# blefaudeux/rusty-marcher

Measured on AMD Instinct MI355X. Metric: Mpixels/sec at 1920x1080, max-bounce=5, higher is better.
Workload: dtype f64

## Files before the change

### rusty-marcher_amd/csrc/rm_classify.inc

```
namespace RM_FLAVOR_NS {
using namespace rmdev;

__device__ __forceinline__ V3 unit(V3 a) {
    const double x = dot(a, a);
    double y = __builtin_amdgcn_rsq(x);
    const double h = 0.5 * x;
    y = y * (1.5 - h * y * y);
    y = y * (1.5 - h * y * y);
    return scaled(a, y);
}

#if RM_KERNEL_ORIENTED
__device__ __forceinline__ V3 cls_dir(const KernelArgs &a, double bx, double by) {
    return mk((bx * a.cam_rx + by * a.cam_ux) + a.cam_fx, (bx * a.cam_ry + by * a.cam_uy) + a.cam_fy, (bx * a.cam_rz + by * a.cam_uz) + a.cam_fz);
}
#else
__device__ __forceinline__ V3 cls_dir(const KernelArgs &, double bx, double by) { return mk(bx, by, -1.); }
#endif
template <bool SHARED>
__device__ __forceinline__ bool cone_of(Bundle &b, const KernelArgs &a, double bx0, double bx1, double by0, double by1, uint32_t sub) {
    const V3 u = unit(cls_dir(a, 0.5 * (bx0 + bx1), 0.5 * (by0 + by1)));
    double cm;
    if (SHARED) {
        cm = dot(unit(cls_dir(a, (sub & 1u) ? bx1 : bx0, (sub & 2u) ? by1 : by0)), u);
// ... 93 lines not shown
struct ClsAsked { double px0, px1, py0, py1, tx0, tx1, ty0, ty1; };
__device__ __forceinline__ ClsAsked classify_ask(const KernelArgs &a, uint32_t patch, bool valid) {
    const uint32_t tile = (valid ? patch : 0u) * 16u + (threadIdx.x & 15u);
    uint32_t tx0, ty0, tyf, ty8;
    tile_origin(a, tile, tx0, ty0, tyf, ty8);
    const uint32_t px0 = tx0 & ~31u, py0 = ty0 & ~31u;
    return ClsAsked{a.bp_x[px0], a.bp_x[px0 + 31u], a.bp_y[py0], a.bp_y[py0 + 31u],
                    a.bp_x[tx0], a.bp_x[tx0 + TILE_W - 1u], a.bp_y[ty0], a.bp_y[ty0 + TILE_H - 1u]};
}
template <bool EDGES>
__device__ __forceinline__ bool classify_patches(const ClsView &scene_blob, const KernelArgs &a, uint32_t patch, bool valid, const ClsAsked &asked,
                                                 unsigned long long *__restrict__ tile_mask, uint32_t n, uint32_t tag, unsigned long long &sig, unsigned long long &own) {
    const uint32_t lane = threadIdx.x & 63u, sub = lane & 15u;
    const uint32_t tile = (valid ? patch : 0u) * 16u + sub;

    Bundle b;
    const bool patch_usable = cone_of<true>(b, a, asked.px0, asked.px1, asked.py0, asked.py1, sub);
    unsigned long long pm = 0ull;
#ifdef RM_CLASSIFY_TWO_CHAINS
    for (uint32_t base = 0; base < n; base += 32u) {
        const uint32_t pid_a = base + sub, pid_b = base + 16u + sub;
        const bool in_a = pid_a < n, in_b = pid_b < n;
        bool keep_a, keep_b;
        keeps2<EDGES>(scene_blob, a, b, pid_a, in_a, pid_b, in_b, keep_a, keep_b);
        pm |= (in_a & (keep_a | !patch_usable)) ? (1ull << (pid_a & 63u)) : 0ull;
        pm |= (in_b & (keep_b | !patch_usable)) ? (1ull << (pid_b & 63u)) : 0ull;
    }
#else
    for (uint32_t base = 0; base < n; base += 16u) {
        const uint32_t pid = base + sub;
        const bool in = pid < n;
        const bool keep = in & (keeps<EDGES>(scene_blob, a, b, pid, in) | !patch_usable);
        pm |= keep ? (1ull << (pid & 63u)) : 0ull;
    }
#endif
    auto group_or = [](unsigned long long v) {
        for (uint32_t off = 1u; off < 16u; off <<= 1) {
            const uint32_t lo = (uint32_t)v | (uint32_t)__shfl_xor((int)(uint32_t)v, (int)off, 64);
            const uint32_t hi = (uint32_t)(v >> 32) | (uint32_t)__shfl_xor((int)(uint32_t)(v >> 32), (int)off, 64);
            v = ((unsigned long long)hi << 32) | lo;
        }
        return v;
    };
    pm = group_or(pm);

    unsigned long long mask = 0ull;
    if (n > (tag ? 56u : 64u)) {
        mask = pm != 0ull ? ~0ull : 0ull;
    } else if (__any(pm != 0ull)) {
        const bool tile_usable = cone_of<false>(b, a, asked.tx0, asked.tx1, asked.ty0, asked.ty1, sub);
        unsigned long long m = pm;
#ifdef RM_CLASSIFY_TWO_CHAINS
        while (__any(m != 0ull)) {
            const bool in_a = m != 0ull;
            const uint32_t pid_a = in_a ? (uint32_t)__builtin_ctzll(m) : 0u;
            m &= m - 1ull;
            const bool in_b = m != 0ull;
            const uint32_t pid_b = in_b ? (uint32_t)__builtin_ctzll(m) : 0u;
            m &= m - 1ull;
            bool keep_a, keep_b;
            keeps2<EDGES>(scene_blob, a, b, pid_a, in_a, pid_b, in_b, keep_a, keep_b);
            mask |= (in_a & (keep_a | !tile_usable)) ? (1ull << pid_a) : 0ull;
            mask |= (in_b & (keep_b | !tile_usable)) ? (1ull << pid_b) : 0ull;
        }
#else
        while (__any(m != 0ull)) {
            const bool in = m != 0ull;
            const uint32_t pid = in ? (uint32_t)__builtin_ctzll(m) : 0u;
            m &= m - 1ull;
            const bool keep = in & (keeps<EDGES>(scene_blob, a, b, pid, in) | !tile_usable);
            mask |= keep ? (1ull << pid) : 0ull;
        }
#endif
    }
    if (valid) {
        if (tag) __hip_atomic_store(tile_mask + tile, ((unsigned long long)tag << 56) | (mask & 0x00FFFFFFFFFFFFFFull), __ATOMIC_RELAXED, __HIP_MEMORY_SCOPE_AGENT);
        else tile_mask[tile] = mask;
    }
    own = valid ? mask : 0ull;
    sig = group_or(own);
    return sig != 0ull;
}

__device__ __forceinline__ uint32_t cost_bucket(uint32_t ticks) {
    if (ticks < 512u) return RM_ORD_SKY - 1u;
    const uint32_t e = 31u - (uint32_t)__builtin_clz(ticks);
    const uint32_t b = 2u * (e - 9u) + ((ticks >> (e - 1u)) & 1u);
    return RM_ORD_SKY - 1u - min(b, RM_ORD_SKY - 1u);
}

struct OrdRec { uint32_t patch, bucket_slot, index; };

struct OrdAsked { uint32_t done, index, cost; };
__device__ __forceinline__ OrdAsked order_ask(const KernelArgs &a, uint32_t patch, bool valid) {
    OrdAsked q;
    q.done = (a.static_list && a.lists_done) ? *a.lists_done : 0u;
    q.index = a.dyn_index ? a.dyn_index[valid ? patch : 0u] : 0u;
    q.cost = (a.key_mode == RM_KEY_COST && a.cost_prev) ? a.cost_prev[valid ? patch : 0u] : 0u;
    return q;
}
__device__ __forceinline__ void order_slot(const KernelArgs &a, uint32_t id, uint32_t patch, bool valid, unsigned long long sig, unsigned long long own, uint32_t prim_cost, const OrdAsked &asked, OrdRec *rec, uint32_t *grec) {
    const uint32_t lane = threadIdx.x & 63u, n_patches = a.n_tiles >> 4, n_dyn = n_patches - (a.n_static >> 4);
    uint32_t c = 0u;
    if (a.key_mode == RM_KEY_CONTENT) {
        unsigned long long m = (valid && own != ~0ull) ? own : 0ull;
        bool unseen = false;
        while (__any(m != 0ull)) {
            const bool in = m != 0ull;
            const uint32_t pid = in ? (uint32_t)__builtin_ctzll(m) : 0u;
            const uint32_t v = (uint32_t)__shfl((int)prim_cost, (int)pid, 64);
            m &= m - 1ull;
            unseen = unseen | (in & (v == ~0u));
            c = max(c, (in && v != ~0u) ? v : 0u);
        }
        c = unseen ? 0x00FFFFFFu : c;
        for (uint32_t off = 1u; off < 16u; off <<= 1) c = max(c, (uint32_t)__shfl_xor((int)c, (int)off, 64));
    } else if (a.key_mode == RM_KEY_COST) {
        c = asked.cost;
    }
    const bool leader = (lane & 15u) == 0u;
    const bool have_lists = a.static_list && a.lists_done && uniform_u32(asked.done) == a.lists_tag;
    const uint32_t index = !valid ? RM_ORD_STATIC_BIT : have_lists ? asked.index : patch < n_dyn ? 0u : RM_ORD_STATIC_BIT | (n_patches - 1u - patch);
    const bool placed = valid & leader & !(index & RM_ORD_STATIC_BIT), first_round = valid & leader & ((index & RM_ORD_STATIC_BIT) != 0u);
    const uint32_t bucket = sig == 0ull ? RM_ORD_SKY
                          : a.key_mode == RM_KEY_PLACE ? (uint32_t)(((unsigned long long)(n_patches - 1u - patch) * (RM_ORD_SKY)) / n_patches)
                                                       : cost_bucket(c);
    const uint32_t counter = bucket * RM_ORD_SUBS + (id & (RM_ORD_SUBS - 1u));
    const uint32_t key = (placed | first_round) ? ((first_round ? RM_ORD_COUNTERS : 0u) | counter) : 0xFFFFu;
    uint32_t before = 0u, total = 0u, first_of = lane >> 4;
#pragma unroll
    for (uint32_t i = 0; i < 4u; i++) {
        const bool same = (uint32_t)__builtin_amdgcn_readlane((int)key, (int)(16u * i)) == key;
        total += same ? 1u : 0u;
        before += (same & (i < (lane >> 4))) ? 1u : 0u;
        first_of = (same & (i < first_of)) ? i : first_of;
    }
    uint32_t base = 0u;
    if (key != 0xFFFFu && before == 0u)
        base = __hip_atomic_fetch_add(a.ord_cnt + ((key & RM_ORD_COUNTERS) ? RM_ORD_FIRST : 0u) + (key & (RM_ORD_COUNTERS - 1u)) * RM_ORD_LINE, total, __ATOMIC_RELAXED, __HIP_MEMORY_SCOPE_AGENT);
    const uint32_t slot = (uint32_t)__shfl((int)base, (int)(16u * first_of), 64) + before;
    if (leader) {
        rec[lane >> 4].patch = valid ? patch : ~0u;
        rec[lane >> 4].bucket_slot = (counter << 24) | slot;
        rec[lane >> 4].index = index;
        if (grec) {
            __hip_atomic_store(grec + (lane >> 4) * 3u + 0u, valid ? patch : ~0u, __ATOMIC_RELAXED, __HIP_MEMORY_SCOPE_AGENT);
            __hip_atomic_store(grec + (lane >> 4) * 3u + 1u, (counter << 24) | slot, __ATOMIC_RELAXED, __HIP_MEMORY_SCOPE_AGENT);
            __hip_atomic_store(grec + (lane >> 4) * 3u + 2u, index, __ATOMIC_RELAXED, __HIP_MEMORY_SCOPE_AGENT);
        }
        if (valid && a.cost_zero) a.cost_zero[patch] = 0u;
    }
}

__device__ __forceinline__ void order_places(const KernelArgs &a, uint32_t id, const OrdRec *rec, bool arrive, bool wait) {
    const uint32_t lane = threadIdx.x & 63u, n_patches = a.n_tiles >> 4, ns16 = a.n_static >> 4, n_dyn = n_patches - ns16;
    const uint32_t n_groups = (a.cls_blocks + 31u) >> 5;
    uint32_t go = 0u;
    if (arrive && lane == 0u && !(a.test_stall == 2u && a.ord_read == a.ord_flat)) {
        const uint32_t g = id >> 5, of = min(32u, a.cls_blocks - 32u * g);
        if (__hip_atomic_fetch_add(a.ord_cnt + RM_ORD_ARRIVE + g * RM_ORD_LINE, 1u, __ATOMIC_RELAXED, __HIP_MEMORY_SCOPE_AGENT) + 1u == of)
            if (__hip_atomic_fetch_add(a.ord_cnt + RM_ORD_GROUPS, 1u, __ATOMIC_RELAXED, __HIP_MEMORY_SCOPE_AGENT) + 1u == n_groups) {
                uint32_t expected = 0u;
                go = __hip_atomic_compare_exchange_strong(a.ord_cnt + RM_ORD_GO, &expected, a.ord_tag, __ATOMIC_RELAXED, __ATOMIC_RELAXED, __HIP_MEMORY_SCOPE_AGENT) ? a.ord_tag : expected;
                if (go == a.ord_tag && a.lists_done_next && a.static_next) *a.lists_done_next = a.ord_tag;
            }
    }
// ... 57 lines not shown
```

### rusty-marcher_amd/csrc/rm_device.hip

```cpp
#include <hip/hip_runtime.h>

#include <chrono>
#include <cmath>
#include <cstdio>
#include <cstdlib>
#include <cstring>
#include <initializer_list>
#include <limits>
#include <new>
#include <string>
#include <utility>
#include <vector>

#include "rm_image.hpp"
#include "rm_internal.h"
#include "rm_kernel_args.hpp"
#include "rm_plan.hpp"
#include "rm_sampling.hpp"
#include "rm_query.hpp"
#include "rm_radiance.hpp"
#include "rm_refine.hpp"
#include "rm_lens.hpp"
#include "rm_accum.hpp"
#include "rm_soft.hpp"
// ... 40 lines not shown
        m = __builtin_fmax(__builtin_fmax(part[0], part[1]), __builtin_fmax(part[2], part[3]));
        atomicMax(out_bits, (unsigned long long)__double_as_longlong(m));
    }
}

__global__ __launch_bounds__(256) void rm_scale_quantize_kernel(double *__restrict__ v, size_t n, const unsigned long long *max_bits,
                                                               int do_scale, uint8_t *__restrict__ out8) {
    double s = 1.;
    bool scale = false;
    if (do_scale) {
        const double max_val = __longlong_as_double((long long)*max_bits);
        if (max_val > 0.) { s = 1. / max_val; scale = true; }
    }
    for (size_t i = (size_t)blockIdx.x * blockDim.x + threadIdx.x; i < n; i += (size_t)gridDim.x * blockDim.x) {
        double f = v[i];
        if (scale) { f = f * s; v[i] = f; }
        if (out8) {
            const double c = 255. * __builtin_fmin(__builtin_fmax(f, 0.), 1.);
            out8[i] = (uint8_t)c;
        }
    }
}


struct rm_frame_slot {
    hipStream_t render = nullptr;
    hipEvent_t begun = nullptr, rendered = nullptr, gathered = nullptr;
    hipEvent_t exchanged = nullptr;
    bool used = false;
    bool stamped = false;
};

struct rm_feedback {
    hipStream_t stream = nullptr;
    void *block = nullptr;
    size_t set_bytes = 0;
    uint64_t used = 0;
    rm_feedback_state s;
};

struct rm_hostio;
struct rm_progressive;
struct rm_tick_swept;
struct rm_converging;
struct rm_denoising;

struct rm_tile_lists {
    hipStream_t stream = nullptr;
    uint32_t cap = 0;
    void *block = nullptr;
    uint64_t used = 0;
    void *order_block = nullptr;
    uint32_t order_cap = 0;
    unsigned long long *hint = nullptr;
    rm_stream_state s;
    unsigned long long *mask() const { return static_cast<unsigned long long *>(block); }
};

struct rm_ctx {
    int device = -1;
    hipStream_t stream = nullptr;
    hipEvent_t ev0 = nullptr, ev1 = nullptr;
    std::string error;
    hipDeviceProp_t prop{};

    bool have_scene = false;
    rm_image image;
    double *d_scene = nullptr;
    size_t d_scene_words = 0;
    rm_vec3 camera{0., 0., 0.};
    bool oriented = false;
    rm_camera_basis basis{{1., 0., 0.}, {0., 1., 0.}, {0., 0., -1.}};
    uint64_t upload_calls = 0, upload_copies = 0;
    std::vector<unsigned char> desc_bytes;
    size_t desc_sizes[6] = {0, 0, 0, 0, 0, 0};
    const rm_knobs knobs = rm_knobs_from_env();
    bool last_launch_exact_only = false;
    uint32_t *d_redo = nullptr;
    std::vector<rm_feedback> feedback;
    uint64_t feedback_clock = 0, scene_epoch = 0;
    uint64_t image_epoch = 0;
    std::vector<rm_tile_lists> tile_lists;
    uint32_t last_launch_grid = 0, last_launch_tail = 0;
    uint32_t last_launch_tiles = 0;
    bool last_launch_classified = false;
    hipStream_t last_launch_stream = nullptr;

    double *d_frame = nullptr;
    size_t frame_bytes = 0;
    uint32_t frame_w = 0, frame_h = 0;

    void *comm = nullptr;
    void *slot_comm[RM_MAX_FRAME_SLOTS] = {};
    int n_comms = 0;
    bool frame_stamps = false;
    bool exchange_all_ranks = false;
    bool comm_failed = false;
    bool comm_local = false;
    int rank = 0, world = 1;
    rm_frame_slot slots[RM_MAX_FRAME_SLOTS];

    double *d_backproject = nullptr;
    size_t backproject_words = 0;
    double backproject_key[6] = {};

    rm_hostio *hostio = nullptr;
    bool comm_stuck = false;

    uint32_t *d_pid_map = nullptr;
    size_t pid_map_words = 0;
    void *d_query = nullptr;
    size_t query_bytes = 0;

    std::vector<std::pair<const void *, int>> shade_occupancy;

    void *d_refine_ws = nullptr;
    size_t refine_ws_bytes = 0;

    void *d_lens_table = nullptr;
    void *d_lens_frame = nullptr;
    size_t lens_frame_bytes = 0;

    rm_progressive *progressive = nullptr;

    rm_converging *converging = nullptr;

    rm_denoising *denoising = nullptr;

    rm_tick_swept *tick_swept = nullptr;
    uint32_t swept_walked = 0;
    uint32_t swept_builds = 0;
    std::vector<rm_swept *> swept_handles;

    unsigned long long *d_max = nullptr;
    uint8_t *d_rgb8 = nullptr;
    size_t rgb8_bytes = 0;
};

static void hostio_destroy(rm_ctx *ctx, bool device_ok);
static bool hostio_packs(rm_ctx *ctx, size_t band_bytes);
static void progressive_destroy(rm_ctx *ctx, bool device_ok);
static void converging_destroy(rm_ctx *ctx, bool device_ok);
static void denoising_destroy(rm_ctx *ctx, bool device_ok);
static void tick_swept_destroy(rm_ctx *ctx, bool device_ok);

static rm_status ctx_fail(rm_ctx *ctx, rm_status st, const std::string &msg) {
    if (ctx) ctx->error = msg;
    else rm_set_host_error(msg);
    return st;
}

template <class F>
static rm_status guarded(rm_ctx *ctx, const char *who, F &&body) {
    try {
        return body();
    } catch (const std::bad_alloc &) {
        return ctx_fail(ctx, RM_ERR_INVALID_ARG, std::string(who) + ": out of host memory");
    } catch (const std::exception &e) {
        return ctx_fail(ctx, RM_ERR_INVALID_ARG, std::string(who) + ": " + e.what());
    } catch (...) {
        return ctx_fail(ctx, RM_ERR_INVALID_ARG, std::string(who) + ": unexpected exception");
    }
}

template <class T>
static T *entry_of(std::vector<T> &v, hipStream_t stream) {
// ... 308 lines not shown
    if (!p) return ctx_fail(ctx, RM_ERR_INVALID_ARG, "render: NULL params");
    if (!ctx->have_scene) return ctx_fail(ctx, RM_ERR_NO_SCENE, "render: no scene uploaded (rm_scene_upload)");
    if (p->patch_size != RM_PATCH_SIZE) return ctx_fail(ctx, RM_ERR_INVALID_ARG, "render: patch_size must be 32 (renderer.rs:47)");
    if (p->max_depth > RM_MAX_DEPTH) return ctx_fail(ctx, RM_ERR_DEPTH, "render: max_depth above RM_MAX_DEPTH");
    if (p->frame_width == 0 || p->frame_height == 0) return ctx_fail(ctx, RM_ERR_INVALID_ARG, "render: empty frame");
    if (p->frame_width % RM_PATCH_SIZE != 0)
        return ctx_fail(ctx, RM_ERR_DIMENSIONS,
                        "render: frame width is not a multiple of 32; the reference's scatter "
                        "(renderer.rs:92-108) indexes out of bounds and panics");
    if (!rm_band_of(*p, band)) return ctx_fail(ctx, RM_ERR_INVALID_ARG, "render: patch_row_begin > patch_row_end");
    return RM_OK;
}

static rm_status backproject_tables(rm_ctx *ctx, const rm_params *p) {
    const double key[6] = {p->width, p->height, p->half_fov, p->ratio, (double)p->frame_width, (double)p->frame_height};
    if (ctx->d_backproject && std::memcmp(key, ctx->backproject_key, sizeof key) == 0) return RM_OK;
    std::vector<double> t((size_t)p->frame_width + p->frame_height);
    for (uint32_t x = 0; x < p->frame_width; x++) t[x] = 2. * ((double)x / p->width - 0.5) * p->half_fov * p->ratio;
    for (uint32_t y = 0; y < p->frame_height; y++) t[p->frame_width + y] = -2. * ((double)y / p->height - 0.5) * p->half_fov;
    RM_HIP(ctx, hipDeviceSynchronize());
    if (ctx->backproject_words < t.size()) {
        if (ctx->d_backproject) RM_HIP(ctx, hipFree(ctx->d_backproject));
        ctx->d_backproject = nullptr;
        RM_HIP(ctx, hipMalloc(&ctx->d_backproject, t.size() * sizeof(double)));
        ctx->backproject_words = t.size();
    }
    RM_HIP(ctx, hipMemcpy(ctx->d_backproject, t.data(), t.size() * sizeof(double), hipMemcpyHostToDevice));
    std::memcpy(ctx->backproject_key, key, sizeof key);
    return RM_OK;
}

static constexpr uint32_t RM_FEEDBACK_STREAMS = 8, RM_CLASSIFY_STREAMS = 8;

static rm_status feedback_for(rm_ctx *ctx, hipStream_t stream, const rm_launch_plan &P, rm_feedback **out) {
    rm_feedback *f = entry_of(ctx->feedback, stream);
    if (!f) {
        if (ctx->feedback.size() >= RM_FEEDBACK_STREAMS) {
            size_t old = 0;
            for (size_t i = 1; i < ctx->feedback.size(); i++)
                if (ctx->feedback[i].used < ctx->feedback[old].used) old = i;
            if (ctx->feedback[old].block) RM_HIP(ctx, hipFree(ctx->feedback[old].block));
            ctx->feedback.erase(ctx->feedback.begin() + (long)old);
        }
        ctx->feedback.emplace_back();
        f = &ctx->feedback.back();
        f->stream = stream;
    }
    f->used = ++ctx->feedback_clock;
    if (P.feedback_reset) {
        f->s.valid = false;
        if (!f->block || f->set_bytes != P.feedback_set_bytes) {
            if (f->block) RM_HIP(ctx, hipFree(f->block));
            f->block = nullptr;
            RM_HIP(ctx, hipMalloc(&f->block, P.feedback_bytes));
        }
        f->set_bytes = P.feedback_set_bytes;
        RM_HIP(ctx, hipMemsetAsync(f->block, 0, P.feedback_bytes, stream));
    }
    *out = f;
    return RM_OK;
}

static rm_status tile_lists_for(rm_ctx *ctx, hipStream_t stream, uint32_t n_tiles, rm_tile_lists **out) {
    rm_tile_lists *t = entry_of(ctx->tile_lists, stream);
    if (!t) {
        if (ctx->tile_lists.size() >= RM_CLASSIFY_STREAMS) {
            size_t old = 0;
            for (size_t i = 1; i < ctx->tile_lists.size(); i++)
                if (ctx->tile_lists[i].used < ctx->tile_lists[old].used) old = i;
            if (ctx->tile_lists[old].block) RM_HIP(ctx, hipFree(ctx->tile_lists[old].block));
            if (ctx->tile_lists[old].order_block) RM_HIP(ctx, hipFree(ctx->tile_lists[old].order_block));
            if (ctx->tile_lists[old].hint) RM_HIP(ctx, hipHostFree(ctx->tile_lists[old].hint));
            ctx->tile_lists.erase(ctx->tile_lists.begin() + (long)old);
        }
        ctx->tile_lists.emplace_back();
        t = &ctx->tile_lists.back();
        t->stream = stream;
    }
    t->used = ++ctx->feedback_clock;
    if (!t->block || t->cap < n_tiles) {
        if (t->block) RM_HIP(ctx, hipFree(t->block));
        t->block = nullptr;
        t->cap = n_tiles;
        RM_HIP(ctx, hipMalloc(&t->block, (size_t)n_tiles * sizeof(unsigned long long)));
    }
    *out = t;
    return RM_OK;
}

static rm_status void_frame_check(rm_ctx *ctx, const char *who) {
    for (rm_tile_lists &t : ctx->tile_lists)
        if (t.hint) {
            const unsigned long long e = *(volatile unsigned long long *)(t.hint + 1);
            if (e) {
                *(volatile unsigned long long *)(t.hint + 1) = 0ull;
                return ctx_fail(ctx, RM_ERR_HIP, std::string(who) + ": launch " + std::to_string((uint32_t)(e >> 32)) +
                                                     " of its stream gave up waiting for its own classification (that frame is void)");
            }
        }
    return RM_OK;
}

static rm_plan_scene plan_scene_of(const rm_ctx *ctx) {
    const rm_image &img = ctx->image;
    return rm_plan_scene{&img.H, ctx->scene_epoch, img.occ_camera_limit, img.integer_exponents, ctx->oriented,
                         ctx->camera, &ctx->basis, (uint32_t)ctx->prop.multiProcessorCount, img.exact_only, img.dead_camera_limit};
}

static rm_status no_kernel(rm_ctx *ctx) { return ctx_fail(ctx, RM_ERR_INVALID_ARG, "render: no kernel for this scene / depth combination"); }

static rm_status choose_kernel(rm_ctx *ctx, const rm_params *p, uint32_t tiles, rm_kernel_choice *k) {
    return choose_kernel(ctx->knobs, plan_scene_of(ctx), *p, tiles, k) ? RM_OK : no_kernel(ctx);
}

static rm_status dump_order(rm_ctx *ctx, const rm_launch_plan &P, hipStream_t stream) {
    const KernelArgs &a = P.args;
    uint32_t c[RM_ORD_BUCKETS] = {}, c1[RM_ORD_BUCKETS] = {}, raw[RM_ORD_ARRIVE] = {};
    RM_HIP(ctx, hipStreamSynchronize(stream));
    RM_HIP(ctx, hipMemcpy(raw, a.ord_cnt, sizeof raw, hipMemcpyDeviceToHost));
    for (uint32_t b = 0; b < RM_ORD_BUCKETS; b++)
        for (uint32_t u = 0; u < RM_ORD_SUBS; u++) { c[b] += raw[(b * RM_ORD_SUBS + u) * RM_ORD_LINE]; c1[b] += raw[RM_ORD_FIRST + (b * RM_ORD_SUBS + u) * RM_ORD_LINE]; }
    uint32_t lit = 0;
    for (uint32_t b = 0; b < RM_ORD_SKY; b++) lit += c[b];
    std::fprintf(stderr, "[rm_order] launch %u keys %u: %u classifying workgroups x %u, first round %u waves, %u + %u sky places; tail %u, room to hand on %u, handed on %u; buckets", a.launch_seq, a.key_mode,
                 a.cls_blocks, a.cls_iters, a.n_static, lit, c[RM_ORD_SKY], a.tail_patches, a.ov_cap, a.tail_patches > c[RM_ORD_SKY] ? std::min(a.ov_cap, a.tail_patches - c[RM_ORD_SKY]) : 0u);
    for (uint32_t b = 0; b < RM_ORD_BUCKETS; b++) std::fprintf(stderr, " %u", c[b]);
    std::fprintf(stderr, " | first round's");
    for (uint32_t b = 0; b < RM_ORD_BUCKETS; b++) std::fprintf(stderr, " %u", c1[b]);
    const uint32_t n_pat = a.n_tiles / 16u, n_dyn_ = n_pat - a.n_static / 16u;
    std::vector<uint32_t> fl(n_dyn_);
    RM_HIP(ctx, hipMemcpy(fl.data(), a.ord_flat, n_dyn_ * sizeof(uint32_t), hipMemcpyDeviceToHost));
    std::vector<uint8_t> seen(n_pat, 0);
    uint32_t untagged = 0, twice = 0, bad = 0;
    for (uint32_t v : fl) {
        if ((v >> RM_ORD_TAG_SHIFT) != a.ord_tag) { untagged++; continue; }
        const uint32_t pch = v & (RM_ORD_SKY_BIT - 1u);
        if (pch >= n_pat) { bad++; continue; }
        twice += seen[pch]; seen[pch] = 1;
    }
    std::fprintf(stderr, " | order laid out: %u places, %u without the tag, %u patches twice, %u out of range; dispatched by %s order; places written %s\n", n_dyn_, untagged, twice, bad,
                 a.ord_read == a.ord_flat ? "its own" : "its predecessor's", a.ord_rec ? "at the grid's end" : "by the classifying workgroups");
    return RM_OK;
}

#if defined(RM_EXP_STAMPS) || defined(RM_EXP_PHASES)
static rm_status stamps_begin(rm_ctx *ctx, rm_launch_plan &P, hipStream_t stream) {
    const size_t n_waves = (size_t)P.grid * P.k.mode.waves;
    RM_HIP(ctx, hipMalloc(&P.args.debug_stamps, n_waves * 48));
    RM_HIP(ctx, hipMemsetAsync(P.args.debug_stamps, 0, n_waves * 48, stream));
    return RM_OK;
}
static rm_status stamps_end(rm_ctx *ctx, const rm_launch_plan &P, hipStream_t stream) {
    const KernelArgs &a = P.args;
    const size_t n_waves = (size_t)P.grid * P.k.mode.waves;
    RM_HIP(ctx, hipStreamSynchronize(stream));
    if (const char *path = std::getenv("RM_DEBUG_STAMPS")) {
        std::fprintf(stderr, "stamps: grid %u cls_blocks %u n_static %u n_tiles %u tail_patches %u tail_q %u ov_cap %u key_mode %u\n", P.grid, a.cls_blocks, a.ord_cnt ? a.n_static : 0u, a.n_tiles, a.tail_patches, a.tail_q, a.ov_cap, a.key_mode);
        std::vector<unsigned long long> h(n_waves * 4);
        RM_HIP(ctx, hipMemcpy(h.data(), a.debug_stamps, n_waves * 32, hipMemcpyDeviceToHost));
        if (FILE *f = std::fopen(path, "wb")) { std::fwrite(h.data(), 8, h.size(), f); std::fclose(f); }
        std::vector<unsigned long long> x(n_waves * 2);
        RM_HIP(ctx, hipMemcpy(x.data(), a.debug_stamps + n_waves * 4, n_waves * 16, hipMemcpyDeviceToHost));
        if (FILE *f = std::fopen((std::string(path) + ".ext").c_str(), "wb")) { std::fwrite(x.data(), 8, x.size(), f); std::fclose(f); }
    }
    RM_HIP(ctx, hipFree(a.debug_stamps));
    return RM_OK;
}
#endif

static rm_status launch_render(rm_ctx *ctx, const rm_params *p, const rm_band &band, double *d_frame,
                               uint8_t *d_frame8, hipStream_t stream) {
    const uint32_t n_rows = band.count();
    if (n_rows == 0) return RM_OK;
    if (p->max_depth == 0) {
        const uint32_t run = band.stride == 1 ? n_rows : 1u;
        for (uint32_t k = 0; k < n_rows; k += run) {
            const size_t first_px = (size_t)((p->flags & RM_FLAG_F64_COMPACT) ? k : band.begin + k * band.stride) * 32u * p->frame_width;
            const size_t n_px = (size_t)run * 32u * p->frame_width;
            hipLaunchKernelGGL(rm_fill_band_kernel, dim3((unsigned)((n_px + 255) / 256)), dim3(256), 0, stream, d_frame,
                               first_px, n_px, p->background.x, p->background.y, p->background.z);
            RM_HIP(ctx, hipGetLastError());
        }
        return RM_OK;
    }
    rm_status bst = backproject_tables(ctx, p);
    if (bst != RM_OK) return bst;
    static const rm_stream_state no_launches;
    static const rm_feedback_state no_feedback;
    rm_tile_lists *tl = entry_of(ctx->tile_lists, stream);
    rm_feedback *fb = entry_of(ctx->feedback, stream);
    const unsigned long long hint = tl && tl->hint ? *(volatile unsigned long long *)tl->hint : 0ull;
    rm_launch_plan P;
    if (!plan_launch(ctx->knobs, plan_scene_of(ctx), *p, band, tl ? tl->s : no_launches, tl ? tl->order_cap : 0u, fb ? fb->s : no_feedback, hint, &P))
        return no_kernel(ctx);
    if (P.ordered)
        if (rm_status vst = void_frame_check(ctx, "render")) return vst;

    if (P.feedback)
        if (rm_status fst = feedback_for(ctx, stream, P, &fb)) return fst;
    if (P.classify) {
        if (rm_status cst = tile_lists_for(ctx, stream, P.args.n_tiles, &tl)) return cst;
        if (P.clear_masks) RM_HIP(ctx, hipMemsetAsync(tl->block, 0, (size_t)tl->cap * sizeof(unsigned long long), stream));
    }
    if (P.ordered) {
        if (tl->order_cap < P.order_patches) {
            if (tl->order_block) RM_HIP(ctx, hipFree(tl->order_block));
            tl->order_block = nullptr;
            tl->order_cap = 0;
            RM_HIP(ctx, hipMalloc(&tl->order_block, rm_order_layout{P.order_cap}.bytes()));
            tl->order_cap = P.order_cap;
        }
        const rm_order_layout L{tl->order_cap};
        if (P.order_clear == rm_launch_plan::ORDER_CLEAR_ALL)
            RM_HIP(ctx, hipMemsetAsync(tl->order_block, 0, L.bytes(), stream));
        else if (P.order_clear == rm_launch_plan::ORDER_CLEAR_FLAT)
            RM_HIP(ctx, hipMemsetAsync(static_cast<uint32_t *>(tl->order_block) + L.flat(0), 0, 2u * L.cap * sizeof(uint32_t), stream));
        if (!tl->hint) {
            RM_HIP(ctx, hipHostMalloc((void **)&tl->hint, 2u * sizeof(unsigned long long), hipHostMallocDefault));
            tl->hint[0] = tl->hint[1] = 0ull;
        }
    }

    KernelArgs &a = P.args;
    char *base[RM_BUF_COUNT] = {};
    if (P.classify) { base[RM_BUF_MASKS] = static_cast<char *>(tl->block); base[RM_BUF_ORDER] = static_cast<char *>(tl->order_block); base[RM_BUF_HINT] = reinterpret_cast<char *>(tl->hint); }
    if (P.feedback) base[RM_BUF_FEEDBACK] = static_cast<char *>(fb->block);
    for (uint32_t i = 0; i < P.n_refs; i++) {
        char *at = base[P.refs[i].buf] + P.refs[i].offset;
        std::memcpy(reinterpret_cast<char *>(&a) + P.refs[i].field, &at, sizeof at);
    }
    a.bp_x = ctx->d_backproject;
    a.bp_y = ctx->d_backproject + p->frame_width;
    a.frame8 = d_frame8;
    a.redo_count = ctx->d_redo;

    if (P.cls_fn) {
        P.cls_args.tile_mask = tl->mask();
        void *cargs[] = {(void *)&ctx->d_scene, (void *)&a, (void *)&P.cls_args};
        RM_HIP(ctx, hipLaunchKernel(P.cls_fn, dim3(P.cls_grid), dim3(64), cargs, 0, stream));
    }
#if defined(RM_EXP_STAMPS) || defined(RM_EXP_PHASES)
    if (rm_status sst = stamps_begin(ctx, P, stream)) return sst;
#endif
    void *args[] = {(void *)&ctx->d_scene, (void *)&a, (void *)&d_frame};
    RM_HIP(ctx, hipLaunchKernel(P.k.fn, dim3(P.grid), dim3(P.block), args, P.lds_bytes, stream));

    if (P.classify) tl->s = P.after;
    if (P.feedback) fb->s = P.feedback_after;
    ctx->last_launch_tiles = a.n_tiles;
    ctx->last_launch_classified = P.classify;
    ctx->last_launch_stream = stream;
    ctx->last_launch_grid = P.grid;
    ctx->last_launch_tail = a.tail_patches;
    ctx->last_launch_exact_only = P.exact_only;
    if (ctx->knobs.debug_tail && P.ordered)
        if (rm_status dst = dump_order(ctx, P, stream)) return dst;
#if defined(RM_EXP_STAMPS) || defined(RM_EXP_PHASES)
    if (rm_status sst = stamps_end(ctx, P, stream)) return sst;
#endif
    return RM_OK;
}

static rm_status rm_render_device_impl(rm_ctx *ctx, const rm_params *params, void *device_rgb, void *hip_stream) {
    if (!ctx) return ctx_fail(nullptr, RM_ERR_INVALID_ARG, "rm_render_device: NULL ctx");
    if (!device_rgb) return ctx_fail(ctx, RM_ERR_INVALID_ARG, "rm_render_device: NULL device buffer");
    rm_band band;
    rm_status st = check_params(ctx, params, &band);
    if (st != RM_OK) return st;
    RM_HIP(ctx, hipSetDevice(ctx->device));
    hipStream_t s = (hipStream_t)hip_stream;
    return launch_render(ctx, params, band, (double *)device_rgb, nullptr, s);
}

rm_status rm_render_device(rm_ctx *ctx, const rm_params *params, void *device_rgb, void *hip_stream) {
    return guarded(ctx, "rm_render_device", [&]() { return rm_render_device_impl(ctx, params, device_rgb, hip_stream); });
}

static rm_status rm_render_device_u8_impl(rm_ctx *ctx, const rm_params *params, void *device_rgb, void *device_rgb8,
                              void *hip_stream) {
    if (!ctx) return ctx_fail(nullptr, RM_ERR_INVALID_ARG, "rm_render_device_u8: NULL ctx");
    if (!device_rgb || !device_rgb8) return ctx_fail(ctx, RM_ERR_INVALID_ARG, "rm_render_device_u8: NULL device buffer");
    rm_band band;
    rm_status st = check_params(ctx, params, &band);
    if (st != RM_OK) return st;
    if (params->max_depth == 0)
        return ctx_fail(ctx, RM_ERR_DEPTH, "rm_render_device_u8: max_depth 0 renders no ray; use rm_render_device + rm_postprocess");
    RM_HIP(ctx, hipSetDevice(ctx->device));
    return launch_render(ctx, params, band, (double *)device_rgb, (uint8_t *)device_rgb8, (hipStream_t)hip_stream);
}

rm_status rm_render_device_u8(rm_ctx *ctx, const rm_params *params, void *device_rgb, void *device_rgb8,
                              void *hip_stream) {
    return guarded(ctx, "rm_render_device_u8", [&]() { return rm_render_device_u8_impl(ctx, params, device_rgb, device_rgb8, hip_stream); });
}

static rm_status rm_render_impl(rm_ctx *ctx, const rm_params *params, double *host_rgb, rm_timing *timing) {
    if (!ctx) return ctx_fail(nullptr, RM_ERR_INVALID_ARG, "rm_render: NULL ctx");
    const auto t_begin = std::chrono::steady_clock::now();
    rm_band band;
    rm_status st = check_params(ctx, params, &band);
    if (st != RM_OK) return st;
    if (params->flags & (RM_FLAG_F64_COMPACT | RM_FLAG_U8_COMPACT))
        return ctx_fail(ctx, RM_ERR_INVALID_ARG, "rm_render: the packed layouts are for rm_render_device* (caller-owned device buffers)");
    RM_HIP(ctx, hipSetDevice(ctx->device));

    const size_t need = (size_t)params->frame_width * params->frame_height * 3u * sizeof(double);
    if (ctx->frame_bytes != need || ctx->frame_w != params->frame_width || ctx->frame_h != params->frame_height) {
        RM_HIP(ctx, hipStreamSynchronize(ctx->stream));
        if (ctx->d_frame) RM_HIP(ctx, hipFree(ctx->d_frame));
        ctx->d_frame = nullptr;
        ctx->frame_bytes = 0;
        RM_HIP(ctx, hipMalloc(&ctx->d_frame, need));
        RM_HIP(ctx, hipMemsetAsync(ctx->d_frame, 0, need, ctx->stream));
        ctx->frame_bytes = need;
        ctx->frame_w = params->frame_width;
        ctx->frame_h = params->frame_height;
    }

    const size_t row_bytes = (size_t)params->frame_width * 3u * sizeof(double);
    const uint32_t n_rows = band.count();
    if (host_rgb && n_rows > 0 && hostio_packs(ctx, (size_t)n_rows * 32u * row_bytes)) {
        std::vector<double *> rows(params->frame_height);
        for (uint32_t y = 0; y < params->frame_height; y++) rows[y] = host_rgb + (size_t)y * params->frame_width * 3u;
        return rm_render_rows(ctx, params, rows.data(), timing);
    }
    RM_HIP(ctx, hipEventRecord(ctx->ev0, ctx->stream));
    st = launch_render(ctx, params, band, ctx->d_frame, nullptr, ctx->stream);
    if (st != RM_OK) return st;
    RM_HIP(ctx, hipEventRecord(ctx->ev1, ctx->stream));

    double d2h_ms = 0.;
    if (host_rgb && n_rows > 0) {
        RM_HIP(ctx, hipStreamSynchronize(ctx->stream));
        const auto t0 = std::chrono::steady_clock::now();
        const uint32_t run = band.stride == 1 ? n_rows : 1u;
        for (uint32_t k = 0; k < n_rows; k += run) {
            const size_t off = (size_t)(band.begin + k * band.stride) * 32u * row_bytes;
            RM_HIP(ctx, hipMemcpy((char *)host_rgb + off, (const char *)ctx->d_frame + off, (size_t)run * 32u * row_bytes,
                                  hipMemcpyDeviceToHost));
        }
        d2h_ms = std::chrono::duration<double, std::milli>(std::chrono::steady_clock::now() - t0).count();
    } else {
        RM_HIP(ctx, hipStreamSynchronize(ctx->stream));
    }
    if (rm_status vst = void_frame_check(ctx, "rm_render")) return vst;
    if (timing) {
        float ms = 0.f;
        RM_HIP(ctx, hipEventElapsedTime(&ms, ctx->ev0, ctx->ev1));
        timing->kernel_ms = ms;
        timing->d2h_ms = d2h_ms;
        timing->total_ms = std::chrono::duration<double, std::milli>(std::chrono::steady_clock::now() - t_begin).count();
    }
    return RM_OK;
}

rm_status rm_render(rm_ctx *ctx, const rm_params *params, double *host_rgb, rm_timing *timing) {
    return guarded(ctx, "rm_render", [&]() { return rm_render_impl(ctx, params, host_rgb, timing); });
}

rm_status rm_kernel_name(rm_ctx *ctx, const rm_params *params, char *buf, size_t buflen) {
    if (!ctx) return ctx_fail(nullptr, RM_ERR_INVALID_ARG, "rm_kernel_name: NULL ctx");
    if (!buf || buflen == 0) return ctx_fail(ctx, RM_ERR_INVALID_ARG, "rm_kernel_name: NULL buffer");
    rm_band band;
    rm_status st = check_params(ctx, params, &band);
    if (st != RM_OK) return st;
    if (params->max_depth == 0) { std::snprintf(buf, buflen, "rm_fill_band_kernel"); return RM_OK; }
    rm_kernel_choice k;
    st = choose_kernel(ctx, params, band.count() * (params->frame_width / RM_PATCH_SIZE) * 16u, &k);
    if (st != RM_OK) return st;
    std::snprintf(buf, buflen, "%s%s::rm_render_static<%d, %d, %d, %d, %s, %s, %s, %s, %s, %s>", k.fast ? "rmdev_fast" : "rmdev_strict", ctx->oriented ? "_o" : "", k.stack,
                  k.pow_mode, k.mode.waves, k.mode.per_wave, k.staged ? "true" : "false", k.bvh ? "true" : "false",
                  k.cull ? "true" : "false", k.edges ? "true" : "false", (k.order || ctx->oriented) ? "true" : "false", k.feedback ? "true" : "false");
    return RM_OK;
}

rm_status rm_launch_stats(rm_ctx *ctx, uint32_t *workgroups, uint32_t *tail_patches) {
    if (!ctx) return ctx_fail(nullptr, RM_ERR_INVALID_ARG, "rm_launch_stats: NULL ctx");
    if (workgroups) *workgroups = ctx->last_launch_grid;
    if (tail_patches) *tail_patches = ctx->last_launch_tail;
    return RM_OK;
}

static rm_status rm_tile_stats_impl(rm_ctx *ctx, void *hip_stream, uint32_t *tiles, uint32_t *tiles_listed) {
    if (!ctx) return ctx_fail(nullptr, RM_ERR_INVALID_ARG, "rm_tile_stats: NULL ctx");
    RM_HIP(ctx, hipSetDevice(ctx->device));
    RM_HIP(ctx, hipDeviceSynchronize());
    const uint32_t n = ctx->last_launch_tiles;
    uint32_t listed = n;
    for (const rm_tile_lists &t : ctx->tile_lists)
        if (t.stream == (hip_stream ? (hipStream_t)hip_stream : ctx->last_launch_stream) && t.block && ctx->last_launch_classified && n <= t.cap) {
            std::vector<unsigned long long> m(n);
            RM_HIP(ctx, hipMemcpy(m.data(), t.mask(), (size_t)n * 8u, hipMemcpyDeviceToHost));
            listed = 0;
            uint32_t hist[64] = {};
            uint64_t bits = 0;
            for (unsigned long long v : m) {
                if (t.s.tagged) v &= 0x00FFFFFFFFFFFFFFull;
                listed += v != 0ull;
                for (int b = 0; b < 64 && v != ~0ull; b++)
                    if (v >> b & 1ull) { hist[b]++; bits++; }
            }
            if (std::getenv("RM_DEBUG_CLASSIFY")) {
                std::fprintf(stderr, "[rm_classify] %u of %u tiles have something to hit, %.2f primitives each; tiles per pid:", listed, n,
                             listed ? (double)bits / listed : 0.);
                for (int b = 0; b < 64; b++)
                    if (hist[b]) std::fprintf(stderr, " %d:%u", b, hist[b]);
                std::fprintf(stderr, "\n");
            }
        }
    if (tiles) *tiles = n;
    if (tiles_listed) *tiles_listed = listed;
    return RM_OK;
}

rm_status rm_tile_stats(rm_ctx *ctx, void *hip_stream, uint32_t *tiles, uint32_t *tiles_listed) {
    return guarded(ctx, "rm_tile_stats", [&]() { return rm_tile_stats_impl(ctx, hip_stream, tiles, tiles_listed); });
}

rm_status rm_device_framebuffer(rm_ctx *ctx, void **device_rgb, size_t *bytes) {
    if (!ctx) return ctx_fail(nullptr, RM_ERR_INVALID_ARG, "rm_device_framebuffer: NULL ctx");
    if (!ctx->d_frame) return ctx_fail(ctx, RM_ERR_INVALID_ARG, "rm_device_framebuffer: nothing rendered yet");
    if (device_rgb) *device_rgb = ctx->d_frame;
    if (bytes) *bytes = ctx->frame_bytes;
    return RM_OK;
}

static rm_status rm_postprocess_impl(rm_ctx *ctx, void *device_rgb, uint32_t w, uint32_t h, int normalize, uint8_t *host_rgb8,
                         double *max_out) {
    if (!ctx) return ctx_fail(nullptr, RM_ERR_INVALID_ARG, "rm_postprocess: NULL ctx");
    RM_HIP(ctx, hipSetDevice(ctx->device));
    double *v = (double *)device_rgb;
    if (!v) {
        if (!ctx->d_frame) return ctx_fail(ctx, RM_ERR_INVALID_ARG, "rm_postprocess: nothing rendered yet");
        if (w != ctx->frame_w || h != ctx->frame_h)
            return ctx_fail(ctx, RM_ERR_INVALID_ARG, "rm_postprocess: size differs from the rendered frame");
        v = ctx->d_frame;
    }
    const size_t n = (size_t)w * h * 3u;
    if (n == 0) return ctx_fail(ctx, RM_ERR_INVALID_ARG, "rm_postprocess: empty frame");
    const unsigned blocks = (unsigned)std::min<size_t>((n + 255) / 256, 2048);
    RM_HIP(ctx, hipMemsetAsync(ctx->d_max, 0, sizeof(unsigned long long), ctx->stream));
    if (normalize) {
        hipLaunchKernelGGL(rm_max_kernel, dim3(blocks), dim3(256), 0, ctx->stream, v, n, ctx->d_max);
        RM_HIP(ctx, hipGetLastError());
    }
    uint8_t *d8 = nullptr;
    if (host_rgb8) {
        if (ctx->rgb8_bytes < n) {
            RM_HIP(ctx, hipStreamSynchronize(ctx->stream));
            if (ctx->d_rgb8) RM_HIP(ctx, hipFree(ctx->d_rgb8));
            ctx->d_rgb8 = nullptr;
            ctx->rgb8_bytes = 0;
            RM_HIP(ctx, hipMalloc(&ctx->d_rgb8, n));
            ctx->rgb8_bytes = n;
        }
        d8 = ctx->d_rgb8;
    }
    if (normalize || d8) {
        hipLaunchKernelGGL(rm_scale_quantize_kernel, dim3(blocks), dim3(256), 0, ctx->stream, v, n, ctx->d_max,
                           normalize ? 1 : 0, d8);
        RM_HIP(ctx, hipGetLastError());
    }
    RM_HIP(ctx, hipStreamSynchronize(ctx->stream));
// ... 37 lines not shown
```

### rusty-marcher_amd/csrc/rm_image.cpp

```cpp
#include "rm_image.hpp"

#include <algorithm>
#include <cmath>
#include <cstring>
#include <limits>

#include "rm_bvh.hpp"
#include "rm_plan.hpp"

namespace {

constexpr uint64_t RM_SCENE_MAX_WORDS = 0xFFFFFFF0ull;
constexpr size_t RM_BVH_MIN_SPHERES = 16, RM_BVH_MIN_TRIANGLES = 12;
constexpr uint32_t RM_SHADOW_MASK_MAX_PRIMS = 64u;
constexpr unsigned RM_EMPTY_SIDE_POS = 1u, RM_EMPTY_SIDE_NEG = 2u;
constexpr double RM_EMPTY_SIDES_CAMERA_MAX = 1e9;

inline uint64_t pack_u32x2(uint32_t lo, uint32_t hi) { return (uint64_t)lo | ((uint64_t)hi << 32); }

inline rm_vec3 v3(double x, double y, double z) { return rm_vec3{x, y, z}; }
inline rm_vec3 operator-(rm_vec3 a, rm_vec3 b) { return v3(a.x - b.x, a.y - b.y, a.z - b.z); }
inline rm_vec3 scaled(rm_vec3 a, double s) { return v3(a.x * s, a.y * s, a.z * s); }
inline double dot(rm_vec3 a, rm_vec3 b) { return a.x * b.x + a.y * b.y + a.z * b.z; }
inline rm_vec3 cross(rm_vec3 a, rm_vec3 b) { return v3(a.y * b.z - a.z * b.y, a.z * b.x - a.x * b.z, a.x * b.y - a.y * b.x); }


struct PlaneSep { bool h = false, n = false; };
inline void try_plane(PlaneSep &sep, rm_vec3 n, const rm_vec3 *w, uint32_t nv, rm_vec3 cl, double r, rm_vec3 a, double sin_t,
                      double marg) {
    const double len = std::sqrt(dot(n, n));
    if (!(len > 1e-150) || !std::isfinite(len)) return;
    n = scaled(n, 1. / len);
    for (int sign = 0; sign < 2; sign++, n = scaled(n, -1.)) {
        double lo = HUGE_VAL;
        for (uint32_t i = 0; i < nv; i++) lo = std::fmin(lo, dot(w[i], n));
        if (!std::isfinite(lo)) continue;
        sep.h = sep.h || lo > std::fmax(0., dot(cl, n) + r) + marg;
        sep.n = sep.n || (dot(a, n) >= sin_t + 1e-9 && lo > marg);
    }
}

void rm_build_shadow_masks(const double *blob, const rm_dev_header &H, unsigned long long *occ) {
    const uint32_t n = H.n_spheres + H.n_polygons + H.n_triangles, nl = H.n_lights;
    const unsigned long long all = n >= 64u ? ~0ull : ((1ull << n) - 1ull);
    const double rho = H.shadow_rho;
    auto finite3 = [](rm_vec3 v) { return std::isfinite(v.x) && std::isfinite(v.y) && std::isfinite(v.z); };
    auto mag = [](rm_vec3 v) { return std::fabs(v.x) + std::fabs(v.y) + std::fabs(v.z); };
    for (uint32_t l = 0; l < nl; l++) {
        const double *lw = blob + H.off_lights + RM_LIGHT_WORDS * l;
        const rm_vec3 L = v3(lw[0], lw[1], lw[2]);
        for (uint32_t P = 0; P < n; P++) {
            unsigned long long &m = occ[(size_t)P * nl + l];
            m = all;
            const double *bp = blob + H.off_bounds + 4u * P;
            const rm_vec3 c = v3(bp[0], bp[1], bp[2]);
            if (!(bp[3] >= 0.) || !std::isfinite(bp[3]) || !finite3(c) || !finite3(L) || !(rho >= 0.) || !std::isfinite(rho)) continue;
            const double tol = 1e-7 * (1. + mag(L) + mag(c) + bp[3]);
            const double r = bp[3] + tol;
            const rm_vec3 cl = c - L;
            const double D = std::sqrt(dot(cl, cl));
            if (!(D > r * (1. + 1e-6) + rho + tol)) continue;
            const rm_vec3 a = scaled(cl, 1. / D);
            const double sin_t = std::fmin(1., r / D * (1. + 1e-9) + 1e-9);
            const double cos_t = std::sqrt(std::fmax(0., 1. - sin_t * sin_t)) * (1. - 1e-9);
            const double cap = D + r;
            unsigned long long keep = 1ull << P;
            for (uint32_t Q = 0; Q < n; Q++) {
                if (Q == P) continue;
                const double *bq = blob + H.off_bounds + 4u * Q;
                if (bq[3] < 0.) continue;
                const rm_vec3 cq = v3(bq[0], bq[1], bq[2]);
                if (!std::isfinite(bq[3]) || !finite3(cq)) { keep |= 1ull << Q; continue; }
                const double marg = rho + tol + 1e-7 * (mag(cq) + bq[3]);
                const double R = bq[3] + marg;
                const rm_vec3 v = cq - L, x = cross(v, a);
                const double h = dot(v, a), q = std::sqrt(dot(x, x));
                bool out = (q * cos_t - std::fabs(h) * sin_t > R) || (h - R > cap);
                if (!out && Q >= H.n_spheres) {
                    const double *pl = blob + H.off_planar + 16u * (Q - H.n_spheres);
                    const uint32_t nv = pl[12] == 3. ? 3u : pl[12] == 4. ? 4u : 0u;
                    rm_vec3 w[4];
                    bool fin = nv != 0u;
                    for (uint32_t i = 0; i < nv; i++) { w[i] = v3(pl[3 * i], pl[3 * i + 1], pl[3 * i + 2]) - L; fin = fin && finite3(w[i]); }
                    if (fin) {
                        PlaneSep sep;
                        try_plane(sep, a, w, nv, cl, r, a, sin_t, marg);
                        try_plane(sep, v3(1., 0., 0.), w, nv, cl, r, a, sin_t, marg);
                        try_plane(sep, v3(0., 1., 0.), w, nv, cl, r, a, sin_t, marg);
                        try_plane(sep, v3(0., 0., 1.), w, nv, cl, r, a, sin_t, marg);
                        try_plane(sep, cross(w[1] - w[0], w[2] - w[0]), w, nv, cl, r, a, sin_t, marg);
                        for (uint32_t i = 0; i < nv; i++) try_plane(sep, cross(w[i], w[(i + 1u) % nv]), w, nv, cl, r, a, sin_t, marg);
                        out = sep.h && sep.n;
                    }
                }
                if (!out) keep |= 1ull << Q;
            }
            m = keep;
        }
    }
}

void rm_build_empty_sides(const double *blob, const rm_dev_header &H, unsigned char *sides) {
    const uint32_t n = H.n_spheres + H.n_polygons + H.n_triangles;
    const double rho = H.shadow_rho, big = 1e6;
    auto finite3 = [](rm_vec3 v) { return std::isfinite(v.x) && std::isfinite(v.y) && std::isfinite(v.z); };
    auto mag = [](rm_vec3 v) { return std::fabs(v.x) + std::fabs(v.y) + std::fabs(v.z); };
    for (uint32_t P = 0; P < n; P++) sides[P] = 0;
    if (!(rho >= 0.) || !std::isfinite(rho)) return;
    for (uint32_t P = H.n_spheres; P < n; P++) {
        const double *rec = P < H.n_spheres + H.n_polygons ? blob + H.off_polygons + RM_POLYGON_WORDS * (P - H.n_spheres)
                                                           : blob + H.off_triangles + RM_TRIANGLE_WORDS * (P - H.n_spheres - H.n_polygons);
        const rm_vec3 nrm = v3(rec[0], rec[1], rec[2]), pp = v3(rec[3], rec[4], rec[5]);
        const double *bp = blob + H.off_bounds + 4u * P;
        const rm_vec3 c = v3(bp[0], bp[1], bp[2]);
        if (!(bp[3] >= 0.) || !std::isfinite(bp[3]) || !finite3(c) || !finite3(nrm) || !finite3(pp)) continue;
        if (!(std::fabs(std::sqrt(dot(nrm, nrm)) - 1.) <= 1e-6)) continue;
        if (!(mag(c) + bp[3] < big) || !(mag(pp) < big)) continue;
        bool pos = true, neg = true;
        for (uint32_t Q = 0; Q < n && (pos || neg); Q++) {
            if (Q == P) continue;
            const double *bq = blob + H.off_bounds + 4u * Q;
            if (bq[3] < 0.) continue;
            const rm_vec3 cq = v3(bq[0], bq[1], bq[2]);
            if (!std::isfinite(bq[3]) || !finite3(cq) || !(mag(cq) + bq[3] < big)) { pos = neg = false; break; }
            const double marg = 1e-4 + rho + 1e-7 * (1. + mag(pp) + mag(cq) + bq[3]);
            const double h = dot(cq - pp, nrm);
            bool below = h + bq[3] < -marg, above = h - bq[3] > marg;
            if (!below && !above && Q >= H.n_spheres) {
                const double *pl = blob + H.off_planar + 16u * (Q - H.n_spheres);
                const uint32_t nv = pl[12] == 3. ? 3u : pl[12] == 4. ? 4u : 0u;
                bool lo = nv != 0u, hi = nv != 0u;
                for (uint32_t i = 0; i < nv; i++) {
                    const rm_vec3 w = v3(pl[3 * i], pl[3 * i + 1], pl[3 * i + 2]);
                    if (!finite3(w) || !(mag(w) < big)) { lo = hi = false; break; }
                    const double mw = 1e-4 + rho + 1e-7 * (1. + mag(pp) + mag(w));
                    const double hw = dot(w - pp, nrm);
                    lo = lo && hw < -mw;
                    hi = hi && hw > mw;
                }
                below = lo; above = hi;
            }
            pos = pos && below;
            neg = neg && above;
        }
        sides[P] = (unsigned char)((pos ? RM_EMPTY_SIDE_POS : 0u) | (neg ? RM_EMPTY_SIDE_NEG : 0u));
    }
}
bool scene_exact_only(const rm_scene_desc *d) {
    bool ok = true;
    auto v3 = [&](const rm_vec3 &v) { ok = ok && rm_checked_coord_ok(v.x) && rm_checked_coord_ok(v.y) && rm_checked_coord_ok(v.z); };
    for (uint32_t i = 0; i < d->n_spheres; i++) {
        v3(d->spheres[i].center);
        const double r2 = d->spheres[i].radius_square;
        ok = ok && r2 >= RM_CHECKED_R2_MIN && r2 <= RM_CHECKED_R2_MAX && rm_checked_coord_ok(r2);
    }
    for (uint32_t i = 0; i < d->n_polygons; i++) { v3(d->polygons[i].plane_normal); v3(d->polygons[i].plane_point); }
    for (uint32_t i = 0; i < d->n_polygon_vertices; i++) v3(d->polygon_vertices[i]);
    for (uint32_t i = 0; i < d->n_triangles; i++) {
        const rm_triangle &t = d->triangles[i];
        v3(t.normal); v3(t.center);
        for (const rm_vec3 &v : t.vertices) v3(v);
    }
    for (uint32_t i = 0; i < d->n_lights; i++) {
        v3(d->lights[i].position); v3(d->lights[i].color);
        ok = ok && rm_checked_coord_ok(d->lights[i].intensity);
    }
    return !ok;
}

struct kind_list {
    std::vector<uint32_t> src;
    std::vector<uint32_t> key;
};

// ... 283 lines not shown
    double camera_limit() const {
        double size = 0.;
        for (uint32_t q = 0; q < n_prims; q++) {
            const double *w = &blob[H.off_bounds + 4u * q];
            if (w[3] >= 0.) size = std::fmax(size, std::fabs(w[0]) + std::fabs(w[1]) + std::fabs(w[2]) + w[3]);
        }
        for (uint32_t l = 0; l < H.n_lights; l++) {
            const double *w = &blob[H.off_lights + RM_LIGHT_WORDS * l];
            size = std::fmax(size, std::fabs(w[0]) + std::fabs(w[1]) + std::fabs(w[2]));
        }
        return std::isfinite(size) ? 1e6 * (1. + size) : 0.;
    }

    void mark_empty_sides() {
        if (n_prims == 0u || n_prims > RM_SHADOW_MASK_MAX_PRIMS) return;
        img.empty_sides.assign(n_prims, 0);
        rm_build_empty_sides(blob.data(), H, img.empty_sides.data());
        bool any = false;
        for (uint32_t q = 0; q < n_prims; q++) {
            double &glass = blob[H.off_materials + RM_MATERIAL_WORDS * q + 8];
            if (glass != 0. && img.empty_sides[q]) {
                glass = 1. + ((img.empty_sides[q] & RM_EMPTY_SIDE_POS) ? 2. : 0.) + ((img.empty_sides[q] & RM_EMPTY_SIDE_NEG) ? 4. : 0.);
                any = true;
            }
        }
        if (any) img.dead_camera_limit = std::fmin(camera_limit(), RM_EMPTY_SIDES_CAMERA_MAX);
    }

    void append_occluder_masks() {
        if (n_prims == 0u || n_prims > RM_SHADOW_MASK_MAX_PRIMS || H.n_lights == 0u) return;
        const uint64_t words = (uint64_t)n_prims * H.n_lights;
        if ((uint64_t)H.total_words + words + 2u > RM_SCENE_MAX_WORDS) return;
        H.off_occ = H.total_words;
        blob.resize((size_t)H.total_words + ((words + 1u) & ~1ull), 0.);
        rm_build_shadow_masks(blob.data(), H, reinterpret_cast<unsigned long long *>(&blob[H.off_occ]));
        img.occ_camera_limit = camera_limit();
    }
};

}

bool rm_desc_arrays_present(const rm_scene_desc *d) {
    return !((d->n_shapes && !d->shapes) || (d->n_spheres && !d->spheres) || (d->n_polygons && !d->polygons) ||
             (d->n_polygon_vertices && !d->polygon_vertices) || (d->n_triangles && !d->triangles) || (d->n_lights && !d->lights));
}

rm_status rm_build_image(const rm_scene_desc *d, const rm_image_options &opt, rm_image &img, std::string &error) {
    img = rm_image{};
    image_builder b(d, img, error);
    if (!rm_desc_arrays_present(d)) return b.fail(RM_ERR_INVALID_ARG, "rm_scene_upload: NULL array with non-zero count");
    if (rm_status st = b.regroup()) return st;
    if (opt.use_bvh) b.build_hierarchies();
    b.number_pids();
    if (rm_status st = b.lay_out()) return st;
    b.write_records();
    b.write_groups();
    b.mark_empty_sides();
    if (opt.shadow_masks) b.append_occluder_masks();
    img.exact_only = scene_exact_only(d);
    return RM_OK;
}


static rm_status hook_image(const char *who, const rm_scene_desc *d, const void *out, const rm_image_options &opt, rm_image &img) {
    std::string error = std::string(who) + ": NULL argument";
    const rm_status st = (d && out) ? rm_build_image(d, opt, img, error) : RM_ERR_INVALID_ARG;
    if (st) rm_set_host_error(error);
    return st;
}

extern "C" rm_status rmi_shadow_masks(const rm_scene_desc *d, uint64_t *occ, uint32_t *shape_of, uint32_t cap, uint32_t *dims) {
    rm_image img;
    if (rm_status st = hook_image("rmi_shadow_masks", d, dims, rm_image_options{}, img)) return st;
    const rm_dev_header &H = img.H;
    const uint32_t n = H.n_spheres + H.n_polygons + H.n_triangles;
    dims[0] = n; dims[1] = H.n_lights; dims[2] = H.off_occ ? 1u : 0u;
    if (H.off_occ && occ && shape_of && (uint64_t)n * H.n_lights <= cap) {
        std::memcpy(occ, &img.blob[H.off_occ], (size_t)n * H.n_lights * sizeof(uint64_t));
        for (uint32_t q = 0; q < n; q++) shape_of[q] = img.pid_map[2u * q];
    }
    return RM_OK;
}

extern "C" rm_status rmi_empty_sides(const rm_scene_desc *d, uint8_t *sides, double *glass, uint32_t *shape_of, uint32_t cap, uint32_t *dims, double *camera_limit) {
    rm_image img;
    if (rm_status st = hook_image("rmi_empty_sides", d, dims, rm_image_options{}, img)) return st;
    const rm_dev_header &H = img.H;
    const uint32_t n = H.n_spheres + H.n_polygons + H.n_triangles;
    dims[0] = n; dims[1] = img.empty_sides.empty() ? 0u : 1u;
    if (camera_limit) *camera_limit = img.dead_camera_limit;
    if (dims[1] && sides && glass && shape_of && n <= cap) {
        for (uint32_t q = 0; q < n; q++) {
            sides[q] = img.empty_sides[q];
            glass[q] = img.blob[H.off_materials + RM_MATERIAL_WORDS * q + 8];
            shape_of[q] = img.pid_map[2u * q];
        }
    }
    return RM_OK;
}

extern "C" rm_status rmi_upload_numerics(const rm_scene_desc *d, double *materials, uint32_t cap, uint32_t *dims) {
    rm_image img;
    if (rm_status st = hook_image("rmi_upload_numerics", d, dims, rm_image_options{}, img)) return st;
    const uint32_t n = img.H.n_spheres + img.H.n_polygons + img.H.n_triangles;
    dims[0] = n; dims[1] = img.exact_only ? 1u : 0u;
    if (materials && (uint64_t)n * RM_MATERIAL_WORDS <= cap)
        std::memcpy(materials, &img.blob[img.H.off_materials], (size_t)n * RM_MATERIAL_WORDS * sizeof(double));
    return RM_OK;
}

extern "C" rm_status rmi_scene_image(const rm_scene_desc *d, uint32_t use_bvh, uint32_t shadow_masks, uint64_t *sizes, uint32_t *header,
                                     double *reals, uint32_t *verdicts, uint64_t *blob, uint64_t blob_cap, uint32_t *pid_map, uint64_t map_cap) {
    rm_image img;
    const bool outs = sizes && header && reals && verdicts;
    if (rm_status st = hook_image("rmi_scene_image", d, outs ? sizes : nullptr, rm_image_options{use_bvh != 0, shadow_masks != 0}, img)) return st;
    const rm_dev_header &H = img.H;
    const uint32_t fields[19] = {H.n_spheres, H.n_polygons, H.n_triangles, H.n_lights, H.off_spheres, H.off_polygons, H.off_pverts,
                                 H.off_triangles, H.off_materials, H.off_lights, H.off_keys, H.total_words, H.list_ordered,
                                 H.off_bvh_spheres, H.off_bvh_triangles, H.off_bounds, H.off_planar, H.off_groups, H.off_occ};
    std::memcpy(header, fields, sizeof fields);
    reals[0] = H.shadow_rho; reals[1] = img.occ_camera_limit; reals[2] = img.dead_camera_limit;
    verdicts[0] = img.exact_only ? 1u : 0u; verdicts[1] = img.integer_exponents ? 1u : 0u;
    sizes[0] = img.blob.size(); sizes[1] = img.pid_map.size();
    if (blob && pid_map && img.blob.size() <= blob_cap && img.pid_map.size() <= map_cap) {
        std::memcpy(blob, img.blob.data(), img.blob.size() * sizeof(double));
        if (!img.pid_map.empty()) std::memcpy(pid_map, img.pid_map.data(), img.pid_map.size() * sizeof(uint32_t));
    }
    return RM_OK;
}
```

### rusty-marcher_amd/csrc/rm_kernel_args.hpp

```cpp
#ifndef RM_KERNEL_ARGS_HPP
#define RM_KERNEL_ARGS_HPP

#include <stdint.h>

#include "rm_internal.h"

#define RM_ORD_BUCKETS 16u
#define RM_ORD_SKY 15u
#define RM_ORD_MAX_CLS 1024u
#define RM_ORD_LINE 32u
#define RM_ORD_SUBS 4u
#define RM_ORD_COUNTERS (RM_ORD_BUCKETS * RM_ORD_SUBS)
#define RM_ORD_FIRST (RM_ORD_COUNTERS * RM_ORD_LINE)
#define RM_ORD_ARRIVE (2u * RM_ORD_COUNTERS * RM_ORD_LINE)
#define RM_ORD_GROUPS (RM_ORD_ARRIVE + (RM_ORD_MAX_CLS / 32u) * RM_ORD_LINE)
#define RM_ORD_GO (RM_ORD_GROUPS + RM_ORD_LINE)
#define RM_ORD_CNT_WORDS (RM_ORD_GO + RM_ORD_LINE)
#define RM_ORD_STATIC_BIT 0x80000000u
#define RM_ORD_FALLBACK_BIT 0x80000000u
#define RM_ORD_PATIENCE 4096u
#define RM_ORD_PATCH_BITS 20u
#define RM_ORD_SKY_BIT (1u << RM_ORD_PATCH_BITS)
#define RM_ORD_TAG_SHIFT (RM_ORD_PATCH_BITS + 1u)
#define RM_ORD_TAG_BITS 11u
#define RM_CTAB_WORDS 128u
enum { RM_KEY_PLACE = 0, RM_KEY_COST = 1, RM_KEY_CONTENT = 2 };

#ifndef RM_MIN_WAVES
#define RM_MIN_WAVES 4
#endif
#ifndef RM_EDGES_WAVES
#define RM_EDGES_WAVES 3
#endif

namespace rmdev {

enum { POW_GENERIC = 0, POW_INTEGER = 1 };


#ifndef RM_TILE_W
#define RM_TILE_W 16
#endif
constexpr uint32_t TILE_W = RM_TILE_W, TILE_H = 64u / RM_TILE_W;
static_assert(TILE_W == 8 || TILE_W == 16 || TILE_W == 32, "tile width");

struct KernelArgs {
    rm_dev_header H;
    double half_fov, height, width, ratio;
    double cam_x, cam_y, cam_z;
    double bg_x, bg_y, bg_z;
    uint32_t frame_width;
    uint32_t patch_row_begin;
    uint32_t patch_row_stride;
    uint32_t u8_compact;
    uint32_t max_depth;
    uint32_t n_width;
    uint32_t n_tiles;
    uint32_t order_mul;
    uint32_t order_add;
    uint32_t f64_compact;
    double cull_cos;
    uint8_t *frame8;
    const double *bp_x, *bp_y;
    unsigned long long *debug_stamps;
    const uint32_t *fb_list;
    const uint32_t *fb_count;
    const uint8_t *fb_flag;
    const uint32_t *fb_hist;
    uint32_t *fb_next_list, *fb_next_count, *fb_next_hist;
    uint8_t *fb_next_flag;
    uint32_t *fb_zero;
    uint32_t *fb_threshold;
    uint32_t fb_cap;
    uint32_t fb_long_ticks;
    uint32_t fb_target;
    const unsigned long long *tile_mask;
    uint32_t mask_exact;
    uint32_t mask_tag;
    uint32_t mask_tag_prev;
    uint32_t cls_blocks;
    uint32_t cls_prims;
    uint32_t cls_lds_words;
    uint32_t cull_lds_words;
    uint32_t *ord_cnt;
    uint32_t *ord_cnt_next;
    uint32_t *ord_flat;
    const uint32_t *ord_read;
    uint32_t ord_read_tag;
    uint32_t *ord_rec;
    uint32_t ord_cap;
    uint32_t ord_tag;
    uint32_t cls_iters;
    const uint32_t *static_list;
    const uint32_t *dyn_index;
    const uint32_t *dyn_inv;
    uint32_t *static_next, *dyn_index_next, *dyn_inv_next;
    const uint32_t *lists_done;
    uint32_t lists_tag;
    uint32_t *lists_done_next;
    uint32_t n_static;
    uint32_t key_mode;
    uint32_t *patch_cost;
    const uint32_t *cost_prev;
    uint32_t *cost_zero;
    const uint32_t *ctab;
    uint32_t *ctab_cur;
    uint32_t *ctab_zero;
    uint32_t tail_patches;
    uint32_t ov_cap;
    uint32_t first_round;
    uint32_t tail_q;
    unsigned long long *ord_hint;
    unsigned long long *err_word;
    uint32_t launch_seq;
    uint32_t test_stall;
    double cam_rx, cam_ry, cam_rz, cam_ux, cam_uy, cam_uz, cam_fx, cam_fy, cam_fz;
    uint32_t exact_only;
    uint32_t dead_children;
    uint32_t *redo_count;
};

static constexpr uint32_t RM_DEAD_DROP = 1u, RM_DEAD_EARLY_FATES = 2u;

struct ClassifyArgs {
    unsigned long long *tile_mask;
    uint32_t n_prims;
    uint32_t _pad;
};

const void *rm_classify_kernel(bool edges);
const void *rm_classify_kernel_oriented(bool edges);

#define RM_FB_BUCKETS 64u
#define RM_FB_SAMPLE 8u
struct StackEntry {
    double ox, oy, oz, dx, dy, dz, w;
    uint32_t depth, _pad;
};

#define RM_WAVE_L0_DEPTH_WORDS 448u
#define RM_WAVE_BVH_STACK_WORDS 480u
#define RM_WAVE_SUM_WORDS 512u
#define RM_WAVE_PAIR_WORDS 704u
#define RM_WAVE_T0_WORDS 736u
#define RM_WAVE_LDS_WORDS 738u
#define RM_LDS_SCENE_LIMIT_WORDS 512u

}

const void *rm_pick_kernel(bool fast, bool staged, bool bvh, bool cull, bool edges, int order, bool feedback, int stack, int pow_mode);
const void *rm_pick_kernel_oriented(bool fast, bool staged, bool bvh, bool cull, bool edges, int stack, int pow_mode);

#endif
```

### rusty-marcher_amd/csrc/rm_plan.cpp

```cpp
#include "rm_plan.hpp"

#include <algorithm>
#include <cmath>
#include <cstdlib>
#include <cstring>
#include <string>

using namespace rmdev;

namespace {

enum knob_rule {
    IS_1,
    NOT_0,
    IS_SET,
    ONE_OR_ZERO,
    ATOI,
    ATOI_MIN_0,
    ATOI_MIN_1,
    STRTOUL,
    TILE_ORDER,
    TAIL_PLACE,
    CULL_OFF,
    CULL_COS,
    DEAD_CHILDREN,
};

struct knob {
    const char *name;
    knob_rule rule;
    bool rm_knobs::*b = nullptr;
    int rm_knobs::*i = nullptr;
    uint32_t rm_knobs::*u = nullptr;
    double rm_knobs::*d = nullptr;
    constexpr knob(const char *n, bool rm_knobs::*f, knob_rule r) : name(n), rule(r), b(f) {}
    constexpr knob(const char *n, int rm_knobs::*f, knob_rule r) : name(n), rule(r), i(f) {}
    constexpr knob(const char *n, uint32_t rm_knobs::*f, knob_rule r) : name(n), rule(r), u(f) {}
    constexpr knob(const char *n, double rm_knobs::*f, knob_rule r) : name(n), rule(r), d(f) {}
};

const knob k_knobs[] = {
    {"RM_FORCE_GENERIC_POW", &rm_knobs::force_generic_pow, IS_1},
    {"RM_FORCE_FAST_FP", &rm_knobs::force_fast_fp, IS_1},
    {"RM_FORCE_UNSTAGED", &rm_knobs::force_unstaged, IS_1},
    {"RM_SHADOW_MASKS", &rm_knobs::shadow_masks, NOT_0},
    {"RM_DEAD_CHILDREN", &rm_knobs::dead_children, DEAD_CHILDREN},
    {"RM_DISABLE_BVH", &rm_knobs::disable_bvh, IS_1},
    {"RM_SWEPT_BVH", &rm_knobs::swept_bvh, NOT_0},
    {"RM_FORCE_STACK", &rm_knobs::force_stack, ATOI},
    {"RM_FEEDBACK", &rm_knobs::feedback_mode, ONE_OR_ZERO},
    {"RM_FEEDBACK_US", &rm_knobs::feedback_us, ATOI_MIN_1},
    {"RM_FEEDBACK_TARGET", &rm_knobs::feedback_target, ATOI_MIN_0},
    {"RM_DEBUG_EMPTY", &rm_knobs::debug_empty, IS_1},
    {"RM_TILE_CLASSIFY", &rm_knobs::classify_mode, ONE_OR_ZERO},
    {"RM_CLASSIFY_IN_LAUNCH", &rm_knobs::classify_in_launch, IS_1},
    {"RM_PATCH_ORDER", &rm_knobs::patch_order_mode, ONE_OR_ZERO},
    {"RM_SKY_TAIL", &rm_knobs::sky_tail, NOT_0},
    {"RM_SKY_TAIL_FORCE", &rm_knobs::sky_tail_force, ATOI},
    {"RM_PATCH_ORDER_MAX", &rm_knobs::patch_order_max, ATOI_MIN_0},
    {"RM_SKY_TAIL_BIG", &rm_knobs::sky_tail_big, NOT_0},
    {"RM_PATCH_ORDER_MAX_DEEP", &rm_knobs::patch_order_max_deep, ATOI_MIN_0},
    {"RM_SKY_TAIL_ROOM_DIV", &rm_knobs::sky_tail_room_div, ATOI_MIN_1},
    {"RM_SKY_TAIL_BIG_MIN", &rm_knobs::sky_tail_big_min, ATOI_MIN_0},
    {"RM_SKY_TAIL_PLACE", &rm_knobs::sky_tail_place, TAIL_PLACE},
    {"RM_SKY_TAIL_MOTION", &rm_knobs::sky_tail_motion, NOT_0},
    {"RM_SKY_TAIL_CAP", &rm_knobs::sky_tail_cap, ATOI_MIN_0},
    {"RM_ORDER_KEYS", &rm_knobs::order_keys, ATOI},
    {"RM_FIRST_ROUND", &rm_knobs::first_round, ATOI_MIN_0},
    {"RM_FIRST_ROUND_FROM_ORDER", &rm_knobs::first_round_from_order, NOT_0},
    {"RM_ORDER_REUSE", &rm_knobs::order_reuse, NOT_0},
    {"RM_STATIC_ROUNDS", &rm_knobs::static_rounds, ATOI_MIN_1},
    {"RM_CLS_MAX_BLOCKS", &rm_knobs::cls_max_blocks, ATOI_MIN_1},
    {"RM_ORDER_FREEZE", &rm_knobs::order_freeze, ATOI_MIN_0},
    {"RM_ORDER_LATE_PLACES", &rm_knobs::order_late_places, NOT_0},
    {"RM_MASK_REUSE", &rm_knobs::mask_reuse, NOT_0},
    {"RM_CLASSIFY_LDS", &rm_knobs::classify_lds, NOT_0},
    {"RM_CLASSIFY_IN_LAUNCH_PRIMS", &rm_knobs::classify_in_launch_prims, ATOI_MIN_0},
    {"RM_CLASSIFY_MIN_TILES", &rm_knobs::classify_min_tiles, ATOI_MIN_0},
    {"RM_ORD_TAG_WRAP", &rm_knobs::ord_tag_wrap, ATOI_MIN_1},
    {"RM_TEST_STALL_ORDER", &rm_knobs::test_stall_order, ATOI},
    {"RM_TILE_ORDER", &rm_knobs::tile_order, TILE_ORDER},
    {"RM_DISABLE_CULL", &rm_knobs::cull_cos, CULL_OFF},
    {"RM_CULL_COS", &rm_knobs::cull_cos, CULL_COS},
    {"RM_CULL_MIN", &rm_knobs::cull_min_prims, STRTOUL},
    {"RM_CULL_EDGES", &rm_knobs::cull_edges, NOT_0},
    {"RM_CHECKED_NUMERICS", &rm_knobs::checked_numerics, NOT_0},
    {"RM_REFINE_MAX_BLOCKS", &rm_knobs::refine_max_blocks, ATOI_MIN_0},
    {"RM_LENS_MAX_BLOCKS", &rm_knobs::lens_max_blocks, ATOI_MIN_0},
    {"RM_DEBUG_TAIL", &rm_knobs::debug_tail, IS_SET},
};

}

rm_knobs rm_knobs_from_env() {
    rm_knobs kn;
    for (const knob &k : k_knobs) {
        const char *env = std::getenv(k.name);
        if (!env) continue;
        switch (k.rule) {
        case IS_1: kn.*k.b = env[0] == '1'; break;
        case NOT_0: kn.*k.b = env[0] != '0'; break;
        case IS_SET: kn.*k.b = true; break;
        case ONE_OR_ZERO: kn.*k.i = env[0] == '1' ? 1 : 0; break;
        case ATOI: kn.*k.i = std::atoi(env); break;
        case ATOI_MIN_0:
            if (k.i) kn.*k.i = std::max(0, std::atoi(env));
            else kn.*k.u = (uint32_t)std::max(0, std::atoi(env));
            break;
        case ATOI_MIN_1: kn.*k.u = (uint32_t)std::max(1, std::atoi(env)); break;
        case STRTOUL: kn.*k.u = (uint32_t)std::strtoul(env, nullptr, 10); break;
        case TILE_ORDER:
            kn.*k.i = !std::strcmp(env, "reverse") ? TILE_ORDER_REVERSE : !std::strcmp(env, "hash") ? TILE_ORDER_HASH : TILE_ORDER_NATURAL;
            break;
        case TAIL_PLACE: kn.*k.i = env[0] == 'e' && env[1] == 'v' ? 1 : env[0] == 'e' ? 2 : 0; break;
        case CULL_OFF: kn.*k.d = env[0] == '1' ? 2. : kn.*k.d; break;
        case CULL_COS: kn.*k.d = std::max(0.05, std::atof(env)); break;
        case DEAD_CHILDREN: kn.*k.b = env[0] != '0'; kn.early_fates = env[0] != '0' && env[0] != '1'; break;
        }
    }
    if (kn.classify_min_tiles == 0u) kn.classify_min_tiles = RM_CLASSIFY_MIN_TILES_DEFAULT;
    return kn;
}


static constexpr size_t RM_LDS_SCENE_LIMIT_BYTES = RM_LDS_SCENE_LIMIT_WORDS * sizeof(double);
static constexpr uint32_t RM_FEEDBACK_MIN_TILES = 32768;
static constexpr uint32_t RM_CLASSIFY_MAX_COST = 4000;
static constexpr uint32_t RM_CLASSIFY_IN_LAUNCH_MAX_COST = 1000;
// ... 84 lines not shown
    a.frame_width = p.frame_width;
    a.patch_row_begin = band.begin;
    a.patch_row_stride = band.stride;
    a.u8_compact = (p.flags & RM_FLAG_U8_COMPACT) ? 1u : 0u;
    a.f64_compact = (p.flags & RM_FLAG_F64_COMPACT) ? 1u : 0u;
    a.max_depth = p.max_depth;
    a.n_width = p.frame_width / RM_PATCH_SIZE;
    a.n_tiles = band.count() * a.n_width * 16u;
    a.order_mul = 1; a.order_add = 0;
    if (kn.tile_order == TILE_ORDER_REVERSE && a.n_tiles > 1) {
        a.order_mul = a.n_tiles - 1; a.order_add = a.n_tiles - 1;
    } else if (kn.tile_order == TILE_ORDER_HASH && a.n_tiles > 2) {
        uint32_t mul = (uint32_t)(a.n_tiles * 0.6180339887) | 1u;
        auto gcd = [](uint32_t x, uint32_t y) { while (y) { uint32_t t = x % y; x = y; y = t; } return x; };
        while (gcd(mul, a.n_tiles) != 1) mul += 2;
        a.order_mul = mul % a.n_tiles;
    }

    if (!choose_kernel(kn, sc, p, a.n_tiles, &P.k)) return false;
    const rm_kernel_choice &k = P.k;
    const uint32_t n_prims = k.n_prims, n_planar = k.n_planar;
    a.dead_children = ((kn.dead_children && !k.bvh && !k.cull && sc.dead_camera_limit > 0. &&
                        std::fabs(sc.camera.x) + std::fabs(sc.camera.y) + std::fabs(sc.camera.z) <= sc.dead_camera_limit) ? RM_DEAD_DROP : 0u) |
                      ((kn.early_fates && !k.bvh && !k.cull) ? RM_DEAD_EARLY_FATES : 0u);
    const uint32_t cull_steps = (n_prims + 63u) / 64u;
    const uint32_t planar_steps = n_planar ? cull_steps - H.n_spheres / 64u : 0u;
    const uint32_t cull_cost = 25u * cull_steps + (k.planar_edges ? 85u * planar_steps : 0u);
    a.cull_cos = cull_cost > RM_CULL_MAX_COST ? 2. : kn.cull_cos;
    a.first_round = sc.n_cus * 4u * (k.edges ? RM_EDGES_WAVES : RM_MIN_WAVES);
    if (kn.first_round >= 0) a.first_round = (uint32_t)kn.first_round;
    P.block = (uint32_t)k.mode.waves * 64u;
    P.lds_bytes = k.lds_bytes;
    const uint32_t per_wg = (uint32_t)(k.mode.waves * k.mode.per_wave);
    P.grid = (a.n_tiles + per_wg - 1) / per_wg;
    P.feedback = k.feedback && per_wg == 1u && !kn.debug_empty;
    if (P.feedback) {
        const rm_feedback_layout L(a.n_tiles);
        rm_feedback_state &next = P.feedback_after;
        next.valid = true;
        next.key[0] = (uint64_t)a.n_tiles | ((uint64_t)p.frame_width << 32);
        next.key[1] = (uint64_t)band.begin | ((uint64_t)band.stride << 32);
        next.key[2] = sc.scene_epoch;
        next.n_tiles = a.n_tiles;
        const bool same = fb.valid && fb.n_tiles == a.n_tiles && std::memcmp(fb.key, next.key, sizeof fb.key) == 0;
        P.feedback_reset = !same;
        P.feedback_bytes = L.bytes();
        P.feedback_set_bytes = L.set_bytes;
        const int r = same ? fb.cur : 0, w = (r + 1) % 3, z = (r + 2) % 3;
        next.cur = w;
        point(P, &KernelArgs::fb_list, RM_BUF_FEEDBACK, L.list(r)); point(P, &KernelArgs::fb_count, RM_BUF_FEEDBACK, L.count(r));
        point(P, &KernelArgs::fb_flag, RM_BUF_FEEDBACK, L.flag(r)); point(P, &KernelArgs::fb_hist, RM_BUF_FEEDBACK, L.hist(r));
        point(P, &KernelArgs::fb_next_list, RM_BUF_FEEDBACK, L.list(w)); point(P, &KernelArgs::fb_next_count, RM_BUF_FEEDBACK, L.count(w));
        point(P, &KernelArgs::fb_next_flag, RM_BUF_FEEDBACK, L.flag(w)); point(P, &KernelArgs::fb_next_hist, RM_BUF_FEEDBACK, L.hist(w));
        point(P, &KernelArgs::fb_zero, RM_BUF_FEEDBACK, L.hist(z));
        point(P, &KernelArgs::fb_threshold, RM_BUF_FEEDBACK, L.threshold());
        a.fb_cap = L.cap;
        a.fb_long_ticks = kn.feedback_us * 100u;
        const uint32_t slots = sc.n_cus * 16u;
        a.fb_target = kn.feedback_target >= 0 ? (uint32_t)kn.feedback_target : 4u * slots;
        a.fb_target = std::min(a.fb_target, L.cap / 2u);
        P.grid = a.n_tiles + L.cap;
    }
    if (kn.debug_empty) a.n_tiles = 0;

    rm_stream_state s = before;
    uint32_t mask_tag_before = 0u;
    uint32_t cls_words_wanted = 0u;
    P.classify = kn.classify_mode != 0 && !kn.debug_empty && per_wg == 1u && n_prims > 0u &&
                 k.classify_cost <= RM_CLASSIFY_MAX_COST && (kn.classify_mode == 1 || a.n_tiles >= kn.classify_min_tiles);
    if (P.classify) {
        const bool in_launch = kn.classify_in_launch && (n_prims <= kn.classify_in_launch_prims || k.order_in_big_scene) && !k.feedback;
        if (in_launch) {
            if (!s.tagged || s.tagged_tiles != a.n_tiles || s.tagged_scene != sc.scene_epoch || s.tag >= 255u) {
                P.clear_masks = true;
                s.tag = 0;
                s.tagged = true; s.tagged_tiles = a.n_tiles; s.tagged_scene = sc.scene_epoch;
            }
            a.mask_tag = ++s.tag;
            mask_tag_before = a.mask_tag > 1u ? a.mask_tag - 1u : 0u;
            a.cls_blocks = (a.n_tiles / 16u + 3u) / 4u;
            a.cls_prims = n_prims;
            P.grid += a.cls_blocks;
            cls_words_wanted = (!k.staged && kn.classify_lds) ? 4u * n_prims + 22u * n_planar : 0u;
        } else {
            s.tagged = false;
            P.cls_fn = sc.oriented ? rm_classify_kernel_oriented(n_planar > 0u) : rm_classify_kernel(n_planar > 0u);
            P.cls_grid = (a.n_tiles / 16u + 3u) / 4u;
            P.cls_args.n_prims = n_prims;
        }
        point(P, &KernelArgs::tile_mask, RM_BUF_MASKS, 0);
        a.mask_exact = n_prims <= (in_launch ? 56u : 64u) ? 1u : 0u;
    }
    const uint32_t n_patches = a.n_tiles / 16u;
    const uint64_t rounds = (uint64_t)a.first_round * kn.static_rounds * 2u <= a.n_tiles ? kn.static_rounds : 1u;
    a.n_static = (uint32_t)std::min<uint64_t>(((uint64_t)a.first_round * rounds) & ~15ull, a.n_tiles);
    const uint32_t n_dyn = n_patches - a.n_static / 16u;
    const uint32_t cls_max = std::min<uint32_t>(RM_ORD_MAX_CLS, std::max(1u, kn.cls_max_blocks));
    P.ordered = k.order && per_wg == 1u && a.cls_blocks != 0u && n_dyn > 0u && n_patches < (1u << RM_ORD_PATCH_BITS) &&
                n_patches <= 16u * 4u * cls_max;
    if (P.ordered) {
        const uint64_t key[3] = {(uint64_t)a.n_tiles | ((uint64_t)p.frame_width << 32), (uint64_t)band.begin | ((uint64_t)band.stride << 32),
                                 sc.scene_epoch ^ ((uint64_t)a.n_static << 40)};
        P.order_patches = n_patches;
        const bool grown = order_cap < n_patches;
        const rm_order_layout L{grown ? n_patches : order_cap};
        P.order_cap = (uint32_t)L.cap;
        const uint32_t tag_wrap = kn.ord_tag_wrap ? kn.ord_tag_wrap : (1u << RM_ORD_TAG_BITS) - 1u;
        const bool fresh = grown || std::memcmp(s.order_key, key, sizeof key) != 0;
        if (fresh || s.ord_tag >= tag_wrap) {
            P.order_clear = fresh ? rm_launch_plan::ORDER_CLEAR_ALL : rm_launch_plan::ORDER_CLEAR_FLAT;
            if (fresh) {
                std::memcpy(s.order_key, key, sizeof key);
                s.order_frames = 0;
                s.static_read = s.static_written = -1;
                s.list_tag[0] = s.list_tag[1] = 0u;
            }
            s.ord_tag = 0;
            s.last_tag = 0;
        }
        const uint32_t f = s.order_frames++;
        const uint32_t seq = ++s.seq;
        if (f == 0u) s.key_seq0 = seq;
        const double view[16] = {sc.camera.x, sc.camera.y, sc.camera.z, p.half_fov, p.height, p.width, p.ratio,
                                 cb.right.x, cb.right.y, cb.right.z, cb.up.x, cb.up.y, cb.up.z, cb.forward.x, cb.forward.y, cb.forward.z};
        if (f == 0u || std::memcmp(s.view, view, sizeof view) != 0) {
            std::memcpy(s.view, view, sizeof view);
            s.view_seq0 = seq;
        }
        const bool timed = n_patches <= (k.order_in_big_scene ? kn.patch_order_max_deep : kn.patch_order_max);
        const uint32_t groups4 = (n_patches + 3u) / 4u;
        a.cls_iters = (groups4 + cls_max - 1u) / cls_max;
        a.cls_blocks = (groups4 + a.cls_iters - 1u) / a.cls_iters;
        const bool reuse = kn.order_reuse && f >= 3u && seq >= s.view_seq0 + 3u && s.last_tag != 0u;
        a.ord_cap = P.order_cap;
        a.ord_tag = ++s.ord_tag;
        a.ord_read_tag = reuse ? s.last_tag : a.ord_tag;
        s.last_tag = a.ord_tag;
        const bool late_places = reuse && kn.order_late_places;
        a.mask_tag_prev = reuse && kn.mask_reuse ? mask_tag_before : 0u;
        P.frozen = kn.order_freeze > 0 && reuse && f >= 4u && before.frozen_run < (uint32_t)kn.order_freeze && a.mask_tag > 1u &&
                   a.mask_tag_prev != 0u && late_places && kn.test_stall_order == 0 && kn.sky_tail_force < 0 && !kn.debug_tail;
        const bool lays_out = !P.frozen;
        point(P, &KernelArgs::ord_cnt, RM_BUF_ORDER, 4u * L.cnt(f & 1u));
        point(P, &KernelArgs::ord_flat, RM_BUF_ORDER, 4u * L.flat(f & 1u));
        point(P, &KernelArgs::ord_read, RM_BUF_ORDER, 4u * L.flat(reuse ? (f + 1u) & 1u : f & 1u));
        if (lays_out) point(P, &KernelArgs::ord_cnt_next, RM_BUF_ORDER, 4u * L.cnt((f + 1u) & 1u));
        if (lays_out && late_places) point(P, &KernelArgs::ord_rec, RM_BUF_ORDER, 4u * L.rec());
        if (timed) point(P, &KernelArgs::patch_cost, RM_BUF_ORDER, 4u * L.cost(f % 3u));
        if (timed) point(P, &KernelArgs::cost_prev, RM_BUF_ORDER, 4u * L.cost((f + 2u) % 3u));
        if (timed && lays_out) point(P, &KernelArgs::cost_zero, RM_BUF_ORDER, 4u * L.cost((f + 1u) % 3u));
        point(P, &KernelArgs::ctab, RM_BUF_ORDER, 4u * L.ctab((f + 2u) % 3u));
        if (timed && kn.order_keys != 1) point(P, &KernelArgs::ctab_cur, RM_BUF_ORDER, 4u * L.ctab(f % 3u));
        if (lays_out) point(P, &KernelArgs::ctab_zero, RM_BUF_ORDER, 4u * L.ctab((f + 1u) % 3u));
        if (kn.first_round_from_order) {
            const int read = reuse ? s.static_read : s.static_written;
            const uint32_t write = read == 0 ? 1u : 0u;
            if (read >= 0) {
                point(P, &KernelArgs::static_list, RM_BUF_ORDER, 4u * L.first((uint32_t)read));
                point(P, &KernelArgs::dyn_index, RM_BUF_ORDER, 4u * L.index((uint32_t)read));
                point(P, &KernelArgs::dyn_inv, RM_BUF_ORDER, 4u * L.inv((uint32_t)read));
                point(P, &KernelArgs::lists_done, RM_BUF_ORDER, 4u * (L.done() + (uint32_t)read));
                a.lists_tag = s.list_tag[read];
            }
            if (lays_out) {
                point(P, &KernelArgs::static_next, RM_BUF_ORDER, 4u * L.first(write));
                point(P, &KernelArgs::dyn_index_next, RM_BUF_ORDER, 4u * L.index(write));
// ... 183 lines not shown
```

### rusty-marcher_amd/csrc/rm_plan.hpp

```cpp
#ifndef RM_PLAN_HPP
#define RM_PLAN_HPP

#include <stddef.h>
#include <stdint.h>

#include "rm_internal.h"
#include "rm_kernel_args.hpp"

enum { TILE_ORDER_NATURAL = 0, TILE_ORDER_REVERSE = 1, TILE_ORDER_HASH = 2 };

static constexpr uint32_t RM_CLASSIFY_MIN_TILES_DEFAULT = 3584;
static constexpr uint32_t RM_CULL_MIN_PRIMS = 12, RM_CULL_EDGES_MIN_PLANAR = 4, RM_CULL_MAX_COST = 250;

struct rm_knobs {
    bool force_generic_pow = false;
    bool force_fast_fp = false;
    int tile_order = TILE_ORDER_REVERSE;
    bool disable_bvh = false;
    bool swept_bvh = true;
    double cull_cos = 0.975;
    uint32_t cull_min_prims = RM_CULL_MIN_PRIMS;
    bool cull_edges = true;
    bool force_unstaged = false;
    bool shadow_masks = true;
    bool dead_children = true;
    bool early_fates = true;
    int force_stack = 0;
    bool debug_empty = false;
    int feedback_mode = -1;
    uint32_t feedback_us = 50;
    int feedback_target = -1;
    int classify_mode = -1;
    bool classify_in_launch = true;
    bool sky_tail = true;
    uint32_t patch_order_max = 4096;
    uint32_t patch_order_max_deep = 65536;
    uint32_t sky_tail_big_min = 16384;
    uint32_t sky_tail_room_div = 16;
    bool sky_tail_big = true;
    bool sky_tail_motion = true;
    int sky_tail_place = 0;
    int sky_tail_cap = -1;
    bool classify_lds = true;
    uint32_t classify_in_launch_prims = 56;
    uint32_t classify_min_tiles = RM_CLASSIFY_MIN_TILES_DEFAULT;
    bool mask_reuse = true;
    uint32_t static_rounds = 2;
    uint32_t cls_max_blocks = RM_ORD_MAX_CLS;
    int order_freeze = 7;
    bool order_late_places = true;
    bool order_reuse = true;
    bool first_round_from_order = true;
    int first_round = -1;
    int order_keys = -1;
    uint32_t ord_tag_wrap = 0;
    int test_stall_order = 0;
    int sky_tail_force = -1;
    int patch_order_mode = -1;
    bool checked_numerics = true;
    uint32_t refine_max_blocks = 0;
    uint32_t lens_max_blocks = 0;
    bool debug_tail = false;
};
rm_knobs rm_knobs_from_env();

struct rm_band {
    uint32_t begin = 0, end = 0, stride = 1;
    uint32_t count() const { return end > begin ? (end - begin + stride - 1) / stride : 0; }
};

bool rm_band_of(const rm_params &p, rm_band *band);

struct rm_plan_scene {
    const rm_dev_header *H;
    uint64_t scene_epoch;
    double occ_camera_limit;
    bool integer_exponents;
    bool oriented;
    rm_vec3 camera;
    const rm_camera_basis *basis;
    uint32_t n_cus;
    bool exact_only = false;
    double dead_camera_limit = 0.;
};

static constexpr double RM_CHECKED_COORD_MAX = 0x1p+200;
static constexpr double RM_CHECKED_R2_MIN = 0x1p-600, RM_CHECKED_R2_MAX = 0x1p+600;
inline bool rm_checked_coord_ok(double v) { return v >= -RM_CHECKED_COORD_MAX && v <= RM_CHECKED_COORD_MAX; }
bool rm_camera_exact_only(const rm_plan_scene &sc);

struct rm_launch_mode {
    int waves = 0;
    int per_wave = 1;
};

struct rm_kernel_choice {
    const void *fn = nullptr;
    rm_launch_mode mode;
    size_t lds_bytes = 0;
    int stack = 0, pow_mode = 0;
    bool fast = false, staged = false, bvh = false, cull = false, edges = false, order = false, feedback = false;
    bool order_in_big_scene = false;
    uint32_t n_prims = 0, n_planar = 0, classify_cost = 0;
    bool planar_edges = false;
};
bool choose_kernel(const rm_knobs &kn, const rm_plan_scene &sc, const rm_params &p, uint32_t tiles, rm_kernel_choice *k);

struct rm_shading_variant {
    bool bvh;
    int pow_mode;
    int stack;
};
rm_shading_variant rm_shading_variant_of(const rm_knobs &kn, const rm_dev_header &H, bool integer_exponents, uint32_t max_depth);

uint32_t rm_shading_grid(uint32_t total, uint32_t rays_per_pixel, int n_cus, int per_cu, uint32_t max_blocks);

struct rm_stream_state {
    uint32_t order_frames = 0;
    uint64_t order_key[3] = {0, 0, 0};
    uint32_t list_tag[2] = {0, 0};
    int static_read = -1, static_written = -1;
    uint32_t last_tag = 0;
    uint32_t seq = 0, view_seq0 = 0, key_seq0 = 0, ord_tag = 0;
    double view[16] = {0., 0., 0., 0., 0., 0., 0., 0., 0., 0., 0., 0., 0., 0., 0., 0.};
    uint32_t tag = 0, tagged_tiles = 0;
    uint64_t tagged_scene = 0;
    bool tagged = false;
    uint32_t frozen_run = 0;
};

struct rm_feedback_state {
    bool valid = false;
    uint64_t key[3] = {0, 0, 0};
    uint32_t n_tiles = 0;
    int cur = 0;
};

struct rm_order_layout {
    size_t cap;
    size_t cost(uint32_t j) const { return (size_t)j * cap; }
    size_t ctab(uint32_t j) const { return 3u * cap + j * RM_CTAB_WORDS; }
    size_t cnt(uint32_t j) const { return 3u * cap + 3u * RM_CTAB_WORDS + j * RM_ORD_CNT_WORDS; }
    size_t flat(uint32_t j) const { return cnt(2) + (size_t)j * cap; }
    size_t first(uint32_t j) const { return flat(2u + j); }
    size_t index(uint32_t j) const { return flat(4u + j); }
    size_t inv(uint32_t j) const { return flat(6u + j); }
    size_t rec() const { return flat(8u); }
    size_t done() const { return rec() + 3u * (cap + 4096u); }
    size_t bytes() const { return (cap * 11u + 64u + 3u * (cap + 4096u) + 3u * RM_CTAB_WORDS + 2u * RM_ORD_CNT_WORDS) * 4u; }
};

struct rm_feedback_layout {
    uint32_t n_tiles, cap;
    size_t set_bytes;
    explicit rm_feedback_layout(uint32_t tiles)
        : n_tiles(tiles), cap((tiles + 7u) / 8u > 64u ? (tiles + 7u) / 8u : 64u),
          set_bytes((((size_t)cap + RM_FB_BUCKETS + 4u) * sizeof(uint32_t) + tiles + 255u) & ~(size_t)255u) {}
    size_t hist(int j) const { return (size_t)j * set_bytes; }
    size_t count(int j) const { return hist(j) + RM_FB_BUCKETS * 4u; }
    size_t list(int j) const { return hist(j) + (RM_FB_BUCKETS + 4u) * 4u; }
    size_t flag(int j) const { return list(j) + (size_t)cap * 4u; }
    size_t threshold() const { return hist(3); }
    size_t bytes() const { return 3u * set_bytes + 256u; }
};

enum rm_buf : uint8_t { RM_BUF_MASKS, RM_BUF_ORDER, RM_BUF_HINT, RM_BUF_FEEDBACK, RM_BUF_COUNT };
struct rm_arg_ref {
    uint16_t field;
    rm_buf buf;
    uint32_t offset;
};

struct rm_launch_plan {
    rm_kernel_choice k;
    uint32_t grid = 0, block = 0;
    size_t lds_bytes = 0;
    rmdev::KernelArgs args{};
    rm_arg_ref refs[40];
    uint32_t n_refs = 0;
    bool feedback = false;
    bool classify = false;
    const void *cls_fn = nullptr;
    uint32_t cls_grid = 0;
    rmdev::ClassifyArgs cls_args{};
    bool exact_only = false;
    bool ordered = false;
    bool frozen = false;
    bool feedback_reset = false;
    size_t feedback_bytes = 0, feedback_set_bytes = 0;
    bool clear_masks = false;
    uint32_t order_patches = 0;
    enum { ORDER_CLEAR_NONE, ORDER_CLEAR_FLAT, ORDER_CLEAR_ALL } order_clear = ORDER_CLEAR_NONE;
    uint32_t order_cap = 0;
    rm_stream_state after;
    rm_feedback_state feedback_after;
};

bool plan_launch(const rm_knobs &kn, const rm_plan_scene &sc, const rm_params &p, const rm_band &band, const rm_stream_state &s,
                 uint32_t order_cap, const rm_feedback_state &fb, unsigned long long hint, rm_launch_plan *out);

#endif
```

### rusty-marcher_amd/csrc/rm_render_kernel.hpp

```cpp
#ifndef RM_RENDER_KERNEL_HPP
#define RM_RENDER_KERNEL_HPP

#include <hip/hip_runtime.h>

#include "rm_kernel_args.hpp"

namespace rmdev {

__device__ __forceinline__ uint32_t fb_bucket(uint32_t ticks) {
    const uint32_t t = ticks < 4u ? 4u : ticks;
    const uint32_t e = 31u - (uint32_t)__builtin_clz(t);
    const uint32_t b = 4u * (e - 2u) + ((t >> (e - 2u)) & 3u);
    return b < RM_FB_BUCKETS ? b : RM_FB_BUCKETS - 1u;
}
__device__ __forceinline__ uint32_t fb_edge(uint32_t b) { return (4u + (b & 3u)) << (b >> 2); }

__device__ __forceinline__ double own_sgpr(double v) { double r; asm("s_mov_b64 %0, %1" : "=s"(r) : "s"(v)); return r; }
__device__ __forceinline__ uint32_t own_sgpr(uint32_t v) { uint32_t r; asm("s_mov_b32 %0, %1" : "=s"(r) : "s"(v)); return r; }

__device__ __forceinline__ uint32_t uniform_u32(uint32_t v) { return (uint32_t)__builtin_amdgcn_readfirstlane((int)v); }
__device__ __forceinline__ unsigned long long uniform_u64(unsigned long long v) {
    return ((unsigned long long)uniform_u32((uint32_t)(v >> 32)) << 32) | uniform_u32((uint32_t)v);
}

__device__ __forceinline__ bool lists_ok(const KernelArgs &a) {
    return a.static_list && a.lists_done && uniform_u32(*a.lists_done) == a.lists_tag;
}

__device__ __forceinline__ const char *reread_kernargs(const char *kargs) {
    unsigned long long p = uniform_u64((unsigned long long)kargs);
    asm volatile("s_mov_b64 %0, %1" : "=s"(p) : "s"(p));
    return (const char *)reinterpret_cast<const __attribute__((address_space(4))) char *>(p);
}

extern __shared__ double rm_lds[];

__device__ __forceinline__ void stage_scene(const double *__restrict__ scene_blob, const rm_dev_header &H) {
    const double2 *src = reinterpret_cast<const double2 *>(scene_blob);
    double2 *dst = reinterpret_cast<double2 *>(rm_lds);
    const uint32_t n2 = H.total_words / 2;
    for (uint32_t i = threadIdx.x; i < n2; i += blockDim.x) dst[i] = src[i];
    __syncthreads();
}

struct SceneAsked { double2 v[RM_LDS_SCENE_LIMIT_WORDS / 128u]; };
__device__ __forceinline__ SceneAsked stage_scene_ask(const double *__restrict__ scene_blob, const rm_dev_header &H) {
    const double2 *src = reinterpret_cast<const double2 *>(scene_blob);
    const uint32_t n2 = H.total_words / 2, lane = threadIdx.x & 63u;
    SceneAsked p;
#pragma unroll
    for (uint32_t k = 0; k < RM_LDS_SCENE_LIMIT_WORDS / 128u; k++) {
        p.v[k] = double2{0., 0.};
        if (lane + 64u * k < n2) p.v[k] = src[lane + 64u * k];
    }
    return p;
}
__device__ __forceinline__ void stage_scene_put(const SceneAsked &p, const rm_dev_header &H) {
    double2 *dst = reinterpret_cast<double2 *>(rm_lds);
    const uint32_t n2 = H.total_words / 2, lane = threadIdx.x & 63u;
#pragma unroll
    for (uint32_t k = 0; k < RM_LDS_SCENE_LIMIT_WORDS / 128u; k++)
        if (lane + 64u * k < n2) dst[lane + 64u * k] = p.v[k];
    __syncthreads();
}

__device__ __forceinline__ uint32_t tile_of_id(const KernelArgs &a, uint32_t id) {
    const uint32_t last = a.n_tiles - 1u;
    return (a.order_mul == 1u && a.order_add == 0u) ? id
         : (a.order_mul == last && a.order_add == last) ? last - id
         : (uint32_t)(((unsigned long long)id * a.order_mul + a.order_add) % a.n_tiles);
}

__device__ __forceinline__ void tile_origin(const KernelArgs &a, uint32_t tile, uint32_t &tx0, uint32_t &ty0, uint32_t &tyf,
                                            uint32_t &ty8) {
    const uint32_t patch = tile >> 4, sub = tile & 15u;
    const uint32_t pcol = patch % a.n_width, prow = patch / a.n_width;
    tx0 = pcol * 32u + (sub & (32u / TILE_W - 1u)) * TILE_W;
    const uint32_t in_patch = (sub / (32u / TILE_W)) * TILE_H;
    ty0 = (a.patch_row_begin + prow * a.patch_row_stride) * 32u + in_patch;
    const uint32_t packed = prow * 32u + in_patch;
    tyf = a.f64_compact ? packed : ty0;
    ty8 = a.u8_compact ? packed : ty0;
}

}

#ifndef RM_KERNEL_ORIENTED
#define RM_KERNEL_ORIENTED 0
// ... 53 lines not shown
```

### rusty-marcher_amd/csrc/rm_render_kernel.inc

```
namespace RM_FLAVOR_NS {
using namespace rmdev;

template <int STACK, int POW, bool BVH, bool CULL, bool EDGES, bool PREFETCHED>
__device__ __forceinline__ bool render_tile(const SceneView &sc, const KernelArgs &a, uint32_t tx0, uint32_t ty0,
                                            uint32_t tyf, uint32_t ty8, double bp_x, double bp_y, double *wl,
                                            double *__restrict__ frame_in, unsigned long long *stats, bool have_mask,
                                            unsigned long long first_mask, const char *kargs_of_kernel) {
    const uint32_t lane = threadIdx.x & 63u;
    const V3 bg = mk(own_sgpr(a.bg_x), own_sgpr(a.bg_y), own_sgpr(a.bg_z));
    const uint32_t max_depth = own_sgpr(a.max_depth);
#if RM_CHECKED
    bool sus = false;
#endif

    double *const lds0 = wl + lane;
    uint32_t *const l0_depth = reinterpret_cast<uint32_t *>(wl + RM_WAVE_L0_DEPTH_WORDS);
    double *const sum = wl + RM_WAVE_SUM_WORDS;
    uint32_t *const pair = reinterpret_cast<uint32_t *>(wl + RM_WAVE_PAIR_WORDS);

#if RM_KERNEL_ORIENTED
    const double bx = PREFETCHED ? bp_x : a.bp_x[tx0 + (lane % TILE_W)], by = PREFETCHED ? bp_y : a.bp_y[ty0 + (lane / TILE_W)];
    V3 dir = RM_NORMALIZED(mk((bx * a.cam_rx + by * a.cam_ux) + a.cam_fx, (bx * a.cam_ry + by * a.cam_uy) + a.cam_fy, (bx * a.cam_rz + by * a.cam_uz) + a.cam_fz), true);
#else
    V3 dir = RM_NORMALIZED(PREFETCHED ? mk(bp_x, bp_y, -1.) : mk(a.bp_x[tx0 + (lane % TILE_W)], a.bp_y[ty0 + (lane / TILE_W)], -1.), true);
#endif
    V3 orig = mk(a.cam_x, a.cam_y, a.cam_z);
    double weight = 1.;
    uint32_t depth = 1;
    uint32_t pix = lane;
    bool on = true;
    V3 acc = mk(0., 0., 0.);
    bool handed = false;

    StackEntry deep[STACK > 1 ? STACK - 1 : 1];
    uint32_t n_deep = 0;
    bool l0_full = false;
#ifdef RM_EXP_STAMPS
    uint32_t st_steps = 0, st_rays = 0, st_taken = 0;
#endif
    __builtin_amdgcn_wave_barrier();
#if defined(RM_EXP_STAMPS) && defined(RM_EXP_STARTUP)
    if (dir.x == 12345.678) sc.cnt[2] = 1u;
    sc.cnt[1] |= (((uint32_t)__builtin_amdgcn_s_memrealtime() - sc.cnt[3]) & 0xFFFFu) << 16;
#endif

    constexpr bool DIV = !CULL;
    constexpr bool HANDOVER = CULL;
    const uint32_t dead_word = DIV ? own_sgpr(a.dead_children) : 0u;
    const bool dead_children = (dead_word & RM_DEAD_DROP) != 0u, early_fates = (dead_word & RM_DEAD_EARLY_FATES) != 0u;
    uint32_t step = 0;
    for (;; step++) {
        if (step == 1u) __builtin_amdgcn_s_setprio(1);
        else if (step == 2u) __builtin_amdgcn_s_setprio(2);
        else if (step == 3u) __builtin_amdgcn_s_setprio(3);
#ifdef RM_EXP_STAMPS
        st_steps++; st_rays += (uint32_t)__popcll(__ballot(on));
#endif
        bool next = false;
        if (where<DIV>(on)) {
            Hit h;
            const unsigned long long t_ch = RM_PHASE_T();
            const bool got = closest_hit<BVH, CULL, EDGES>(sc, orig, dir, on, h, have_mask & (step == 0u), first_mask) & on;
            RM_PHASE_ADD(sc, 0, t_ch);
            V3 L = bg;
            const double w_add = (on & (got | (depth > 1u))) ? weight : 0.;
            double w_cap = 0.;
            if (DIV && !got && depth > 1u) acc = acc + scaled(bg, weight);
            if (where<DIV>(got)) {
                const Surface s = surface_at<DIV>(sc, orig, dir, h, got RM_SUS_ARG);
                const unsigned long long t_sd = RM_PHASE_T();
                L = pick(got, bg + shade_direct<POW, BVH, CULL, EDGES>(sc, neg(dir), s, got, h.pid RM_SUS_ARG), bg);
                RM_PHASE_ADD(sc, 3, t_sd);
                if (DIV) acc = acc + scaled(L, weight);
                const bool glass = got & (s.mat[8] != 0.);
                if (where<DIV>(glass)) {
                    const double reflection = s.mat[6], ri = s.mat[7], inv_ri = s.mat[9];
                    V3 ro, rd, to, td;
                    double dn_r, dn_t;
                    const bool has_r = glass & reflect_child<DIV>(dir, s, ri, inv_ri, ro, rd, dn_r);
                    bool has_t = false, fated_dead = false;
                    if (!DIV) has_t = glass & refract_child(dir, s, ri, inv_ri, glass, to, td, dn_t RM_SUS_ARG);
                    const double wr = weight * reflection, wt = weight * (1. - reflection);
                    const bool capped = depth + 1u > max_depth;
                    if (DIV) {
                        const RefractFate f = refract_fate(dir, s, ri, inv_ri);
                        has_t = glass & f.has;
                        bool ray = glass;
                        if (early_fates) {
                            const uint32_t sides = (uint32_t)s.mat[8];
                            fated_dead = dead_children & has_t & !capped & (f.cos_theta_2 >= RM_FATE_COS2_MIN) & (f.r <= RM_FATE_R_MAX) &
                                         ((sides & (f.flip ? 2u : 4u)) != 0u);
                            ray = has_t & !capped & !fated_dead;
                        }
                        dn_t = 0.;
                        if (ray) {
                            refract_ray(dir, s, f, glass, to, td, dn_t RM_SUS_ARG);
                            orig = to;
                            dir = td;
                        }
                    }
                    w_cap = ((capped & has_r) ? wr : 0.) + ((capped & has_t) ? wt : 0.);
                    if (DIV && capped) acc = acc + scaled(bg, w_cap);
                    bool live_r = has_r & !capped, live_t = has_t & !capped;
                    if (DIV && dead_children) {
                        const uint32_t sides = (uint32_t)s.mat[8];
                        const bool dead_t = fated_dead | (live_t & (((dn_t > 0.) & ((sides & 2u) != 0u)) | ((dn_t < 0.) & ((sides & 4u) != 0u))));
                        if (dead_t) acc = acc + scaled(bg, wt);
                        live_t = live_t & !dead_t;
                        if (live_r & !live_t) {
                            const bool dead_r = ((dn_r > 0.) & ((sides & 2u) != 0u)) | ((dn_r < 0.) & ((sides & 4u) != 0u));
                            if (dead_r) acc = acc + scaled(bg, wr);
                            live_r = live_r & !dead_r;
                        }
                    }
                    const bool park = live_r & live_t, park_l0 = park & (n_deep == 0u) & !l0_full;
                    if (park_l0) {
                        lds0[0] = ro.x; lds0[64] = ro.y; lds0[128] = ro.z;
                        lds0[192] = rd.x; lds0[256] = rd.y; lds0[320] = rd.z;
                        lds0[384] = wr;
                        l0_depth[lane] = depth + 1u;
                    }
                    if (park & !park_l0) {
                        StackEntry &e = deep[n_deep];
                        e.ox = ro.x; e.oy = ro.y; e.oz = ro.z;
                        e.dx = rd.x; e.dy = rd.y; e.dz = rd.z;
                        e.w = wr; e.depth = depth + 1u;
                    }
                    n_deep += (park & !park_l0) ? 1u : 0u;
                    l0_full = l0_full | park_l0;
                    next = live_r | live_t;
                    orig = pick(live_t, DIV ? orig : to, ro);
                    dir = pick(live_t, DIV ? dir : td, rd);
                    weight = live_t ? wt : wr;
                    depth += 1u;
                }
            }
            const V3 term = mk(__builtin_fma(bg.x, w_cap, L.x * w_add), __builtin_fma(bg.y, w_cap, L.y * w_add),
                               __builtin_fma(bg.z, w_cap, L.z * w_add));
            if (DIV) {
            } else if (!HANDOVER || pix == lane) {
                acc = acc + term;
            } else {
                __hip_atomic_fetch_add(&sum[pix * 3 + 0], term.x, __ATOMIC_RELAXED, __HIP_MEMORY_SCOPE_WAVEFRONT);
                __hip_atomic_fetch_add(&sum[pix * 3 + 1], term.y, __ATOMIC_RELAXED, __HIP_MEMORY_SCOPE_WAVEFRONT);
                __hip_atomic_fetch_add(&sum[pix * 3 + 2], term.z, __ATOMIC_RELAXED, __HIP_MEMORY_SCOPE_WAVEFRONT);
            }
            const bool pop_deep = on & !next & (n_deep > 0u);
            if (where<DIV>(pop_deep)) {
                n_deep -= pop_deep ? 1u : 0u;
                const StackEntry &e = deep[pop_deep ? n_deep : 0u];
                orig = pick(pop_deep, mk(e.ox, e.oy, e.oz), orig);
                dir = pick(pop_deep, mk(e.dx, e.dy, e.dz), dir);
                weight = pop_deep ? e.w : weight;
                depth = pop_deep ? e.depth : depth;
// ... 98 lines not shown
#else
    (void)stats;
#endif
    return false;
}
#undef RM_SUS_PARAM
#undef RM_SUS_ARG
#undef RM_NORMALIZED
#undef RM_SQRT_DISCRIMINANT
#if RM_CHECKED
#undef RM_CHECKED_X_MIN
#undef RM_CHECKED_X_MAX
#endif

#if !RM_CHECKED

#ifndef RM_PATCH_COST_OP
#define RM_PATCH_COST_OP atomicMax
#endif

#ifndef RM_ORD_POLLS
#define RM_ORD_POLLS 65536u
#endif
__device__ __forceinline__ uint32_t order_entry(const KernelArgs &a, uint32_t k, bool &sky, bool &last_resort) {
    const uint32_t n_dyn = (a.n_tiles >> 4) - (a.n_static >> 4);
    uint32_t entry = 0u;
    bool gave_up = k >= a.ord_cap || k >= n_dyn;
    last_resort = false;
    if (a.ord_read != a.ord_flat) {
        if (!gave_up) entry = a.ord_read[k];
        last_resort = (entry >> RM_ORD_TAG_SHIFT) != a.ord_read_tag;
    } else {
        for (uint32_t polls = 0u; !gave_up; polls++) {
            entry = uniform_u32(__hip_atomic_load(a.ord_flat + k, __ATOMIC_RELAXED, __HIP_MEMORY_SCOPE_AGENT));
            if ((entry >> RM_ORD_TAG_SHIFT) == a.ord_tag) break;
            if ((polls & 63u) == 63u) {
                uint32_t go = uniform_u32(__hip_atomic_load(a.ord_cnt + RM_ORD_GO, __ATOMIC_RELAXED, __HIP_MEMORY_SCOPE_AGENT));
                if (go == 0u && polls >= RM_ORD_PATIENCE) {
                    uint32_t expected = 0u;
                    if ((threadIdx.x & 63u) == 0u)
                        (void)__hip_atomic_compare_exchange_strong(a.ord_cnt + RM_ORD_GO, &expected, a.ord_tag | RM_ORD_FALLBACK_BIT, __ATOMIC_RELAXED, __ATOMIC_RELAXED, __HIP_MEMORY_SCOPE_AGENT);
                    go = uniform_u32(__hip_atomic_load(a.ord_cnt + RM_ORD_GO, __ATOMIC_RELAXED, __HIP_MEMORY_SCOPE_AGENT));
                }
                if (go == (a.ord_tag | RM_ORD_FALLBACK_BIT)) { last_resort = true; break; }
                if (polls >= RM_ORD_POLLS) { gave_up = true; break; }
            }
            __builtin_amdgcn_s_sleep(8);
        }
    }
    uint32_t patch = entry & (RM_ORD_SKY_BIT - 1u);
    sky = (entry & RM_ORD_SKY_BIT) != 0u;
    if (last_resort && !gave_up) {
        patch = lists_ok(a) ? a.dyn_inv[k] : n_dyn - 1u - k;
        sky = false;
    }
    if (gave_up || patch >= (a.n_tiles >> 4)) {
        if ((threadIdx.x & 63u) == 0u && a.err_word) __hip_atomic_store(a.err_word, ((unsigned long long)a.launch_seq << 32) | 1ull, __ATOMIC_RELAXED, __HIP_MEMORY_SCOPE_SYSTEM);
        return ~0u;
    }
    return patch;
}

template <int STACK, int POW, bool STAGED, bool BVH, bool CULL, bool EDGES>
__device__ __attribute__((noinline)) void render_patch_alone(const char *kargs_of_kernel, uint32_t tile0, uint32_t n = 16u, bool staged = false) {
    const unsigned long long kv = (unsigned long long)kargs_of_kernel;
    const unsigned long long ku = ((unsigned long long)(uint32_t)__builtin_amdgcn_readfirstlane((int)(uint32_t)(kv >> 32)) << 32) |
                                  (uint32_t)__builtin_amdgcn_readfirstlane((int)(uint32_t)kv);
    const char *kargs = (const char *)reinterpret_cast<const __attribute__((address_space(4))) char *>(ku);
    const double *__restrict__ scene_blob = *reinterpret_cast<const double *const *>(kargs);
    const KernelArgs &a = *reinterpret_cast<const KernelArgs *>(kargs + sizeof(const double *));
    double *__restrict__ frame = *reinterpret_cast<double *const *>(kargs + sizeof(const double *) + sizeof(KernelArgs));
    for (uint32_t t = 0; t < n; t++) {
        const uint32_t tile = tile0 + t;
        uint32_t tx0, ty0, tyf, ty8;
        tile_origin(a, tile, tx0, ty0, tyf, ty8);
        unsigned long long first_mask = ~0ull;
        bool have_mask = false;
        if (a.tile_mask && a.mask_tag) {
            const unsigned long long w = uniform_u64(__hip_atomic_load(const_cast<unsigned long long *>(a.tile_mask) + tile, __ATOMIC_RELAXED, __HIP_MEMORY_SCOPE_AGENT));
            if ((uint32_t)(w >> 56) == a.mask_tag) { first_mask = w & 0x00FFFFFFFFFFFFFFull; have_mask = true; }
        }
        if (STAGED && !staged) stage_scene(scene_blob, a.H);
        double *wl = rm_lds + (STAGED ? a.H.total_words : 0u);
        const unsigned long long t0 = __builtin_amdgcn_s_memrealtime();
        SceneView sc;
        if (STAGED) sc.S = rm_lds; else sc.S = scene_blob;
        sc.G = scene_blob;
        sc.cull_bounds = scene_blob + a.H.off_bounds;
        sc.cull_planar = scene_blob + a.H.off_planar;
        sc.bstack = reinterpret_cast<uint32_t *>(wl + RM_WAVE_BVH_STACK_WORDS);
        sc.cull_cos = a.cull_cos;
        sc.H = a.H;
#ifdef RM_EXP_STAMPS
        uint32_t cull_counts[4] = {0u, 0u, 0u, 0u};
        sc.cnt = cull_counts;
#endif
        (void)render_tile<STACK, POW, BVH, CULL, EDGES, false>(sc, a, tx0, ty0, tyf, ty8, 0., 0., wl, frame, nullptr, have_mask & (a.mask_exact != 0u), first_mask, kargs_of_kernel);
        if (a.patch_cost && (threadIdx.x & 63u) == 0u) {
            const unsigned long long dt = __builtin_amdgcn_s_memrealtime() - t0;
            RM_PATCH_COST_OP(a.patch_cost + (tile >> 4), dt < 0x00FFFFFFull ? (uint32_t)dt : 0x00FFFFFFu);
        }
        __builtin_amdgcn_wave_barrier();
    }
}

template <int STACK, int POW, bool STAGED, bool BVH, bool CULL, bool EDGES>
__device__ __attribute__((noinline)) void sky_tail_patch(const char *kargs_of_kernel, uint32_t t) {
    const unsigned long long kv = (unsigned long long)kargs_of_kernel;
    const unsigned long long ku = ((unsigned long long)(uint32_t)__builtin_amdgcn_readfirstlane((int)(uint32_t)(kv >> 32)) << 32) |
                                  (uint32_t)__builtin_amdgcn_readfirstlane((int)(uint32_t)kv);
    const char *kargs = (const char *)reinterpret_cast<const __attribute__((address_space(4))) char *>(ku);
    const KernelArgs &a = *reinterpret_cast<const KernelArgs *>(kargs + sizeof(const double *));
    double *__restrict__ frame = *reinterpret_cast<double *const *>(kargs + sizeof(const double *) + sizeof(KernelArgs));
    const uint32_t n_dyn = (a.n_tiles >> 4) - (a.n_static >> 4);
    bool sky, last_resort;
    const uint32_t patch = order_entry(a, n_dyn - a.tail_patches + t, sky, last_resort);
    if (patch == ~0u) return;
    const uint32_t tile0 = patch * 16u, lane = threadIdx.x & 63u;
    if (last_resort && a.tile_mask && a.mask_tag) {
        unsigned long long *word = const_cast<unsigned long long *>(a.tile_mask) + tile0 + (lane & 15u);
        for (uint32_t polls = 0u; polls < 64u; polls++) {
            const unsigned long long w = __hip_atomic_load(word, __ATOMIC_RELAXED, __HIP_MEMORY_SCOPE_AGENT);
            if (__all((uint32_t)(w >> 56) == a.mask_tag)) { sky = !__any((w & 0x00FFFFFFFFFFFFFFull) != 0ull); break; }
            __builtin_amdgcn_s_sleep(8);
        }
    }
    if (!sky) {
        if (t < a.ov_cap && !last_resort) return;
        render_patch_alone<STACK, POW, STAGED, BVH, CULL, EDGES>(kargs, tile0);
        return;
    }
    constexpr uint32_t PIECES = TILE_W * 3u / 2u, P8 = TILE_W * 3u / 8u;
    for (uint32_t i = 0; i < 16u; i++) {
        uint32_t tx0, ty0, tyf, ty8;
        tile_origin(a, tile0 + i, tx0, ty0, tyf, ty8);
        for (uint32_t q = lane; q < 96u; q += 64u) {
            double2 *dst = reinterpret_cast<double2 *>(frame + ((size_t)(tyf + q / PIECES) * a.frame_width + tx0) * 3u);
            dst[q % PIECES] = double2{0., 0.};
        }
        if (a.frame8 && lane < 24u) {
            unsigned long long *dst = reinterpret_cast<unsigned long long *>(a.frame8 + ((size_t)(ty8 + lane / P8) * a.frame_width + tx0) * 3u);
            dst[lane % P8] = 0ull;
        }
    }
}

#ifndef RM_ORDERED_TILE_INLINE
#define RM_ORDERED_TILE_INLINE __forceinline__
#endif
template <int STACK, int POW, bool STAGED, bool BVH, bool CULL, bool EDGES>
__device__ RM_ORDERED_TILE_INLINE uint32_t ordered_tile(const char *kargs_of_kernel, uint32_t id_v) {
    const unsigned long long kv = (unsigned long long)kargs_of_kernel;
    const unsigned long long ku = ((unsigned long long)(uint32_t)__builtin_amdgcn_readfirstlane((int)(uint32_t)(kv >> 32)) << 32) |
                                  (uint32_t)__builtin_amdgcn_readfirstlane((int)(uint32_t)kv);
    const char *kargs = (const char *)reinterpret_cast<const __attribute__((address_space(4))) char *>(ku);
    const KernelArgs &a = *reinterpret_cast<const KernelArgs *>(kargs + sizeof(const double *));
    const uint32_t id = (uint32_t)__builtin_amdgcn_readfirstlane((int)id_v);
    const uint32_t n_dyn = (a.n_tiles >> 4) - (a.n_static >> 4), behind = 16u * (n_dyn - a.tail_patches);
    uint32_t m = id - a.n_static, k, sub;
    bool handed = false;
    if (m >= behind + a.tail_patches) {
        m -= behind + a.tail_patches;
        if (m >= 16u * a.ov_cap) {
            order_places(a, m - 16u * a.ov_cap, nullptr, false, true);
            return ~0u;
        }
        k = n_dyn - a.tail_patches + (m >> 4);
        sub = m & 15u;
        handed = true;
    } else {
        if (a.tail_patches) {
            const uint32_t before = a.tail_q == 1u ? (m >= behind ? m - behind : 0u) : a.tail_q ? __umulhi(m, a.tail_q) : min(m, a.tail_patches);
            const bool mine = a.tail_q == 1u ? m >= behind : a.tail_q ? __umulhi(m + 1u, a.tail_q) > before : m < a.tail_patches;
            if (mine) {
                sky_tail_patch<STACK, POW, STAGED, BVH, CULL, EDGES>(kargs_of_kernel, before);
                return ~0u;
            }
            m -= before;
        }
        k = m >> 4;
        sub = 15u - (m & 15u);
    }
    bool sky, last_resort;
    const uint32_t patch = order_entry(a, k, sky, last_resort);
    if (patch == ~0u || (handed && (sky || last_resort))) return ~0u;
    return patch * 16u + sub;
}

#ifndef RM_CLASSIFY_WG_INLINE
#define RM_CLASSIFY_WG_INLINE __forceinline__
#endif
template <bool ORDER, bool STAGED>
__device__ RM_CLASSIFY_WG_INLINE unsigned long long classify_workgroup(const char *kargs_of_kernel, uint32_t id_v, unsigned long long t_start) {
    const unsigned long long kv = (unsigned long long)kargs_of_kernel;
    const unsigned long long ku = ((unsigned long long)(uint32_t)__builtin_amdgcn_readfirstlane((int)(uint32_t)(kv >> 32)) << 32) |
                                  (uint32_t)__builtin_amdgcn_readfirstlane((int)(uint32_t)kv);
    const char *kargs = (const char *)reinterpret_cast<const __attribute__((address_space(4))) char *>(ku);
    const double *__restrict__ scene_blob = *reinterpret_cast<const double *const *>(kargs);
    const KernelArgs &a = *reinterpret_cast<const KernelArgs *>(kargs + sizeof(const double *));
    const uint32_t id = (uint32_t)__builtin_amdgcn_readfirstlane((int)id_v);
    unsigned long long stats = 0ull;
    (void)t_start;
    const uint32_t n_patches = a.n_tiles >> 4;
    const bool bottom_up = a.order_mul == a.n_tiles - 1u && a.order_add == a.n_tiles - 1u && a.n_tiles > 1u;
    const bool ordering = ORDER && a.ord_cnt;
    if (ordering && a.ord_read == a.ord_flat) __builtin_amdgcn_s_setprio(3);
    const uint32_t iters = ordering ? a.cls_iters : 1u;
    auto patch_of = [&](uint32_t it, bool &valid) {
        const uint32_t q = (it * a.cls_blocks + id) * 4u + ((threadIdx.x & 63u) >> 4);
        valid = q < n_patches;
        return !valid ? 0u : bottom_up ? n_patches - 1u - q : q;
    };
    bool valid;
    uint32_t patch = patch_of(0u, valid);
    ClsAsked cls_asked = classify_ask(a, patch, valid);
    OrdAsked ord_asked{0u, 0u, 0u};
    if (ordering) ord_asked = order_ask(a, patch, valid);
    uint32_t ct_sum = 0u, ct_num = 0u;
    if (ordering && a.key_mode == RM_KEY_CONTENT) { ct_sum = a.ctab[threadIdx.x & 63u]; ct_num = a.ctab[64u + (threadIdx.x & 63u)]; }
#ifndef RM_CLASSIFY_FROM_MEMORY
    ClsView blob;
    OrdRec *rec;
    if (STAGED) {
        stage_scene(scene_blob, a.H);
        blob = cls_view_of_blob(rm_lds, a.H);
        rec = reinterpret_cast<OrdRec *>(rm_lds + a.H.total_words);
    } else if (a.cls_lds_words) {
        blob = cls_stage(scene_blob, a.H, rm_lds);
        rec = reinterpret_cast<OrdRec *>(rm_lds + a.cls_lds_words);
    } else {
        blob = cls_view_of_blob(scene_blob, a.H);
        rec = reinterpret_cast<OrdRec *>(rm_lds);
    }
#else
    const ClsView blob = cls_view_of_blob(scene_blob, a.H);
    OrdRec *rec = reinterpret_cast<OrdRec *>(rm_lds);
#endif
    const uint32_t prim_cost = !(ordering && a.key_mode == RM_KEY_CONTENT) ? 0u : ct_num ? (ct_sum / ct_num) << 6 : ~0u;
    if (ordering && id == 0u) {
        if (a.ord_cnt_next) for (uint32_t i = threadIdx.x & 63u; i < RM_ORD_CNT_WORDS; i += 64u) a.ord_cnt_next[i] = 0u;
        if (a.ctab_zero) for (uint32_t i = threadIdx.x & 63u; i < RM_CTAB_WORDS; i += 64u) a.ctab_zero[i] = 0u;
    }
    for (uint32_t it = 0; it < iters; it++) {
        bool valid_next = false;
        uint32_t patch_next = 0u;
        ClsAsked cls_next = cls_asked;
        OrdAsked ord_next = ord_asked;
        if (it + 1u < iters) {
            patch_next = patch_of(it + 1u, valid_next);
            cls_next = classify_ask(a, patch_next, valid_next);
            ord_next = order_ask(a, patch_next, valid_next);
        }
        unsigned long long sig, own;
        (void)classify_patches<true>(blob, a, patch, valid, cls_asked, const_cast<unsigned long long *>(a.tile_mask), a.cls_prims, a.mask_tag, sig, own);
#ifdef RM_EXP_STAMPS
        if (it + 1u == iters) stats = (__builtin_amdgcn_s_memrealtime() - t_start) & 0xFFFFFull;
#endif
        if (ordering) order_slot(a, id, patch, valid, sig, a.mask_exact ? own : ~0ull, prim_cost, ord_asked, rec + it * 4u, a.ord_rec ? a.ord_rec + (size_t)(it * a.cls_blocks + id) * 12u : nullptr);
        patch = patch_next; valid = valid_next; cls_asked = cls_next; ord_asked = ord_next;
    }
    if (ordering) {
        __builtin_amdgcn_wave_barrier();
#ifdef RM_EXP_STAMPS
        stats |= ((__builtin_amdgcn_s_memrealtime() - t_start) & 0xFFFFFull) << 20;
#endif
        order_places(a, id, rec, true, a.ord_rec == nullptr);
    }
    return stats;
}

template <int STACK, int POW, int WAVES, int TPW, bool STAGED = true, bool BVH = false, bool CULL = false, bool EDGES = false, bool ORDER = false, bool FEEDBACK = false>
__global__ __launch_bounds__(WAVES * 64) __attribute__((amdgpu_waves_per_eu(POW == POW_INTEGER ? (EDGES ? RM_EDGES_WAVES : RM_MIN_WAVES) : 1, 8))) void rm_render_static(const double *__restrict__ scene_blob, KernelArgs a,
                                                              double *__restrict__ frame) {
    static_assert(WAVES == 1 && TPW == 1, "one tile per wave, one wave per workgroup");
#ifdef RM_EXP_STAMPS
    const unsigned long long t_start = __builtin_amdgcn_s_memrealtime();
    unsigned long long tile_stats = 0;
    uint32_t cull_counts[4] = {0u, 0u, 0u, 0u};
    uint32_t st_tile = ~0u;
    unsigned long long st_mask = ~0ull;
    auto stamp = [&]() {
        if ((threadIdx.x & 63u) == 0 && a.debug_stamps) {
            unsigned long long *o = a.debug_stamps + 4ull * blockIdx.x;
            o[0] = t_start; o[1] = tile_stats; o[2] = __builtin_amdgcn_s_memrealtime();
            unsigned long long *x = a.debug_stamps + 4ull * gridDim.x + 2ull * blockIdx.x;
#if defined(RM_EXP_WALKSTATS) || defined(RM_EXP_PHASES) || defined(RM_EXP_STARTUP)
            o[3] = (unsigned long long)cull_counts[0] | ((unsigned long long)cull_counts[1] << 32);
            x[0] = st_tile; x[1] = (unsigned long long)cull_counts[2] | ((unsigned long long)cull_counts[3] << 32);
#else
            o[3] = (unsigned long long)cull_counts[0] | ((unsigned long long)cull_counts[1] << 16) |
                   ((unsigned long long)cull_counts[2] << 40) | ((unsigned long long)cull_counts[3] << 52);
            x[0] = st_tile; x[1] = st_mask;
#endif
        }
    };
#else
    auto stamp = []() {};
#endif
    const bool feedback = FEEDBACK && a.fb_flag != nullptr;
    if (feedback && blockIdx.x == 0u) {
        const uint32_t b = threadIdx.x;
        a.fb_zero[b] = 0u;
        if (b == 0u) a.fb_zero[RM_FB_BUCKETS] = 0u;
        if (a.fb_target != 0u) {
            uint32_t above = a.fb_hist[b] * RM_FB_SAMPLE;
            for (uint32_t off = 1u; off < 64u; off <<= 1) {
                const uint32_t o = (uint32_t)__shfl_down((int)above, off, 64);
                above += (b + off < 64u) ? o : 0u;
            }
            const unsigned long long fits = __ballot(above <= a.fb_target);
            const uint32_t first = (uint32_t)__builtin_ctzll(fits | (1ull << 63));
            const uint32_t total = (uint32_t)__shfl((int)above, 0, 64);
            if (b == 0u) *a.fb_threshold = total == 0u ? a.fb_long_ticks : max(fb_edge(first), 200u);
        }
    }

    uint32_t id = blockIdx.x;
    if (a.cls_blocks) {
        if (id < a.cls_blocks) {
#ifdef RM_EXP_STAMPS
            tile_stats = classify_workgroup<ORDER, STAGED>((const char *)__builtin_amdgcn_kernarg_segment_ptr(), id, t_start);
#else
            (void)classify_workgroup<ORDER, STAGED>((const char *)__builtin_amdgcn_kernarg_segment_ptr(), id, 0ull);
#endif
            stamp();
            return;
        }
        id -= a.cls_blocks;
    }
#ifdef RM_EARLY_LOADS
    constexpr bool EARLY = ORDER;
#else
    constexpr bool EARLY = false;
#endif
    SceneAsked scene_asked;
    if (STAGED && EARLY) scene_asked = stage_scene_ask(scene_blob, a.H);
    uint32_t tile = 0u;
    bool late = id >= a.first_round;
    bool listed_tile = false;
    if (ORDER && a.ord_cnt && id >= a.n_static) {
        tile = uniform_u32(ordered_tile<STACK, POW, STAGED, BVH, CULL, EDGES>((const char *)__builtin_amdgcn_kernarg_segment_ptr(), id));
        if (tile == ~0u) { stamp(); return; }
        late = true;
    } else if (feedback && id < a.fb_cap) {
        if (id >= min(a.fb_count[0], a.fb_cap)) { stamp(); return; }
        tile = a.fb_list[id];
        if (tile >= a.n_tiles) { stamp(); return; }
        listed_tile = true;
    } else {
        if (feedback) id -= a.fb_cap;
        if (id >= a.n_tiles) { stamp(); return; }
        if (ORDER && a.ord_cnt && a.static_list && a.lists_done) {
            const uint32_t done = *a.lists_done, cand = a.static_list[id >> 4];
            tile = done == a.lists_tag ? cand * 16u + (15u - (id & 15u)) : tile_of_id(a, id);
        } else {
            tile = tile_of_id(a, id);
        }
    }
#if defined(RM_EXP_STAMPS) && defined(RM_EXP_STARTUP)
    cull_counts[3] = (uint32_t)t_start;
    cull_counts[0] = ((uint32_t)__builtin_amdgcn_s_memrealtime() - cull_counts[3]) & 0xFFFFu;
#endif
    const uint32_t flagged = (feedback && !listed_tile) ? a.fb_flag[tile] : 0u;
    uint32_t tx0, ty0, tyf, ty8;
    tile_origin(a, tile, tx0, ty0, tyf, ty8);
    double bp_x = 0., bp_y = 0.;
    if (FEEDBACK || EARLY) { bp_x = a.bp_x[tx0 + ((threadIdx.x & 63u) % TILE_W)]; bp_y = a.bp_y[ty0 + ((threadIdx.x & 63u) / TILE_W)]; }
    uint32_t fb_thr = a.fb_long_ticks;
    if (feedback && a.fb_target != 0u) {
        fb_thr = __hip_atomic_load(a.fb_threshold, __ATOMIC_RELAXED, __HIP_MEMORY_SCOPE_AGENT);
        fb_thr = fb_thr ? fb_thr : a.fb_long_ticks;
    }
    if (flagged) { stamp(); return; }

    bool have_mask = a.tile_mask != nullptr && a.mask_exact != 0u;
    unsigned long long first_mask = ~0ull;
    if (a.tile_mask && a.mask_tag) {
        have_mask = false;
        if (late || a.mask_tag_prev) {
            unsigned long long *word = const_cast<unsigned long long *>(a.tile_mask) + tile;
            const unsigned long long t0 = __builtin_amdgcn_s_memrealtime();
            if (a.mask_tag_prev) {
                const unsigned long long w = a.tile_mask[tile];
                if ((uint32_t)(w >> 56) == a.mask_tag || (uint32_t)(w >> 56) == a.mask_tag_prev) { first_mask = w & 0x00FFFFFFFFFFFFFFull; have_mask = true; }
            }
            while (!have_mask) {
                const unsigned long long w = uniform_u64(__hip_atomic_load(word, __ATOMIC_RELAXED, __HIP_MEMORY_SCOPE_AGENT));
                if ((uint32_t)(w >> 56) == a.mask_tag || (a.mask_tag_prev && (uint32_t)(w >> 56) == a.mask_tag_prev)) { first_mask = w & 0x00FFFFFFFFFFFFFFull; have_mask = true; break; }
                if (__builtin_amdgcn_s_memrealtime() - t0 > 2000ull) break;
                __builtin_amdgcn_s_sleep(4);
            }
        }
    } else if (a.tile_mask) {
        first_mask = uniform_u64(a.tile_mask[tile]);
    }
    if (a.tile_mask) {
        if (first_mask == 0ull && !listed_tile) {
            const uint32_t lane = threadIdx.x & 63u;
            constexpr uint32_t PIECES = TILE_W * 3u / 2u, P8 = TILE_W * 3u / 8u;
            for (uint32_t q = lane; q < 96u; q += 64u) {
                double2 *dst = reinterpret_cast<double2 *>(frame + ((size_t)(tyf + q / PIECES) * a.frame_width + tx0) * 3u);
                dst[q % PIECES] = double2{0., 0.};
            }
            if (a.frame8 && lane < 24u) {
                unsigned long long *dst = reinterpret_cast<unsigned long long *>(a.frame8 + ((size_t)(ty8 + lane / P8) * a.frame_width + tx0) * 3u);
                dst[lane % P8] = 0ull;
            }
            if (feedback && (threadIdx.x & 63u) == 0u) a.fb_next_flag[tile] = 0;
            stamp();
            return;
        }
    }

#ifdef RM_EXP_STAMPS
    st_tile = tile; st_mask = have_mask ? first_mask : ~0ull;
#endif
    have_mask = have_mask & (a.mask_exact != 0u);
#if defined(RM_EXP_STAMPS) && defined(RM_EXP_STARTUP)
    cull_counts[0] |= (((uint32_t)__builtin_amdgcn_s_memrealtime() - cull_counts[3]) & 0xFFFFu) << 16;
#endif
    if (STAGED) { if (EARLY) stage_scene_put(scene_asked, a.H); else stage_scene(scene_blob, a.H); }
#if defined(RM_EXP_STAMPS) && defined(RM_EXP_STARTUP)
    cull_counts[1] = ((uint32_t)__builtin_amdgcn_s_memrealtime() - cull_counts[3]) & 0xFFFFu;
#endif
    const uint32_t cull_words = (!STAGED && CULL) ? a.cull_lds_words : 0u;
    if (!STAGED && CULL && cull_words) { cull_stage(scene_blob, a.H, rm_lds); __syncthreads(); }
    double *wl = rm_lds + (STAGED ? a.H.total_words : cull_words);
    if (ORDER && (threadIdx.x & 63u) == 0u) reinterpret_cast<uint32_t *>(wl + RM_WAVE_T0_WORDS)[0] = (uint32_t)__builtin_amdgcn_s_memrealtime();
#ifdef RM_CHECKED_NS
    constexpr bool CHECKED = STAGED && !BVH && !CULL;
    namespace tile_ns = RM_CHECKED_NS;
#else
    constexpr bool CHECKED = false;
    namespace tile_ns = RM_FLAVOR_NS;
#endif
    const unsigned long long fb_t0 = feedback ? __builtin_amdgcn_s_memrealtime() : 0ull;
    bool exact = CHECKED && a.exact_only != 0u;
    if (!exact) {
        tile_ns::SceneView sc;
        if (STAGED) sc.S = rm_lds; else sc.S = scene_blob;
        sc.G = scene_blob;
        sc.cull_bounds = cull_words ? rm_lds : scene_blob + a.H.off_bounds;
        sc.cull_planar = cull_words ? rm_lds + 4u * (a.H.n_spheres + a.H.n_polygons + a.H.n_triangles) : scene_blob + a.H.off_planar;
        sc.bstack = reinterpret_cast<uint32_t *>(wl + RM_WAVE_BVH_STACK_WORDS);
        sc.cull_cos = own_sgpr(a.cull_cos);
#ifdef RM_EXP_STAMPS
        sc.cnt = cull_counts;
#endif
        sc.H.n_spheres = own_sgpr(a.H.n_spheres);         sc.H.n_polygons = own_sgpr(a.H.n_polygons);
        sc.H.n_triangles = own_sgpr(a.H.n_triangles);     sc.H.n_lights = own_sgpr(a.H.n_lights);
        sc.H.off_spheres = own_sgpr(a.H.off_spheres);     sc.H.off_polygons = own_sgpr(a.H.off_polygons);
        sc.H.off_pverts = own_sgpr(a.H.off_pverts);       sc.H.off_triangles = own_sgpr(a.H.off_triangles);
        sc.H.off_materials = own_sgpr(a.H.off_materials); sc.H.off_lights = own_sgpr(a.H.off_lights);
        sc.H.off_keys = own_sgpr(a.H.off_keys);           sc.H.total_words = a.H.total_words;
        sc.H.list_ordered = own_sgpr(a.H.list_ordered);   sc.H.off_bvh_spheres = own_sgpr(a.H.off_bvh_spheres);
        sc.H.off_bvh_triangles = own_sgpr(a.H.off_bvh_triangles); sc.H.off_bounds = own_sgpr(a.H.off_bounds);
        sc.H.off_planar = own_sgpr(a.H.off_planar);       sc.H.off_groups = own_sgpr(a.H.off_groups);
        sc.H.off_occ = own_sgpr(a.H.off_occ);
        sc.H.shadow_rho = own_sgpr(a.H.shadow_rho);

#if defined(RM_EXP_STAMPS) && defined(RM_EXP_PHASES)
        cull_counts[2] = (uint32_t)(__builtin_amdgcn_s_memrealtime() - t_start);
#endif
#ifdef RM_EXP_STAMPS
        exact = tile_ns::render_tile<STACK, POW, BVH, CULL, EDGES, FEEDBACK || EARLY>(sc, a, tx0, ty0, tyf, ty8, bp_x, bp_y, wl, frame, &tile_stats, have_mask, first_mask, (const char *)__builtin_amdgcn_kernarg_segment_ptr());
#else
        exact = tile_ns::render_tile<STACK, POW, BVH, CULL, EDGES, FEEDBACK || EARLY>(sc, a, tx0, ty0, tyf, ty8, bp_x, bp_y, wl, frame, nullptr, have_mask, first_mask, (const char *)__builtin_amdgcn_kernarg_segment_ptr());
#endif
        if (CHECKED && exact) {
            const KernelArgs &b = *reinterpret_cast<const KernelArgs *>(reread_kernargs((const char *)__builtin_amdgcn_kernarg_segment_ptr()) + sizeof(const double *));
            if (b.redo_count && (threadIdx.x & 63u) == 0u) atomicAdd(b.redo_count, 1u);
        }
    }
    if constexpr (CHECKED) if (exact) render_patch_alone<STACK, POW, STAGED, BVH, CULL, EDGES>((const char *)__builtin_amdgcn_kernarg_segment_ptr(), tile, 1u, true);
    if (ORDER) {
#ifdef RM_NO_REREAD
        const KernelArgs &b = a;
#else
        const KernelArgs &b = *reinterpret_cast<const KernelArgs *>(reread_kernargs((const char *)__builtin_amdgcn_kernarg_segment_ptr()) + sizeof(const double *));
#endif
        if (b.patch_cost) {
            const uint32_t dt = min(uniform_u32((uint32_t)__builtin_amdgcn_s_memrealtime() - reinterpret_cast<const uint32_t *>(wl + RM_WAVE_T0_WORDS)[0]), 0x00FFFFFFu);
            if ((threadIdx.x & 63u) == 0u) RM_PATCH_COST_OP(b.patch_cost + (tile >> 4), dt);
            if ((tile & 15u) == 0u && b.ctab_cur && b.tile_mask && b.mask_tag && b.mask_exact) {
                const unsigned long long w = uniform_u64(__hip_atomic_load(const_cast<unsigned long long *>(b.tile_mask) + tile, __ATOMIC_RELAXED, __HIP_MEMORY_SCOPE_AGENT));
                if ((uint32_t)(w >> 56) == b.mask_tag && ((w >> (threadIdx.x & 63u)) & 1ull) && (threadIdx.x & 63u) < 56u) {
                    atomicAdd(b.ctab_cur + (threadIdx.x & 63u), dt >> 6);
                    atomicAdd(b.ctab_cur + 64u + (threadIdx.x & 63u), 1u);
                }
            }
        }
    }
#ifdef RM_EXP_STAMPS
    if (a.tile_mask) st_mask = __hip_atomic_load(const_cast<unsigned long long *>(a.tile_mask) + tile, __ATOMIC_RELAXED, __HIP_MEMORY_SCOPE_AGENT) & 0x00FFFFFFFFFFFFFFull;
#endif
    if (feedback) {
        const unsigned long long fb_dt = __builtin_amdgcn_s_memrealtime() - fb_t0;
        const uint32_t ticks = fb_dt < 0x7FFFFFFFull ? (uint32_t)fb_dt : 0x7FFFFFFFu;
        const bool is_long = ticks >= fb_thr;
        if ((threadIdx.x & 63u) == 0u) {
            if (a.fb_target != 0u && tile % RM_FB_SAMPLE == 0u) atomicAdd(a.fb_next_hist + fb_bucket(ticks), 1u);
            bool listed = false;
            if (is_long) {
                const uint32_t slot = atomicAdd(a.fb_next_count, 1u);
                if (slot < a.fb_cap) { a.fb_next_list[slot] = tile; listed = true; }
            }
            a.fb_next_flag[tile] = listed ? 1 : 0;
        }
    }
    stamp();
}
// ... 5 lines not shown
```

### rusty-marcher_amd/csrc/rm_trace.inc

```
namespace RM_FLAVOR_NS {
using namespace rmdev;


struct V3 { double x, y, z; };

__device__ __forceinline__ V3 mk(double x, double y, double z) { return V3{x, y, z}; }
__device__ __forceinline__ V3 operator+(V3 a, V3 b) { return mk(a.x + b.x, a.y + b.y, a.z + b.z); }
__device__ __forceinline__ V3 operator-(V3 a, V3 b) { return mk(a.x - b.x, a.y - b.y, a.z - b.z); }
__device__ __forceinline__ V3 operator*(V3 a, V3 b) { return mk(a.x * b.x, a.y * b.y, a.z * b.z); }
__device__ __forceinline__ V3 neg(V3 a) { return mk(-a.x, -a.y, -a.z); }
__device__ __forceinline__ V3 scaled(V3 a, double s) { return mk(a.x * s, a.y * s, a.z * s); }
__device__ __forceinline__ V3 pick(bool c, V3 a, V3 b) { return mk(c ? a.x : b.x, c ? a.y : b.y, c ? a.z : b.z); }
__device__ __forceinline__ double dot(V3 a, V3 b) { return a.x * b.x + a.y * b.y + a.z * b.z; }
#ifndef RM_CHECKED
#define RM_CHECKED 0
#endif
#if RM_CHECKED
#define RM_SUS_PARAM , bool &sus
#define RM_SUS_ARG , sus
#else
#define RM_SUS_PARAM
#define RM_SUS_ARG
#endif
#if RM_CHECKED
// ... 896 lines not shown
    const uint32_t ns = sc.H.n_spheres, np = sc.H.n_polygons;
    const uint32_t pid = got ? h.pid : 0u;
    const bool is_s = got & (pid < ns);
    const bool is_p = got & !is_s & (pid < ns + np);
    const bool is_t = got & !is_s & !is_p;
    s.normal = mk(0., 0., 0.);
    if (where<DIV>(is_s)) {
        const double *sp = sc.S + sc.H.off_spheres + RM_SPHERE_WORDS * (is_s ? pid : 0u);
        const V3 centre = spheres.centre(sp, is_s ? pid : 0u);
        s.normal = RM_NORMALIZED(mk(s.point.x - centre.x, s.point.y - centre.y, s.point.z - centre.z), is_s);
    }
    if (where<DIV>(is_p | is_t)) {
        const uint32_t word = is_p ? sc.H.off_polygons + RM_POLYGON_WORDS * (pid - ns)
                            : is_t ? sc.H.off_triangles + RM_TRIANGLE_WORDS * (pid - ns - np)
                                   : 0u;
        const double *rec = sc.S + word;
        s.normal = pick(is_s, s.normal, mk(rec[0], rec[1], rec[2]));
    }
    s.mat = sc.S + sc.H.off_materials + RM_MATERIAL_WORDS * pid;
    return s;
}

__device__ __forceinline__ V3 reflect(V3 incident, V3 normal) {
    return incident - scaled(normal, 2. * dot(incident, normal));
}

template <int POW>
__device__ __forceinline__ double specular_pow(double x, double y) {
    if (POW == POW_GENERIC) return pow(x, y);
    uint32_t n = (uint32_t)y;
    double r = 1., b = x;
    const uint32_t n0 = __builtin_amdgcn_readfirstlane(n);
    if (__all(n == n0)) {
        for (uint32_t m = n0; m != 0u; m >>= 1) {
            if (m & 1u) r = r * b;
            if (m > 1u) b = b * b;
        }
        return r;
    }
    while (__any(n != 0u)) {
        if (n & 1u) r = r * b;
        b = b * b;
        n >>= 1;
    }
    return r;
}

__device__ __forceinline__ double dot_fused(V3 a, V3 b) {
    return __builtin_fma(a.z, b.z, __builtin_fma(a.y, b.y, a.x * b.x));
}

struct LightAt {
    V3 dir;
    V3 from;
    V3 pos;
    double ldn, sf;
    bool dark;
};

struct StoredLights {
    __device__ __forceinline__ V3 operator()(const double *lt, uint32_t) const { return mk(lt[0], lt[1], lt[2]); }
};

template <class LIGHTS = StoredLights>
__device__ __forceinline__ LightAt light_at(const SceneView &sc, uint32_t l, const Surface &s, V3 dir_to_viewer, double exponent, bool got RM_SUS_PARAM,
                                            const LIGHTS &lights = LIGHTS()) {
    (void)got;
    LightAt a;
    const double *lt = sc.G + sc.H.off_lights + RM_LIGHT_WORDS * l;
    a.pos = lights(lt, l);
    a.dir = RM_NORMALIZED(a.pos - s.point, got);
    a.ldn = dot(a.dir, s.normal);
    a.from = s.point + scaled(s.normal, (a.ldn < 0.) ? -1e-3 : 1e-3);
    const double k2 = -2. * dot_fused(a.dir, s.normal);
    const V3 reflected = mk(__builtin_fma(-k2, s.normal.x, -a.dir.x), __builtin_fma(-k2, s.normal.y, -a.dir.y),
                            __builtin_fma(-k2, s.normal.z, -a.dir.z));
    a.sf = __builtin_fmax(dot_fused(reflected, dir_to_viewer), 0.);
    a.dark = !(a.ldn > 0.) & !(a.sf > 0.) & (exponent > 0.);
    return a;
}

template <int POW, bool BVH, bool CULL, bool EDGES, class LIGHTS = StoredLights, class SPHERES = StoredSpheres>
__device__ __forceinline__ V3 shade_direct(const SceneView &sc, V3 neg_dir, const Surface &s, bool got, uint32_t pid RM_SUS_PARAM,
                                           const LIGHTS &lights = LIGHTS(), const SPHERES &spheres = SPHERES()) {
    const double *m = s.mat;
    const double exponent = m[5];
    const V3 dir_to_viewer = neg_dir;
    V3 li = mk(0., 0., 0.);
    auto add_light = [&](uint32_t l, const LightAt &a, bool lit) {
        if (lit) {
            const double *lt = sc.G + sc.H.off_lights + RM_LIGHT_WORDS * l;
            const V3 lcol = mk(lt[3], lt[4], lt[5]);
            const double intensity = lt[6];
            const V3 diffuse_color = mk(m[1], m[2], m[3]);
            const double specular_k = m[4];
            const double diffusion = __builtin_fmax(a.ldn, 0.);
            const double di = diffusion * intensity;
            const double spec = specular_pow<POW>(a.sf * specular_k, exponent);
            li = mk(__builtin_fma(lcol.x, spec, __builtin_fma(lcol.x * diffuse_color.x, di, li.x)),
                    __builtin_fma(lcol.y, spec, __builtin_fma(lcol.y * diffuse_color.y, di, li.y)),
                    __builtin_fma(lcol.z, spec, __builtin_fma(lcol.z * diffuse_color.z, di, li.z)));
        }
    };
    const bool masks = !BVH && !CULL && !SPHERES::moves && sc.H.off_occ != 0u;
    for (uint32_t l = 0; l < sc.H.n_lights;) {
        const LightAt a = light_at(sc, l, s, dir_to_viewer, exponent, got RM_SUS_ARG, lights);
        const bool dec_a = !got | a.dark;
        if (!BVH && !CULL && l + 1u < sc.H.n_lights) {
            const LightAt b = light_at(sc, l + 1u, s, dir_to_viewer, exponent, got RM_SUS_ARG, lights);
            const bool dec_b = !got | b.dark;
            if (__all(dec_a | dec_b | ((a.ldn < 0.) == (b.ldn < 0.)))) {
                bool occ_a, occ_b;
                const unsigned long long t_sh = RM_PHASE_T();
                const V3 from = pick(dec_a, b.from, a.from);
                unsigned long long m_a = 0ull, m_b = 0ull;
                if (masks) shadow_masks2(sc, got, pid, l, m_a, m_b);
                const uint32_t n = sc.H.n_spheres + sc.H.n_polygons + sc.H.n_triangles;
                if (masks && (m_a & m_b) != ((n >= 64u) ? ~0ull : (1ull << n) - 1ull))
                    any_hit2_masked(sc, from, a.dir, b.dir, dec_a, dec_b, occ_a, occ_b, m_a, m_b);
                else
                    any_hit2(sc, from, a.dir, b.dir, dec_a, dec_b, occ_a, occ_b, spheres);
                RM_PHASE_ADD(sc, 1, t_sh);
                add_light(l, a, !occ_a);
                add_light(l + 1u, b, !occ_b);
                l += 2u;
                continue;
            }
        }
        const unsigned long long t_sh = RM_PHASE_T();
        const bool lit = !any_hit<BVH, CULL, EDGES>(sc, a.from, a.dir, dec_a, a.pos, sc.H.shadow_rho, spheres);
        RM_PHASE_ADD(sc, 1, t_sh);
        add_light(l, a, lit);
        l += 1u;
    }
    return scaled(li, m[0]);
}

template <bool LAZY>
__device__ __forceinline__ bool reflect_child(V3 incident, const Surface &s, double ri, double inv_ri, V3 &o, V3 &d, double &dn) {
    const double c = dot(s.normal, incident);
    const double r = (c < 0.) ? ri : inv_ri;
    const double cos_theta_2 = 1. - r * r * (1. - c * c);
    const bool has = !(cos_theta_2 > 0.);
    dn = 0.;
    if (!LAZY || has) {
        d = reflect(incident, s.normal);
        dn = dot(d, s.normal);
        o = s.point + scaled(s.normal, (dn < 0.) ? -1e-4 : 1e-4);
    }
    return has;
}
template <bool LAZY>
__device__ __forceinline__ bool reflect_child(V3 incident, const Surface &s, double ri, double inv_ri, V3 &o, V3 &d) {
    double dn;
    return reflect_child<LAZY>(incident, s, ri, inv_ri, o, d, dn);
}

__device__ __forceinline__ bool refract_child(V3 incident, const Surface &s, double ri, double inv_ri, bool glass, V3 &o, V3 &d, double &dn RM_SUS_PARAM) {
    (void)glass;
    const double c0 = -dot(s.normal, incident);
    const bool flip = c0 < 0.;
    const double r = flip ? ri : inv_ri;
    const double c = flip ? -c0 : c0;
    const double cos_theta_2 = 1. - r * r * (1. - c * c);
    const double k = r * c - __builtin_sqrt(cos_theta_2);
    d = RM_NORMALIZED(scaled(incident, r) + scaled(s.normal, flip ? -k : k), glass & !(cos_theta_2 < 0.));
    dn = dot(d, s.normal);
    const bool along = flip ? (dn < 0.) : (dn > 0.);
    o = s.point + scaled(s.normal, (along != flip) ? 1e-4 : -1e-4);
    return !(cos_theta_2 < 0.);
}
struct RefractFate { double r, c, cos_theta_2; bool flip, has; };
#define RM_FATE_COS2_MIN 0x1p-16
#define RM_FATE_R_MAX 16.
__device__ __forceinline__ RefractFate refract_fate(V3 incident, const Surface &s, double ri, double inv_ri) {
    RefractFate f;
    const double c0 = -dot(s.normal, incident);
    f.flip = c0 < 0.;
    f.r = f.flip ? ri : inv_ri;
    f.c = f.flip ? -c0 : c0;
    f.cos_theta_2 = 1. - f.r * f.r * (1. - f.c * f.c);
    f.has = !(f.cos_theta_2 < 0.);
    return f;
}
__device__ __forceinline__ void refract_ray(V3 incident, const Surface &s, const RefractFate &f, bool glass, V3 &o, V3 &d, double &dn RM_SUS_PARAM) {
    (void)glass;
#ifdef RM_AB_FATE_SCALED_ROOT
    const double k = f.r * f.c - __builtin_sqrt(f.cos_theta_2);
#else
    const double k = f.r * f.c - RM_SQRT_DISCRIMINANT(f.cos_theta_2);
#endif
    d = RM_NORMALIZED(scaled(incident, f.r) + scaled(s.normal, f.flip ? -k : k), glass & f.has);
    dn = dot(d, s.normal);
    const bool along = f.flip ? (dn < 0.) : (dn > 0.);
    o = s.point + scaled(s.normal, (along != f.flip) ? 1e-4 : -1e-4);
}
__device__ __forceinline__ bool refract_child(V3 incident, const Surface &s, double ri, double inv_ri, bool glass, V3 &o, V3 &d RM_SUS_PARAM) {
    double dn;
    return refract_child(incident, s, ri, inv_ri, glass, o, d, dn RM_SUS_ARG);
// ... 4 lines not shown
```

Measured before the change: 33000.

## Add per-tile shadow occluder masks computed during classification

During tile classification, the kernel now computes a second per-tile word holding, for the first two lights, the union of possible shadow occluders over the primitives the tile can hit. It builds these from cone tests on each primitive's tile footprint. Shading reads this word into LDS and ANDs it with the per-primitive shadow masks, so the masked any-hit path tests fewer occluders. The cost is a doubled tile-mask buffer, extra classification work and per-wave reads. Host-side cone code is factored into a shared header, and readback and debug hooks are added.

```diff
diff --git a/rusty-marcher_amd/csrc/rm_classify.inc b/rusty-marcher_amd/csrc/rm_classify.inc
--- a/rusty-marcher_amd/csrc/rm_classify.inc
+++ b/rusty-marcher_amd/csrc/rm_classify.inc
@@ -199,6 +199,30 @@
     return sig != 0ull;
 }
 
+__device__ __forceinline__ unsigned long long tile_shadow_word(const ClsView &v, const double *__restrict__ blob, const KernelArgs &a, const ClsAsked &asked,
+                                                               unsigned long long own) {
+    const uint32_t ns = a.H.n_spheres, np = a.H.n_polygons, n = ns + np + a.H.n_triangles, nl = a.H.n_lights;
+    const unsigned long long all = (1ull << n) - 1ull;
+    const unsigned long long *occ = reinterpret_cast<const unsigned long long *>(blob + a.H.off_occ);
+    const double *lw = blob + a.H.off_lights;
+    const rm_sc_v3 l0{lw[0], lw[1], lw[2]}, l1{lw[RM_LIGHT_WORDS], lw[RM_LIGHT_WORDS + 1u], lw[RM_LIGHT_WORDS + 2u]};
+    const rm_sc_v3 o{a.cam_x, a.cam_y, a.cam_z};
+    auto corner = [&](double bx, double by) { const V3 d = cls_dir(a, bx, by); return rm_sc_v3{d.x, d.y, d.z}; };
+    const rm_sc_v3 corners[4] = {corner(asked.tx0, asked.ty0), corner(asked.tx1, asked.ty0), corner(asked.tx0, asked.ty1), corner(asked.tx1, asked.ty1)};
+    unsigned long long m0 = 0ull, m1 = 0ull;
+    for (unsigned long long m = own & all; m != 0ull; m &= m - 1ull) {
+        const uint32_t pid = (uint32_t)__builtin_ctzll(m);
+        if (pid < ns) { m0 |= occ[pid * nl]; m1 |= occ[pid * nl + 1u]; continue; }
+        const double *rec = pid < ns + np ? v.poly + v.poly_stride * (pid - ns) : v.tri + v.tri_stride * (pid - ns - np);
+        rm_sc_v3 c;
+        double rad;
+        if (!rm_tile_footprint(o, corners, rm_sc_v3{rec[0], rec[1], rec[2]}, rm_sc_v3{rec[3], rec[4], rec[5]}, c, rad)) { m0 = m1 = all; break; }
+        m0 |= rm_shadow_cone_mask(v.bounds, n, pid, l0, c, rad, a.H.shadow_rho);
+        m1 |= rm_shadow_cone_mask(v.bounds, n, pid, l1, c, rad, a.H.shadow_rho);
+    }
+    return ((m1 & all) << 28) | (m0 & all);
+}
+
 __device__ __forceinline__ uint32_t cost_bucket(uint32_t ticks) {
     if (ticks < 512u) return RM_ORD_SKY - 1u;
     const uint32_t e = 31u - (uint32_t)__builtin_clz(ticks);
diff --git a/rusty-marcher_amd/csrc/rm_device.hip b/rusty-marcher_amd/csrc/rm_device.hip
--- a/rusty-marcher_amd/csrc/rm_device.hip
+++ b/rusty-marcher_amd/csrc/rm_device.hip
@@ -146,6 +146,7 @@
     uint64_t image_epoch = 0;
     std::vector<rm_tile_lists> tile_lists;
     uint32_t last_launch_grid = 0, last_launch_tail = 0;
+    uint32_t last_launch_shadow_off = 0, last_launch_mask_tag = 0, last_launch_cls_blocks = 0;
     uint32_t last_launch_tiles = 0;
     bool last_launch_classified = false;
     hipStream_t last_launch_stream = nullptr;
@@ -620,7 +621,8 @@
         if (t->block) RM_HIP(ctx, hipFree(t->block));
         t->block = nullptr;
         t->cap = n_tiles;
-        RM_HIP(ctx, hipMalloc(&t->block, (size_t)n_tiles * sizeof(unsigned long long)));
+        RM_HIP(ctx, hipMalloc(&t->block, 2u * (size_t)n_tiles * sizeof(unsigned long long)));
+        RM_HIP(ctx, hipMemset(t->block, 0, 2u * (size_t)n_tiles * sizeof(unsigned long long)));
     }
     *out = t;
     return RM_OK;
@@ -738,7 +740,7 @@
         if (rm_status fst = feedback_for(ctx, stream, P, &fb)) return fst;
     if (P.classify) {
         if (rm_status cst = tile_lists_for(ctx, stream, P.args.n_tiles, &tl)) return cst;
-        if (P.clear_masks) RM_HIP(ctx, hipMemsetAsync(tl->block, 0, (size_t)tl->cap * sizeof(unsigned long long), stream));
+        if (P.clear_masks) RM_HIP(ctx, hipMemsetAsync(tl->block, 0, 2u * (size_t)tl->cap * sizeof(unsigned long long), stream));
     }
     if (P.ordered) {
         if (tl->order_cap < P.order_patches) {
@@ -771,6 +773,7 @@
     a.bp_y = ctx->d_backproject + p->frame_width;
     a.frame8 = d_frame8;
     a.redo_count = ctx->d_redo;
+    a.tile_shadow_off = P.tile_shadow ? tl->cap : 0u;
 
     if (P.cls_fn) {
         P.cls_args.tile_mask = tl->mask();
@@ -790,6 +793,9 @@
     ctx->last_launch_stream = stream;
     ctx->last_launch_grid = P.grid;
     ctx->last_launch_tail = a.tail_patches;
+    ctx->last_launch_shadow_off = a.tile_shadow_off;
+    ctx->last_launch_mask_tag = a.mask_tag;
+    ctx->last_launch_cls_blocks = a.cls_blocks;
     ctx->last_launch_exact_only = P.exact_only;
     if (ctx->knobs.debug_tail && P.ordered)
         if (rm_status dst = dump_order(ctx, P, stream)) return dst;
@@ -917,6 +923,22 @@
     if (workgroups) *workgroups = ctx->last_launch_grid;
     if (tail_patches) *tail_patches = ctx->last_launch_tail;
     return RM_OK;
+}
+
+extern "C" rm_status rmi_tile_shadow_readback(rm_ctx *ctx, uint64_t *hit, uint64_t *shadow, uint32_t cap, uint32_t *dims) {
+    if (!ctx || !dims) return ctx_fail(ctx, RM_ERR_INVALID_ARG, "rmi_tile_shadow_readback: NULL argument");
+    RM_HIP(ctx, hipSetDevice(ctx->device));
+    RM_HIP(ctx, hipDeviceSynchronize());
+    const uint32_t n = ctx->last_launch_tiles, off = ctx->last_launch_shadow_off;
+    dims[0] = n; dims[1] = off ? 1u : 0u; dims[2] = ctx->last_launch_mask_tag; dims[3] = ctx->last_launch_cls_blocks;
+    if (!off || !hit || !shadow || n > cap) return RM_OK;
+    for (const rm_tile_lists &t : ctx->tile_lists)
+        if (t.stream == ctx->last_launch_stream && t.block && n <= t.cap && off == t.cap) {
+            RM_HIP(ctx, hipMemcpy(hit, t.mask(), (size_t)n * 8u, hipMemcpyDeviceToHost));
+            RM_HIP(ctx, hipMemcpy(shadow, t.mask() + off, (size_t)n * 8u, hipMemcpyDeviceToHost));
+            return RM_OK;
+        }
+    return ctx_fail(ctx, RM_ERR_INVALID_ARG, "rmi_tile_shadow_readback: the last launch's words are gone");
 }
 
 static rm_status rm_tile_stats_impl(rm_ctx *ctx, void *hip_stream, uint32_t *tiles, uint32_t *tiles_listed) {
diff --git a/rusty-marcher_amd/csrc/rm_image.cpp b/rusty-marcher_amd/csrc/rm_image.cpp
--- a/rusty-marcher_amd/csrc/rm_image.cpp
+++ b/rusty-marcher_amd/csrc/rm_image.cpp
@@ -7,6 +7,7 @@
 
 #include "rm_bvh.hpp"
 #include "rm_plan.hpp"
+#include "rm_shadow_cone.hpp"
 
 namespace {
 
@@ -44,8 +45,8 @@
     const uint32_t n = H.n_spheres + H.n_polygons + H.n_triangles, nl = H.n_lights;
     const unsigned long long all = n >= 64u ? ~0ull : ((1ull << n) - 1ull);
     const double rho = H.shadow_rho;
+    auto sc3 = [](rm_vec3 v) { return rm_sc_v3{v.x, v.y, v.z}; };
     auto finite3 = [](rm_vec3 v) { return std::isfinite(v.x) && std::isfinite(v.y) && std::isfinite(v.z); };
-    auto mag = [](rm_vec3 v) { return std::fabs(v.x) + std::fabs(v.y) + std::fabs(v.z); };
     for (uint32_t l = 0; l < nl; l++) {
         const double *lw = blob + H.off_lights + RM_LIGHT_WORDS * l;
         const rm_vec3 L = v3(lw[0], lw[1], lw[2]);
@@ -53,17 +54,9 @@
             unsigned long long &m = occ[(size_t)P * nl + l];
             m = all;
             const double *bp = blob + H.off_bounds + 4u * P;
-            const rm_vec3 c = v3(bp[0], bp[1], bp[2]);
-            if (!(bp[3] >= 0.) || !std::isfinite(bp[3]) || !finite3(c) || !finite3(L) || !(rho >= 0.) || !std::isfinite(rho)) continue;
-            const double tol = 1e-7 * (1. + mag(L) + mag(c) + bp[3]);
-            const double r = bp[3] + tol;
-            const rm_vec3 cl = c - L;
-            const double D = std::sqrt(dot(cl, cl));
-            if (!(D > r * (1. + 1e-6) + rho + tol)) continue;
-            const rm_vec3 a = scaled(cl, 1. / D);
-            const double sin_t = std::fmin(1., r / D * (1. + 1e-9) + 1e-9);
-            const double cos_t = std::sqrt(std::fmax(0., 1. - sin_t * sin_t)) * (1. - 1e-9);
-            const double cap = D + r;
+            rm_shadow_cone k;
+            if (!rm_shadow_cone_of(k, sc3(L), rm_sc_v3{bp[0], bp[1], bp[2]}, bp[3], rho)) continue;
+            const rm_vec3 cl = v3(k.cl.x, k.cl.y, k.cl.z), a = v3(k.a.x, k.a.y, k.a.z);
             unsigned long long keep = 1ull << P;
             for (uint32_t Q = 0; Q < n; Q++) {
                 if (Q == P) continue;
@@ -71,11 +64,8 @@
                 if (bq[3] < 0.) continue;
                 const rm_vec3 cq = v3(bq[0], bq[1], bq[2]);
                 if (!std::isfinite(bq[3]) || !finite3(cq)) { keep |= 1ull << Q; continue; }
-                const double marg = rho + tol + 1e-7 * (mag(cq) + bq[3]);
-                const double R = bq[3] + marg;
-                const rm_vec3 v = cq - L, x = cross(v, a);
-                const double h = dot(v, a), q = std::sqrt(dot(x, x));
-                bool out = (q * cos_t - std::fabs(h) * sin_t > R) || (h - R > cap);
+                const double marg = rm_shadow_cone_margin(k, sc3(cq), bq[3]);
+                bool out = rm_shadow_cone_sphere_out(k, sc3(cq), bq[3], marg);
                 if (!out && Q >= H.n_spheres) {
                     const double *pl = blob + H.off_planar + 16u * (Q - H.n_spheres);
                     const uint32_t nv = pl[12] == 3. ? 3u : pl[12] == 4. ? 4u : 0u;
@@ -84,12 +74,12 @@
                     for (uint32_t i = 0; i < nv; i++) { w[i] = v3(pl[3 * i], pl[3 * i + 1], pl[3 * i + 2]) - L; fin = fin && finite3(w[i]); }
                     if (fin) {
                         PlaneSep sep;
-                        try_plane(sep, a, w, nv, cl, r, a, sin_t, marg);
-                        try_plane(sep, v3(1., 0., 0.), w, nv, cl, r, a, sin_t, marg);
-                        try_plane(sep, v3(0., 1., 0.), w, nv, cl, r, a, sin_t, marg);
-                        try_plane(sep, v3(0., 0., 1.), w, nv, cl, r, a, sin_t, marg);
-                        try_plane(sep, cross(w[1] - w[0], w[2] - w[0]), w, nv, cl, r, a, sin_t, marg);
-                        for (uint32_t i = 0; i < nv; i++) try_plane(sep, cross(w[i], w[(i + 1u) % nv]), w, nv, cl, r, a, sin_t, marg);
+                        try_plane(sep, a, w, nv, cl, k.r, a, k.sin_t, marg);
+                        try_plane(sep, v3(1., 0., 0.), w, nv, cl, k.r, a, k.sin_t, marg);
+                        try_plane(sep, v3(0., 1., 0.), w, nv, cl, k.r, a, k.sin_t, marg);
+                        try_plane(sep, v3(0., 0., 1.), w, nv, cl, k.r, a, k.sin_t, marg);
+                        try_plane(sep, cross(w[1] - w[0], w[2] - w[0]), w, nv, cl, k.r, a, k.sin_t, marg);
+                        for (uint32_t i = 0; i < nv; i++) try_plane(sep, cross(w[i], w[(i + 1u) % nv]), w, nv, cl, k.r, a, k.sin_t, marg);
                         out = sep.h && sep.n;
                     }
                 }
@@ -539,6 +529,50 @@
     return RM_OK;
 }
 
+extern "C" rm_status rmi_tile_shadow_words(const rm_scene_desc *d, const rm_vec3 *camera, const rm_camera_basis *basis, const rm_params *p,
+                                           uint64_t *words, uint64_t cap, uint32_t *shape_of, uint32_t *dims) {
+    rm_image img;
+    if (rm_status st = hook_image("rmi_tile_shadow_words", d, (camera && p) ? dims : nullptr, rm_image_options{}, img)) return st;
+    const rm_dev_header &H = img.H;
+    const uint32_t n = H.n_spheres + H.n_polygons + H.n_triangles;
+    const uint32_t cols = (p->frame_width / RM_PATCH_SIZE) * 2u, rows = (p->frame_height / RM_PATCH_SIZE) * 8u;
+    dims[0] = n; dims[1] = H.n_spheres; dims[2] = H.n_lights;
+    dims[3] = (H.off_occ && n <= RM_TILE_SHADOW_MAX_PRIMS && H.n_lights >= 2u) ? 1u : 0u;
+    dims[4] = cols; dims[5] = rows;
+    if (!dims[3] || !words || !shape_of || (uint64_t)cols * rows * n * 2u > cap) return RM_OK;
+    for (uint32_t q = 0; q < n; q++) shape_of[q] = img.pid_map[2u * q];
+    const double *blob = img.blob.data();
+    const unsigned long long *occ = reinterpret_cast<const unsigned long long *>(blob + H.off_occ);
+    const rm_camera_basis fixed{rm_vec3{1., 0., 0.}, rm_vec3{0., 1., 0.}, rm_vec3{0., 0., -1.}};
+    const rm_camera_basis &cb = basis ? *basis : fixed;
+    auto bp_x = [&](uint32_t x) { return 2. * ((double)x / p->width - 0.5) * p->half_fov * p->ratio; };
+    auto bp_y = [&](uint32_t y) { return -2. * ((double)y / p->height - 0.5) * p->half_fov; };
+    auto dir = [&](double bx, double by) {
+        return rm_sc_v3{(bx * cb.right.x + by * cb.up.x) + cb.forward.x, (bx * cb.right.y + by * cb.up.y) + cb.forward.y, (bx * cb.right.z + by * cb.up.z) + cb.forward.z};
+    };
+    const rm_sc_v3 o{camera->x, camera->y, camera->z};
+    const unsigned long long all = (1ull << n) - 1ull;
+    for (uint32_t row = 0; row < rows; row++)
+        for (uint32_t col = 0; col < cols; col++) {
+            const double x0 = bp_x(16u * col), x1 = bp_x(16u * col + 15u), y0 = bp_y(4u * row), y1 = bp_y(4u * row + 3u);
+            const rm_sc_v3 corners[4] = {dir(x0, y0), dir(x1, y0), dir(x0, y1), dir(x1, y1)};
+            uint64_t *w = words + ((size_t)row * cols + col) * n * 2u;
+            for (uint32_t P = 0; P < n; P++) {
+                if (P < H.n_spheres) { w[2u * P] = occ[(size_t)P * H.n_lights]; w[2u * P + 1u] = occ[(size_t)P * H.n_lights + 1u]; continue; }
+                const double *rec = P < H.n_spheres + H.n_polygons ? blob + H.off_polygons + RM_POLYGON_WORDS * (P - H.n_spheres)
+                                                                   : blob + H.off_triangles + RM_TRIANGLE_WORDS * (P - H.n_spheres - H.n_polygons);
+                rm_sc_v3 c;
+                double rad;
+                const bool ok = rm_tile_footprint(o, corners, rm_sc_v3{rec[0], rec[1], rec[2]}, rm_sc_v3{rec[3], rec[4], rec[5]}, c, rad);
+                for (uint32_t l = 0; l < 2u; l++) {
+                    const double *lw = blob + H.off_lights + RM_LIGHT_WORDS * l;
+                    w[2u * P + l] = ok ? rm_shadow_cone_mask(blob + H.off_bounds, n, P, rm_sc_v3{lw[0], lw[1], lw[2]}, c, rad, H.shadow_rho) : all;
+                }
+            }
+        }
+    return RM_OK;
+}
+
 extern "C" rm_status rmi_empty_sides(const rm_scene_desc *d, uint8_t *sides, double *glass, uint32_t *shape_of, uint32_t cap, uint32_t *dims, double *camera_limit) {
     rm_image img;
     if (rm_status st = hook_image("rmi_empty_sides", d, dims, rm_image_options{}, img)) return st;
diff --git a/rusty-marcher_amd/csrc/rm_kernel_args.hpp b/rusty-marcher_amd/csrc/rm_kernel_args.hpp
--- a/rusty-marcher_amd/csrc/rm_kernel_args.hpp
+++ b/rusty-marcher_amd/csrc/rm_kernel_args.hpp
@@ -1,6 +1,7 @@
 #ifndef RM_KERNEL_ARGS_HPP
 #define RM_KERNEL_ARGS_HPP
 
+#include <stddef.h>
 #include <stdint.h>
 
 #include "rm_internal.h"
@@ -24,6 +25,7 @@
 #define RM_ORD_TAG_SHIFT (RM_ORD_PATCH_BITS + 1u)
 #define RM_ORD_TAG_BITS 11u
 #define RM_CTAB_WORDS 128u
+#define RM_TILE_SHADOW_MAX_PRIMS 28u
 enum { RM_KEY_PLACE = 0, RM_KEY_COST = 1, RM_KEY_CONTENT = 2 };
 
 #ifndef RM_MIN_WAVES
@@ -82,6 +84,7 @@
     uint32_t cls_prims;
     uint32_t cls_lds_words;
     uint32_t cull_lds_words;
+    uint32_t tile_shadow_off;
     uint32_t *ord_cnt;
     uint32_t *ord_cnt_next;
     uint32_t *ord_flat;
@@ -121,6 +124,8 @@
 };
 
 static constexpr uint32_t RM_DEAD_DROP = 1u, RM_DEAD_EARLY_FATES = 2u;
+static_assert(sizeof(KernelArgs) == offsetof(KernelArgs, redo_count) + sizeof(uint32_t *) && offsetof(KernelArgs, ord_cnt) == offsetof(KernelArgs, tile_shadow_off) + 4u,
+              "tile_shadow_off fills padding: nothing behind it moves");
 
 struct ClassifyArgs {
     unsigned long long *tile_mask;
@@ -143,6 +148,7 @@
 #define RM_WAVE_SUM_WORDS 512u
 #define RM_WAVE_PAIR_WORDS 704u
 #define RM_WAVE_T0_WORDS 736u
+#define RM_WAVE_SHADOW_WORDS 737u
 #define RM_WAVE_LDS_WORDS 738u
 #define RM_LDS_SCENE_LIMIT_WORDS 512u
 
diff --git a/rusty-marcher_amd/csrc/rm_plan.cpp b/rusty-marcher_amd/csrc/rm_plan.cpp
--- a/rusty-marcher_amd/csrc/rm_plan.cpp
+++ b/rusty-marcher_amd/csrc/rm_plan.cpp
@@ -44,6 +44,7 @@
     {"RM_FORCE_FAST_FP", &rm_knobs::force_fast_fp, IS_1},
     {"RM_FORCE_UNSTAGED", &rm_knobs::force_unstaged, IS_1},
     {"RM_SHADOW_MASKS", &rm_knobs::shadow_masks, NOT_0},
+    {"RM_TILE_SHADOW", &rm_knobs::tile_shadow, NOT_0},
     {"RM_DEAD_CHILDREN", &rm_knobs::dead_children, DEAD_CHILDREN},
     {"RM_DISABLE_BVH", &rm_knobs::disable_bvh, IS_1},
     {"RM_SWEPT_BVH", &rm_knobs::swept_bvh, NOT_0},
@@ -294,6 +295,8 @@
             a.cls_prims = n_prims;
             P.grid += a.cls_blocks;
             cls_words_wanted = (!k.staged && kn.classify_lds) ? 4u * n_prims + 22u * n_planar : 0u;
+            P.tile_shadow = kn.tile_shadow && k.staged && !k.bvh && !k.cull && a.H.off_occ != 0u && a.H.n_lights >= 2u &&
+                            n_prims <= RM_TILE_SHADOW_MAX_PRIMS;
         } else {
             s.tagged = false;
             P.cls_fn = sc.oriented ? rm_classify_kernel_oriented(n_planar > 0u) : rm_classify_kernel(n_planar > 0u);
diff --git a/rusty-marcher_amd/csrc/rm_plan.hpp b/rusty-marcher_amd/csrc/rm_plan.hpp
--- a/rusty-marcher_amd/csrc/rm_plan.hpp
+++ b/rusty-marcher_amd/csrc/rm_plan.hpp
@@ -23,6 +23,7 @@
     bool cull_edges = true;
     bool force_unstaged = false;
     bool shadow_masks = true;
+    bool tile_shadow = true;
     bool dead_children = true;
     bool early_fates = true;
     int force_stack = 0;
@@ -189,6 +190,7 @@
     bool feedback_reset = false;
     size_t feedback_bytes = 0, feedback_set_bytes = 0;
     bool clear_masks = false;
+    bool tile_shadow = false;
     uint32_t order_patches = 0;
     enum { ORDER_CLEAR_NONE, ORDER_CLEAR_FLAT, ORDER_CLEAR_ALL } order_clear = ORDER_CLEAR_NONE;
     uint32_t order_cap = 0;
diff --git a/rusty-marcher_amd/csrc/rm_render_kernel.hpp b/rusty-marcher_amd/csrc/rm_render_kernel.hpp
--- a/rusty-marcher_amd/csrc/rm_render_kernel.hpp
+++ b/rusty-marcher_amd/csrc/rm_render_kernel.hpp
@@ -4,6 +4,7 @@
 #include <hip/hip_runtime.h>
 
 #include "rm_kernel_args.hpp"
+#include "rm_shadow_cone.hpp"
 
 namespace rmdev {
 
diff --git a/rusty-marcher_amd/csrc/rm_render_kernel.inc b/rusty-marcher_amd/csrc/rm_render_kernel.inc
--- a/rusty-marcher_amd/csrc/rm_render_kernel.inc
+++ b/rusty-marcher_amd/csrc/rm_render_kernel.inc
@@ -50,7 +50,11 @@
     const bool dead_children = (dead_word & RM_DEAD_DROP) != 0u, early_fates = (dead_word & RM_DEAD_EARLY_FATES) != 0u;
     uint32_t step = 0;
     for (;; step++) {
-        if (step == 1u) __builtin_amdgcn_s_setprio(1);
+        if (step == 1u) {
+            __builtin_amdgcn_s_setprio(1);
+            if (!BVH && !CULL && lane == (uint32_t)__builtin_amdgcn_readfirstlane((int)lane))
+                reinterpret_cast<unsigned long long *>(wl + RM_WAVE_SHADOW_WORDS)[0] = ~0ull;
+        }
         else if (step == 2u) __builtin_amdgcn_s_setprio(2);
         else if (step == 3u) __builtin_amdgcn_s_setprio(3);
 #ifdef RM_EXP_STAMPS
@@ -69,7 +73,8 @@
             if (where<DIV>(got)) {
                 const Surface s = surface_at<DIV>(sc, orig, dir, h, got RM_SUS_ARG);
                 const unsigned long long t_sd = RM_PHASE_T();
-                L = pick(got, bg + shade_direct<POW, BVH, CULL, EDGES>(sc, neg(dir), s, got, h.pid RM_SUS_ARG), bg);
+                const unsigned long long *tile_word = (!BVH && !CULL) ? reinterpret_cast<const unsigned long long *>(wl + RM_WAVE_SHADOW_WORDS) : nullptr;
+                L = pick(got, bg + shade_direct<POW, BVH, CULL, EDGES>(sc, neg(dir), s, got, h.pid RM_SUS_ARG, StoredLights(), StoredSpheres(), tile_word), bg);
                 RM_PHASE_ADD(sc, 3, t_sd);
                 if (DIV) acc = acc + scaled(L, weight);
                 const bool glass = got & (s.mat[8] != 0.);
@@ -334,6 +339,7 @@
         }
         if (STAGED && !staged) stage_scene(scene_blob, a.H);
         double *wl = rm_lds + (STAGED ? a.H.total_words : 0u);
+        if (!BVH && !CULL && (threadIdx.x & 63u) == 0u) reinterpret_cast<unsigned long long *>(wl + RM_WAVE_SHADOW_WORDS)[0] = ~0ull;
         const unsigned long long t0 = __builtin_amdgcn_s_memrealtime();
         SceneView sc;
         if (STAGED) sc.S = rm_lds; else sc.S = scene_blob;
@@ -442,7 +448,7 @@
 #ifndef RM_CLASSIFY_WG_INLINE
 #define RM_CLASSIFY_WG_INLINE __forceinline__
 #endif
-template <bool ORDER, bool STAGED>
+template <bool ORDER, bool STAGED, bool SHADOW>
 __device__ RM_CLASSIFY_WG_INLINE unsigned long long classify_workgroup(const char *kargs_of_kernel, uint32_t id_v, unsigned long long t_start) {
     const unsigned long long kv = (unsigned long long)kargs_of_kernel;
     const unsigned long long ku = ((unsigned long long)(uint32_t)__builtin_amdgcn_readfirstlane((int)(uint32_t)(kv >> 32)) << 32) |
@@ -518,6 +524,23 @@
 #endif
         order_places(a, id, rec, true, a.ord_rec == nullptr);
     }
+    if constexpr (SHADOW) {
+        if (a.tile_shadow_off && a.mask_tag) {
+            __builtin_amdgcn_s_setprio(0);
+            unsigned long long *hit_words = const_cast<unsigned long long *>(a.tile_mask);
+            for (uint32_t it = 0; it < iters; it++) {
+                bool v;
+                const uint32_t p = patch_of(it, v);
+                const ClsAsked q = classify_ask(a, p, v);
+                const uint32_t t = p * 16u + (threadIdx.x & 15u);
+                if (v) {
+                    const unsigned long long own = __hip_atomic_load(hit_words + t, __ATOMIC_RELAXED, __HIP_MEMORY_SCOPE_AGENT) & 0x00FFFFFFFFFFFFFFull;
+                    const unsigned long long w = tile_shadow_word(blob, scene_blob, a, q, own);
+                    __hip_atomic_store(hit_words + a.tile_shadow_off + t, ((unsigned long long)a.mask_tag << 56) | w, __ATOMIC_RELAXED, __HIP_MEMORY_SCOPE_AGENT);
+                }
+            }
+        }
+    }
     return stats;
 }
 
@@ -571,9 +594,9 @@
     if (a.cls_blocks) {
         if (id < a.cls_blocks) {
 #ifdef RM_EXP_STAMPS
-            tile_stats = classify_workgroup<ORDER, STAGED>((const char *)__builtin_amdgcn_kernarg_segment_ptr(), id, t_start);
-#else
-            (void)classify_workgroup<ORDER, STAGED>((const char *)__builtin_amdgcn_kernarg_segment_ptr(), id, 0ull);
+            tile_stats = classify_workgroup<ORDER, STAGED, STAGED && !BVH && !CULL>((const char *)__builtin_amdgcn_kernarg_segment_ptr(), id, t_start);
+#else
+            (void)classify_workgroup<ORDER, STAGED, STAGED && !BVH && !CULL>((const char *)__builtin_amdgcn_kernarg_segment_ptr(), id, 0ull);
 #endif
             stamp();
             return;
@@ -679,6 +702,17 @@
     if (!STAGED && CULL && cull_words) { cull_stage(scene_blob, a.H, rm_lds); __syncthreads(); }
     double *wl = rm_lds + (STAGED ? a.H.total_words : cull_words);
     if (ORDER && (threadIdx.x & 63u) == 0u) reinterpret_cast<uint32_t *>(wl + RM_WAVE_T0_WORDS)[0] = (uint32_t)__builtin_amdgcn_s_memrealtime();
+    if constexpr (STAGED && !BVH && !CULL) {
+        unsigned long long ts = ~0ull;
+        if (a.tile_shadow_off && a.tile_mask) {
+            const unsigned long long *word = a.tile_mask + a.tile_shadow_off + tile;
+            const unsigned long long w = a.mask_tag_prev ? *word
+                                                         : uniform_u64(__hip_atomic_load(const_cast<unsigned long long *>(word), __ATOMIC_RELAXED, __HIP_MEMORY_SCOPE_AGENT));
+            const uint32_t tag = (uint32_t)(w >> 56);
+            if (tag != 0u && (tag == a.mask_tag || tag == a.mask_tag_prev)) ts = w & 0x00FFFFFFFFFFFFFFull;
+        }
+        if ((threadIdx.x & 63u) == 0u) reinterpret_cast<unsigned long long *>(wl + RM_WAVE_SHADOW_WORDS)[0] = ts;
+    }
 #ifdef RM_CHECKED_NS
     constexpr bool CHECKED = STAGED && !BVH && !CULL;
     namespace tile_ns = RM_CHECKED_NS;
diff --git a/rusty-marcher_amd/csrc/rm_shadow_cone.hpp b/rusty-marcher_amd/csrc/rm_shadow_cone.hpp
--- /dev/null
+++ b/rusty-marcher_amd/csrc/rm_shadow_cone.hpp
@@ -0,0 +1,89 @@
+#ifndef RM_SHADOW_CONE_HPP
+#define RM_SHADOW_CONE_HPP
+
+#ifdef __HIPCC__
+#define RM_SC_FN __host__ __device__ inline
+#else
+#define RM_SC_FN inline
+#endif
+
+struct rm_sc_v3 { double x, y, z; };
+RM_SC_FN rm_sc_v3 rm_sc_sub(rm_sc_v3 a, rm_sc_v3 b) { return rm_sc_v3{a.x - b.x, a.y - b.y, a.z - b.z}; }
+RM_SC_FN rm_sc_v3 rm_sc_scaled(rm_sc_v3 a, double s) { return rm_sc_v3{a.x * s, a.y * s, a.z * s}; }
+RM_SC_FN double rm_sc_dot(rm_sc_v3 a, rm_sc_v3 b) { return a.x * b.x + a.y * b.y + a.z * b.z; }
+RM_SC_FN rm_sc_v3 rm_sc_cross(rm_sc_v3 a, rm_sc_v3 b) { return rm_sc_v3{a.y * b.z - a.z * b.y, a.z * b.x - a.x * b.z, a.x * b.y - a.y * b.x}; }
+RM_SC_FN double rm_sc_mag(rm_sc_v3 v) { return __builtin_fabs(v.x) + __builtin_fabs(v.y) + __builtin_fabs(v.z); }
+RM_SC_FN bool rm_sc_finite(double v) { return __builtin_fabs(v) <= 1.7976931348623157e308; }
+RM_SC_FN bool rm_sc_finite3(rm_sc_v3 v) { return rm_sc_finite(v.x) && rm_sc_finite(v.y) && rm_sc_finite(v.z); }
+
+struct rm_shadow_cone {
+    rm_sc_v3 L, cl, a;
+    double r, tol, rho, sin_t, cos_t, cap;
+};
+
+RM_SC_FN bool rm_shadow_cone_of(rm_shadow_cone &k, rm_sc_v3 L, rm_sc_v3 c, double rad, double rho) {
+    if (!(rad >= 0.) || !rm_sc_finite(rad) || !rm_sc_finite3(c) || !rm_sc_finite3(L) || !(rho >= 0.) || !rm_sc_finite(rho)) return false;
+    k.L = L;
+    k.rho = rho;
+    k.tol = 1e-7 * (1. + rm_sc_mag(L) + rm_sc_mag(c) + rad);
+    k.r = rad + k.tol;
+    k.cl = rm_sc_sub(c, L);
+    const double D = __builtin_sqrt(rm_sc_dot(k.cl, k.cl));
+    if (!(D > k.r * (1. + 1e-6) + rho + k.tol)) return false;
+    k.a = rm_sc_scaled(k.cl, 1. / D);
+    k.sin_t = __builtin_fmin(1., k.r / D * (1. + 1e-9) + 1e-9);
+    k.cos_t = __builtin_sqrt(__builtin_fmax(0., 1. - k.sin_t * k.sin_t)) * (1. - 1e-9);
+    k.cap = D + k.r;
+    return true;
+}
+
+RM_SC_FN double rm_shadow_cone_margin(const rm_shadow_cone &k, rm_sc_v3 cq, double rq) { return k.rho + k.tol + 1e-7 * (rm_sc_mag(cq) + rq); }
+
+RM_SC_FN bool rm_shadow_cone_sphere_out(const rm_shadow_cone &k, rm_sc_v3 cq, double rq, double marg) {
+    const double R = rq + marg;
+    const rm_sc_v3 v = rm_sc_sub(cq, k.L), x = rm_sc_cross(v, k.a);
+    const double h = rm_sc_dot(v, k.a), q = __builtin_sqrt(rm_sc_dot(x, x));
+    return (q * k.cos_t - __builtin_fabs(h) * k.sin_t > R) || (h - R > k.cap);
+}
+
+RM_SC_FN bool rm_tile_footprint(rm_sc_v3 o, const rm_sc_v3 *d, rm_sc_v3 n, rm_sc_v3 pp, rm_sc_v3 &c, double &rad) {
+    const double num = rm_sc_dot(rm_sc_sub(pp, o), n), mn = rm_sc_mag(n);
+    rm_sc_v3 pt[4];
+    double reach = rm_sc_mag(o);
+    c = rm_sc_v3{0., 0., 0.};
+    for (int i = 0; i < 4; i++) {
+        const double den = rm_sc_dot(d[i], n), md = rm_sc_mag(d[i]);
+        if (!(__builtin_fabs(den) >= 1e-4 * md * mn)) return false;
+        const double t = num / den;
+        if (!(t > 0.) || !rm_sc_finite(t)) return false;
+        pt[i] = rm_sc_v3{o.x + d[i].x * t, o.y + d[i].y * t, o.z + d[i].z * t};
+        if (!rm_sc_finite3(pt[i])) return false;
+        reach = __builtin_fmax(reach, rm_sc_mag(o) + t * md);
+        c.x += 0.25 * pt[i].x; c.y += 0.25 * pt[i].y; c.z += 0.25 * pt[i].z;
+    }
+    double r2 = 0.;
+    for (int i = 0; i < 4; i++) {
+        const rm_sc_v3 e = rm_sc_sub(pt[i], c);
+        r2 = __builtin_fmax(r2, rm_sc_dot(e, e));
+    }
+    rad = __builtin_sqrt(r2) * (1. + 1e-9) + 1e-3 + 1e-9 * reach;
+    return rm_sc_finite3(c) && rm_sc_finite(rad);
+}
+
+RM_SC_FN unsigned long long rm_shadow_cone_mask(const double *bounds, unsigned n, unsigned self, rm_sc_v3 L, rm_sc_v3 c, double rad, double rho) {
+    const unsigned long long all = n >= 64u ? ~0ull : ((1ull << n) - 1ull);
+    rm_shadow_cone k;
+    if (!rm_shadow_cone_of(k, L, c, rad, rho)) return all;
+    unsigned long long keep = self < n ? 1ull << self : 0ull;
+    for (unsigned Q = 0; Q < n; Q++) {
+        if (Q == self) continue;
+        const double *bq = bounds + 4u * Q;
+        if (bq[3] < 0.) continue;
+        const rm_sc_v3 cq = rm_sc_v3{bq[0], bq[1], bq[2]};
+        if (!rm_sc_finite(bq[3]) || !rm_sc_finite3(cq)) { keep |= 1ull << Q; continue; }
+        if (!rm_shadow_cone_sphere_out(k, cq, bq[3], rm_shadow_cone_margin(k, cq, bq[3]))) keep |= 1ull << Q;
+    }
+    return keep;
+}
+
+#endif
diff --git a/rusty-marcher_amd/csrc/rm_trace.inc b/rusty-marcher_amd/csrc/rm_trace.inc
--- a/rusty-marcher_amd/csrc/rm_trace.inc
+++ b/rusty-marcher_amd/csrc/rm_trace.inc
@@ -1002,7 +1002,8 @@
 
 template <int POW, bool BVH, bool CULL, bool EDGES, class LIGHTS = StoredLights, class SPHERES = StoredSpheres>
 __device__ __forceinline__ V3 shade_direct(const SceneView &sc, V3 neg_dir, const Surface &s, bool got, uint32_t pid RM_SUS_PARAM,
-                                           const LIGHTS &lights = LIGHTS(), const SPHERES &spheres = SPHERES()) {
+                                           const LIGHTS &lights = LIGHTS(), const SPHERES &spheres = SPHERES(),
+                                           const unsigned long long *tile_word = nullptr) {
     const double *m = s.mat;
     const double exponent = m[5];
     const V3 dir_to_viewer = neg_dir;
@@ -1034,7 +1035,13 @@
                 const unsigned long long t_sh = RM_PHASE_T();
                 const V3 from = pick(dec_a, b.from, a.from);
                 unsigned long long m_a = 0ull, m_b = 0ull;
-                if (masks) shadow_masks2(sc, got, pid, l, m_a, m_b);
+                if (masks) {
+                    shadow_masks2(sc, got, pid, l, m_a, m_b);
+                    if (tile_word && l == 0u) {
+                        const unsigned long long w = uniform_u64(*tile_word);
+                        if (w != ~0ull) { m_a &= w & 0x0FFFFFFFull; m_b &= (w >> 28) & 0x0FFFFFFFull; }
+                    }
+                }
                 const uint32_t n = sc.H.n_spheres + sc.H.n_polygons + sc.H.n_triangles;
                 if (masks && (m_a & m_b) != ((n >= 64u) ? ~0ull : (1ull << n) - 1ull))
                     any_hit2_masked(sc, from, a.dir, b.dir, dec_a, dec_b, occ_a, occ_b, m_a, m_b);
```

Result: no change. 32830 (-0.5%).
